# duckdb/duckdb-vss

Hardware: AMD Instinct MI355X
Metric: queries/sec at recall@10, 10M×768 FLOAT top-10; index build rows/sec (higher is better)
Workload: dtype f32

## Files before the change

### duckdb-vss_amd/__init__.py

```python
import ctypes as C
import os
import subprocess

import numpy as np

HERE = os.path.dirname(os.path.abspath(__file__))
ROOT = os.path.dirname(HERE)
LIB_PATH = os.environ.get("VSS_LIBRARY") or os.path.join(HERE, "libvssgpu.so")
CSRC = os.path.join(HERE, "csrc")

METRICS = {"l2sq": 0, "cosine": 1, "ip": 2}
FUNCTIONS = {"array_distance": 0, "array_cosine_distance": 1, "array_negative_inner_product": 2}
FREE_KEY = np.iinfo(np.int64).max

HIPCC_FLAGS = ["--offload-arch=gfx950", "-O3", "-std=c++17", "-ffp-contract=off", "-fPIC", "-Wno-int-to-pointer-cast"]


TRANSLATION_UNITS = ["vss_engine.hip", "vss_exchange.hip", "kernels_l2sq.hip", "kernels_cosine.hip", "kernels_ip.hip",
                     "kernels_boxes_l2sq.hip", "kernels_boxes_cosine.hip", "kernels_boxes_ip.hip",
                     "kernels_setboxes_l2sq.hip", "kernels_setboxes_cosine.hip", "kernels_setboxes_ip.hip"]


def build_library(force=False, extra_flags=(), out=None):
    out = out or os.path.join(HERE, "libvssgpu.so")
# ... 14 lines not shown
            raise RuntimeError("hipcc failed")
    subprocess.check_call(["hipcc", "--offload-arch=gfx950", "-shared", "-fPIC"] + objs + ["-o", out])
    return out


_u64, _i64, _vp, _int, _u32 = C.c_uint64, C.c_int64, C.c_void_p, C.c_int, C.c_uint32
WRITE_CB = C.CFUNCTYPE(_int, _vp, _vp, _u64)
READ_CB = C.CFUNCTYPE(_int, _vp, _vp, _u64)

SIGNATURES = {
    "vss_version": (C.c_char_p, []),
    "vss_create": (_int, [_u64, _int, _u64, _u64, _u64, _u64, _int, C.POINTER(_vp)]),
    "vss_destroy": (None, [_vp]),
    "vss_last_error": (C.c_char_p, [_vp]),
    "vss_set_stream": (_int, [_vp, _vp]),
    "vss_synchronize": (_int, [_vp]),
    "vss_reserve": (_int, [_vp, _u64, _u64]),
    "vss_stage_batch": (_int, [_vp, _vp, _vp, _vp, _u64]),
    "vss_stage_batch_device": (_int, [_vp, _vp, _vp, _u64]),
    "vss_build_finalize": (_int, [_vp]),
    "vss_add_batch": (_int, [_vp, _vp, _vp, _vp, _u64]),
    "vss_set_build_params": (_int, [_vp, _u64, _u64]),
    "vss_set_build_reorder": (_int, [_vp, _int]),
    "vss_set_option": (_int, [_vp, C.c_char_p, _i64]),
    "vss_search": (_int, [_vp, _vp, _u64, _u64, _vp, _vp]),
    "vss_search_batch": (_int, [_vp, _vp, _u64, _u64, _u64, _vp, _vp, _vp]),
    "vss_search_batch_device": (_int, [_vp, _vp, _u64, _u64, _u64, _vp, _vp, _vp]),
    "vss_search_batch_filtered": (_int, [_vp, _vp, _u64, _u64, _u64, _vp, _u64, _vp, _vp, _vp]),
    "vss_search_batch_filtered_device": (_int, [_vp, _vp, _u64, _u64, _u64, _vp, _u64, _vp, _vp, _vp]),
    "vss_search_batch_filtered_groups": (_int, [_vp, _vp, _u64, _u64, _u64, _vp, _u64, _u64, _vp, _vp, _vp, _vp]),
    "vss_search_batch_filtered_groups_device": (_int, [_vp, _vp, _u64, _u64, _u64, _vp, _u64, _u64, _vp, _vp, _vp, _vp]),
    "vss_search_batch_device_begin": (_int, [_vp, _int, _vp, _u64, _u64, _u64, _vp, _vp, _vp]),
    "vss_search_multi_device_begin": (_int, [_vp, _int, _u64, _vp, _u64, _u64, _u64, _vp, _vp, _vp]),
    "vss_search_batch_filtered_device_begin": (_int, [_vp, _int, _vp, _u64, _u64, _u64, _vp, _u64, _vp, _vp, _vp]),
    "vss_search_batch_filtered_groups_device_begin": (_int, [_vp, _int, _vp, _u64, _u64, _u64, _vp, _u64, _u64, _vp, _vp, _vp,
                                                             _vp]),
    "vss_search_multi_filtered_device_begin": (_int, [_vp, _int, _u64, _vp, _u64, _u64, _u64, _vp, _vp, _u64, _vp, _vp, _vp,
                                                      _vp]),
    "vss_search_by_label_device_begin": (_int, [_vp, _int, _vp, _u64, _u64, _u64, _vp, _vp, _vp, _vp]),
    "vss_search_multi_by_label_device_begin": (_int, [_vp, _int, _u64, _vp, _u64, _u64, _u64, _vp, _vp, _vp, _vp]),
    "vss_search_batch_end": (_int, [_vp, _int]),
    "vss_search_exact_batch": (_int, [_vp, _vp, _u64, _u64, _vp, _vp, _vp]),
    "vss_search_exact_batch_device": (_int, [_vp, _vp, _u64, _u64, _vp, _vp, _vp]),
    "vss_search_exact_batch_filtered_groups": (_int, [_vp, _vp, _u64, _u64, _vp, _u64, _u64, _vp, _vp, _vp, _vp]),
    "vss_search_exact_batch_filtered_groups_device": (_int, [_vp, _vp, _u64, _u64, _vp, _u64, _u64, _vp, _vp, _vp, _vp]),
    "vss_last_exact_filtered": (_int, [_vp, _vp]),
    "vss_search_batch_filtered_groups_auto": (_int, [_vp, _vp, _u64, _u64, _u64, _vp, _u64, _u64, _vp, _u64, _vp, _vp, _vp,
                                                     _vp]),
    "vss_search_batch_filtered_groups_auto_device": (_int, [_vp, _vp, _u64, _u64, _u64, _vp, _u64, _u64, _vp, _u64, _vp, _vp,
                                                            _vp, _vp]),
    "vss_last_filter_route": (_int, [_vp, _vp]),
    "vss_set_labels": (_int, [_vp, _u64, _vp, _u64]),
    "vss_set_labels_device": (_int, [_vp, _u64, _vp, _u64]),
    "vss_clear_labels": (_int, [_vp]),
    "vss_labelled_rows": (_u64, [_vp]),
    "vss_search_batch_by_label": (_int, [_vp, _vp, _u64, _u64, _u64, _vp, _int, _u64, _vp, _vp, _vp, _vp]),
    "vss_search_batch_by_label_device": (_int, [_vp, _vp, _u64, _u64, _u64, _vp, _int, _u64, _vp, _vp, _vp, _vp]),
    "vss_search_batch_by_label_range": (_int, [_vp, _vp, _u64, _u64, _u64, _vp, _vp, _int, _u64, _vp, _vp, _vp, _vp]),
    "vss_search_batch_by_label_range_device": (_int, [_vp, _vp, _u64, _u64, _u64, _vp, _vp, _int, _u64, _vp, _vp, _vp, _vp]),
    "vss_search_batch_by_label_set": (_int, [_vp, _vp, _u64, _u64, _u64, _vp, _u64, _int, _u64, _vp, _vp, _vp, _vp]),
    "vss_search_batch_by_label_set_device": (_int, [_vp, _vp, _u64, _u64, _u64, _vp, _u64, _int, _u64, _vp, _vp, _vp, _vp]),
    "vss_set_label_column": (_int, [_vp, _u32, _u64, _vp, _u64]),
    "vss_set_label_column_device": (_int, [_vp, _u32, _u64, _vp, _u64]),
    "vss_clear_label_column": (_int, [_vp, _u32]),
    "vss_label_column_rows": (_u64, [_vp, _u32]),
    "vss_search_batch_by_label_box": (_int, [_vp, _vp, _u64, _u64, _u64, _vp, _u64, _vp, _vp, _int, _u64, _vp, _vp, _vp, _vp]),
    "vss_search_batch_by_label_box_device": (_int, [_vp, _vp, _u64, _u64, _u64, _vp, _u64, _vp, _vp, _int, _u64, _vp, _vp, _vp,
                                                    _vp]),
    "vss_set_label_column64": (_int, [_vp, _u32, _u64, _vp, _u64]),
    "vss_set_label_column64_device": (_int, [_vp, _u32, _u64, _vp, _u64]),
    "vss_label_column_width": (_u32, [_vp, _u32]),
    "vss_search_batch_by_label_box64": (_int, [_vp, _vp, _u64, _u64, _u64, _vp, _u64, _vp, _vp, _int, _u64, _vp, _vp, _vp, _vp]),
    "vss_search_batch_by_label_box64_device": (_int, [_vp, _vp, _u64, _u64, _u64, _vp, _u64, _vp, _vp, _int, _u64, _vp, _vp, _vp,
                                                      _vp]),
    "vss_search_batch_by_label_set_box": (_int, [_vp, _vp, _u64, _u64, _u64, _u32, _vp, _u32, _vp, _u64, _vp, _vp, _int, _u64, _vp, _vp,
                                                 _vp, _vp]),
    "vss_search_batch_by_label_set_box_device": (_int, [_vp, _vp, _u64, _u64, _u64, _u32, _vp, _u32, _vp, _u64, _vp, _vp, _int, _u64,
                                                        _vp, _vp, _vp, _vp]),
    "vss_last_exact_fallbacks": (_u64, [_vp]),
    "vss_last_search_stats": (_int, [_vp, _vp]),
    "vss_last_search_shape": (_int, [_vp, _vp]),
    "vss_last_search_prescore": (_int, [_vp, _vp]),
    "vss_last_search_prescore_descent": (_int, [_vp, _vp]),
    "vss_last_search_query_stats": (_int, [_vp, _vp, _u64]),
    "vss_timing": (_int, [_vp, _vp, _int]),
    "vss_build_work": (_int, [_vp, _vp]),
    "vss_remove_batch": (_int, [_vp, _vp, _u64, _vp]),
    "vss_compact": (_int, [_vp]),
    "vss_compact_ex": (_int, [_vp, _int, _vp]),
    "vss_size": (_u64, [_vp]),
    "vss_nodes": (_u64, [_vp]),
    "vss_build_progress": (_int, [_vp, _vp, _vp]),
    "vss_capacity": (_u64, [_vp]),
    "vss_max_level": (_u64, [_vp]),
    "vss_memory_usage": (_u64, [_vp]),
    "vss_dimensions": (_u64, [_vp]),
    "vss_metric": (_int, [_vp]),
    "vss_level_stats": (_int, [_vp, _u64, _vp]),
    "vss_serialized_length": (_u64, [_vp]),
    "vss_save": (_int, [_vp, WRITE_CB, _vp]),
    "vss_load": (_int, [_vp, READ_CB, _vp]),
    "vss_distance_batch": (_int, [_int, _vp, _vp, _int, _u64, _u64, _vp, _int]),
    "vss_distance_batch_device": (_int, [_int, _vp, _vp, _int, _u64, _u64, _vp, _vp]),
    "vss_merge_topk_device": (_int, [_vp, _vp, _u64, _u64, _u64, _vp, _vp, _vp, _vp]),
    "vss_packed_block_bytes": (_u64, [_u64, _u64]),
    "vss_merge_topk_packed_device": (_int, [_vp, _u64, _u64, _u64, _vp, _vp, _vp, _vp]),
    "vss_exchange_available": (_int, []),
    "vss_exchange_last_error": (C.c_char_p, []),
    "vss_exchange_unique_id": (_int, [_vp]),
    "vss_exchange_init_rank": (_int, [C.POINTER(_vp), _int, _vp, _int, _int]),
    "vss_exchange_init_all": (_int, [C.POINTER(_vp), _int, C.POINTER(_int)]),
    "vss_exchange_adopt": (_int, [C.POINTER(_vp), _vp, _int, _int]),
    "vss_exchange_ranks": (_int, [_vp]),
    "vss_exchange_allgather": (_int, [_vp, _vp, _vp, _u64, _vp]),
    "vss_exchange_group_begin": (_int, []),
    "vss_exchange_group_end": (_int, []),
    "vss_exchange_destroy": (_int, [_vp]),
}

_lib = None


def load_library():
    global _lib
    if _lib is None:
        if not os.path.exists(LIB_PATH):
            build_library()
        try:
            import torch
        except Exception:
            pass
        lib = C.CDLL(LIB_PATH)
        for name, (res, args) in SIGNATURES.items():
            fn = getattr(lib, name)
            fn.restype = res
            fn.argtypes = args
        if hasattr(lib, "vss_debug_phase_ticks"):
            lib.vss_debug_phase_ticks.restype = _int
            lib.vss_debug_phase_ticks.argtypes = [_vp, _vp, _u64]
        _lib = lib
    return _lib


def _p(a):
    if a is None:
        return None
    if isinstance(a, np.ndarray):
        return a.ctypes.data
    return a


class VssError(RuntimeError):
    pass


class LabelPredicateStruct(C.Structure):
    _fields_ = [("kind", _int), ("set_column", _u32), ("set_width", _u32), ("n_columns", _u32), ("columns", _u32 * 4),
                ("d_want", _vp), ("d_sets", _vp), ("d_lo", _vp), ("d_hi", _vp)]


class LabelPredicate:
    KINDS = {"eq": 0, "range": 1, "set": 2, "box": 3, "box64": 4, "set_box": 5}

    def __init__(self, kind, want=None, lo=None, hi=None, sets=None, set_width=0, columns=(), set_column=0):
        self.kind = kind
        self.keep = (want, lo, hi, sets)
# ... 451 lines not shown
                                                           _p(route)))
        return keys, d, cnt, route

    def search_batch_by_label_set_device(self, d_Q, nq, k, ef, d_sets, width, d_keys, d_dist, d_counts, d_route=None, mode="auto",
                                         route_c=0):
        self._check(self.lib.vss_search_batch_by_label_set_device(self.h, d_Q, nq, k, ef, d_sets, width,
                                                                  self.BY_LABEL_MODES.get(mode, mode), route_c, d_keys, d_dist,
                                                                  d_counts, d_route))

    def search_batch_device(self, d_Q, nq, k, ef, d_keys, d_dist, d_counts, exact=False):
        if exact:
            self._check(self.lib.vss_search_exact_batch_device(self.h, d_Q, nq, k, d_keys, d_dist, d_counts))
        else:
            self._check(self.lib.vss_search_batch_device(self.h, d_Q, nq, k, ef, d_keys, d_dist, d_counts))

    def search_begin(self, context, d_Q, nq, k, ef, d_keys, d_dist, d_counts):
        self._check(self.lib.vss_search_batch_device_begin(self.h, context, d_Q, nq, k, ef, d_keys, d_dist, d_counts))

    def search_multi_begin(self, context, d_Qs, per_batch, k, ef, d_keys, d_dists, d_counts):
        n = len(d_Qs)
        tables = [(C.c_void_p * n)(*[int(p) if p else None for p in t]) for t in (d_Qs, d_keys, d_dists, d_counts)]
        self._check(self.lib.vss_search_multi_device_begin(self.h, context, n, tables[0], per_batch, k, ef, tables[1], tables[2],
                                                           tables[3]))

    def search_filtered_begin(self, context, d_Q, nq, k, ef, d_bitmap, n_bits, d_keys, d_dist, d_counts):
        self._check(self.lib.vss_search_batch_filtered_device_begin(self.h, context, d_Q, nq, k, ef, d_bitmap, n_bits, d_keys,
                                                                    d_dist, d_counts))

    def search_filtered_groups_begin(self, context, d_Q, nq, k, ef, d_bitmaps, n_groups, n_bits, d_group_of, d_keys, d_dist,
                                     d_counts):
        self._check(self.lib.vss_search_batch_filtered_groups_device_begin(self.h, context, d_Q, nq, k, ef, d_bitmaps, n_groups,
                                                                           n_bits, d_group_of, d_keys, d_dist, d_counts))

    def search_multi_filtered_begin(self, context, d_Qs, per_batch, k, ef, d_bitmaps, n_groups, n_bits, d_group_ofs, d_keys,
                                    d_dists, d_counts):
        n = len(d_Qs)
        tables = [(C.c_void_p * n)(*[int(p) if p else None for p in t]) if t is not None else None
                  for t in (d_Qs, d_bitmaps, d_group_ofs, d_keys, d_dists, d_counts)]
        groups = (C.c_uint64 * n)(*[int(g) for g in n_groups]) if n_groups is not None else None
        self._check(self.lib.vss_search_multi_filtered_device_begin(self.h, context, n, tables[0], per_batch, k, ef, tables[1],
                                                                    groups, n_bits, tables[2], tables[3], tables[4], tables[5]))

    def search_by_label_begin(self, context, d_Q, nq, k, ef, predicate, d_keys, d_dist, d_counts):
        self._check(self.lib.vss_search_by_label_device_begin(self.h, context, d_Q, nq, k, ef, C.byref(predicate.c), d_keys, d_dist,
                                                              d_counts))

    def search_multi_by_label_begin(self, context, d_Qs, per_batch, k, ef, predicates, d_keys, d_dists, d_counts):
        n = len(d_Qs)
        for name, t in (("predicates", predicates), ("d_keys", d_keys), ("d_dists", d_dists), ("d_counts", d_counts)):
            if t is not None and len(t) != n:
                raise ValueError("%s has %d entries for %d batches" % (name, len(t), n))
        tables = [(C.c_void_p * n)(*[int(p) if p else None for p in t]) if t is not None else None
                  for t in (d_Qs, d_keys, d_dists, d_counts)]
        preds =(LabelPredicateStruct * len(predicates))(*[p.c for p in predicates]) if predicates is not None else None
        self._check(self.lib.vss_search_multi_by_label_device_begin(self.h, context, n, tables[0], per_batch, k, ef, preds, tables[1],
                                                                    tables[2], tables[3]))

    def set_search_gating(self, on):
        self.set_option("search.gating", 1 if on else 0)

    def search_end(self, context):
        self._check(self.lib.vss_search_batch_end(self.h, context))

    def last_search_stats(self):
        out = np.zeros(4, dtype=np.uint64)
        self._check(self.lib.vss_last_search_stats(self.h, _p(out)))
        return out

    def last_search_shape(self):
        out = np.zeros(8, dtype=np.uint32)
        self._check(self.lib.vss_last_search_shape(self.h, _p(out)))
        return out

    def last_search_prescore(self):
        out = np.zeros(4, dtype=np.uint64)
        self._check(self.lib.vss_last_search_prescore(self.h, _p(out)))
        return out

    def last_search_prescore_descent(self):
        out = np.zeros(2, dtype=np.uint64)
        self._check(self.lib.vss_last_search_prescore_descent(self.h, _p(out)))
        return out

    def last_exact_fallbacks(self):
        return int(self.lib.vss_last_exact_fallbacks(self.h))

    def timing(self, reset=False):
        out = np.zeros(6, dtype=np.float64)
        self._check(self.lib.vss_timing(self.h, _p(out), int(reset)))
        return dict(search_kernel_ms=out[0], build_phase_a_ms=out[1], build_phase_b_ms=out[2], build_wall_ms=out[3],
                    build_batches=int(out[4]), build_retries=int(out[5]))

    def build_work(self):
        out = np.zeros(3, dtype=np.uint64)
        self._check(self.lib.vss_build_work(self.h, _p(out)))
        return dict(insert_distances=int(out[0]), insert_expansions=int(out[1]), link_distances=int(out[2]))

    def last_query_stats(self, nq):
        out = np.zeros((nq, 2), dtype=np.uint32)
        self._check(self.lib.vss_last_search_query_stats(self.h, _p(out), nq))
        return out

    def remove(self, rowids):
        rowids = np.ascontiguousarray(rowids, dtype=np.int64)
        n = _u64(0)
        self._check(self.lib.vss_remove_batch(self.h, _p(rowids), len(rowids), C.byref(n)))
        return n.value

    def compact(self, reorder=True):
        done = C.c_int(0)
        self._check(self.lib.vss_compact_ex(self.h, 1 if reorder else 0, C.byref(done)))
        return bool(done.value)

    def size(self):
        return self.lib.vss_size(self.h)

    def nodes(self):
        return self.lib.vss_nodes(self.h)

    def capacity(self):
        return self.lib.vss_capacity(self.h)

    def max_level(self):
        return self.lib.vss_max_level(self.h)

    def build_progress(self):
        a, b = _u64(0), _u64(0)
        self.lib.vss_build_progress(self.h, C.byref(a), C.byref(b))
        return a.value, b.value

    def memory_usage(self):
        return self.lib.vss_memory_usage(self.h)

    def level_stats(self, level):
        out = np.zeros(4, dtype=np.uint64)
        self._check(self.lib.vss_level_stats(self.h, level, _p(out)))
        return out

    def save(self):
        chunks = []

        def write(ctx, data, size):
            chunks.append(C.string_at(data, size))
            return 1
        cb = WRITE_CB(write)
        self._check(self.lib.vss_save(self.h, cb, None))
        return b"".join(chunks)

    def serialized_length(self):
        return self.lib.vss_serialized_length(self.h)

    def save_into(self, buf):
        state = {"off": 0}
        base = buf.ctypes.data

        def write(ctx, data, size):
            if state["off"] + size > buf.nbytes:
                return 0
            C.memmove(base + state["off"], data, size)
            state["off"] += size
            return 1
        cb = WRITE_CB(write)
        self._check(self.lib.vss_save(self.h, cb, None))
        return state["off"]

    def load(self, blob):
# ... 25 lines not shown
```

### duckdb-vss_amd/csrc/hnsw_kernels.h

```cpp
#pragma once
#include "wave_primitives.h"
#include "engine_layout.h"
#include "prescore_bound.h"
#include "filter_groups.h"
#include "label_filter.h"
#include <type_traits>

namespace vss {

constexpr int64_t FREE_KEY = 0x7FFFFFFFFFFFFFFFll;

constexpr uint64_t FILTER_PER_QUERY = 1ull << 63;
constexpr uint64_t FILTER_BY_LABEL = 1ull << 62;
constexpr uint64_t FILTER_BY_RANGE = 1ull << 61;
constexpr uint64_t FILTER_BY_SET = 1ull << 60;
constexpr uint64_t FILTER_FLAGS = FILTER_PER_QUERY | FILTER_BY_LABEL | FILTER_BY_RANGE | FILTER_BY_SET;
constexpr uint64_t FILTER_BY_BOX = FILTER_BY_RANGE | FILTER_BY_SET;
__host__ __device__ constexpr bool filter_by_box(uint64_t filter_bits) {
	return (filter_bits & FILTER_BY_BOX) == FILTER_BY_BOX;
}
constexpr uint64_t FILTER_BY_BOX64 = FILTER_BY_LABEL | FILTER_BY_RANGE | FILTER_BY_SET;
__host__ __device__ constexpr bool filter_by_box64(uint64_t filter_bits) {
	return (filter_bits & FILTER_BY_BOX64) == FILTER_BY_BOX64;
}
// ... 100 lines not shown
			return false;
		if (key < 0 || (uint64_t)key >= (filter_bits & ~FILTER_FLAGS))
			return false;
		const auto *table = (const __attribute__((address_space(4))) unsigned long long *)filter;
		const unsigned long long head = table[0];
		const uint32_t m = host::label_box64_head_columns(head);
		const auto *mine = table + host::label_box_query_cell(m, __builtin_amdgcn_readfirstlane(query));
		uint64_t cell[host::LABEL_COLUMNS_MAX];
#pragma unroll
		for (uint32_t j = 0; j < host::LABEL_COLUMNS_MAX; ++j) {
			cell[j] = 0;
			if (j < m) {
				if (host::label_box64_head_wide(head, j))
					cell[j] = reinterpret_cast<const uint64_t *>(table[1 + j])[key];
				else
					cell[j] = host::label_widen(reinterpret_cast<const uint32_t *>(table[1 + j])[key]);
			}
		}
		bool in = true;
#pragma unroll
		for (uint32_t j = 0; j < host::LABEL_COLUMNS_MAX; ++j)
			if (j < m)
				in &= host::label_range64_cell_admits(cell[j], mine[2 * j], mine[2 * j + 1]);
		return in;
	}

	__device__ __forceinline__ bool admitted_set_box(uint32_t slot, uint32_t query) const {
		typedef unsigned long long words2 __attribute__((ext_vector_type(2)));
		const int64_t key = keys[slot];
		if (key == 0x7FFFFFFFFFFFFFFFll)
			return false;
		if (key < 0 || (uint64_t)key >= (filter_bits & ~FILTER_FLAGS))
			return false;
		const auto *table = (const __attribute__((address_space(4))) unsigned long long *)filter;
		const unsigned long long head = table[0];
		const uint32_t m = host::label_set_box_head_ranges(head), padded = host::label_set_box_head_padded(head);
		const auto *mine = table + host::label_set_box_query_cell(m, padded, __builtin_amdgcn_readfirstlane(query));
		uint64_t cell[host::LABEL_COLUMNS_MAX];
#pragma unroll
		for (uint32_t j = 0; j < host::LABEL_COLUMNS_MAX; ++j) {
			cell[j] = 0;
			if (j <= m) {
				if (host::label_set_box_head_wide(head, j))
					cell[j] = reinterpret_cast<const uint64_t *>(table[1 + j])[key];
				else
					cell[j] = host::label_widen(reinterpret_cast<const uint32_t *>(table[1 + j])[key]);
			}
		}
		const auto *chunk = (const __attribute__((address_space(4))) words2 *)mine;
		bool hit = false;
		for (uint32_t j = 0; j != padded / 2; ++j) {
			const words2 w = chunk[j];
			hit |= host::label64_hits2(cell[0], w.x, w.y);
		}
		bool in = hit & (cell[0] != host::NO_LABEL64);
#pragma unroll
		for (uint32_t j = 0; j < host::LABEL_SET_BOX_RANGES_MAX; ++j)
			if (j < m)
				in &= host::label_range64_cell_admits(cell[1 + j], mine[padded + 2 * j], mine[padded + 2 * j + 1]);
		return in;
	}

	__device__ __forceinline__ uint32_t *list_ptr(uint32_t slot, int level) const {
		return level == 0 ? links0 + (size_t)slot * M0 : links_up + ((size_t)upper_off[slot] + (level - 1)) * M;
	}
	__device__ __forceinline__ uint32_t list_cap(int level) const {
		return level == 0 ? M0 : M;
	}
};

struct WaveLds {
	VisitedSet visited;
	float4 *q;
	float4 *q2;
	uint32_t *ids;
	float *dist;
	float *cand_d;
	uint32_t *cand_s;
	uint32_t *kept_s;
	float *kept_d;
	uint32_t touch_lines = 0;
	uint32_t *spill_box = nullptr;
	uint32_t query = 0;
};

struct WorkCounters {
	uint32_t distances;
	uint32_t cycles;
#ifdef VSS_PHASE_TIMERS
	uint32_t t_pick, t_gather, t_dist, t_accept, t_descend, t_total;
	uint32_t t_sync1, t_look, t_slice, t_sync2, t_team_passes, t_solo_passes;
#endif
};

#ifdef VSS_PHASE_TIMERS
#define VSS_TICK(var) const unsigned long long var = __builtin_readcyclecounter()
#define VSS_ACC(field, a, b) wc.field += (uint32_t)((b) - (a))
#define VSS_COUNT(field, n) wc.field += (n)
#define VSS_WC_ARG , WorkCounters &wc
#define VSS_WC_PASS , wc
#define VSS_PHASE_STRIDE 12
#else
#define VSS_WC_ARG
#define VSS_WC_PASS
#define VSS_TICK(var)
#define VSS_ACC(field, a, b)
#define VSS_COUNT(field, n)
#endif

__device__ __forceinline__ bool mark_first_visit(VisitedSet &visited, uint32_t id, bool have, bool twins, uint32_t &bad) {
	if (!twins)
		return have && !visited.test_and_set(id, bad);
	const int seen = have ? visited.probe(id, bad) : VisitedSet::SEEN_BEFORE;
	bool fresh = seen == VisitedSet::INSERTED;
	unsigned long long lost = __ballot(seen == VisitedSet::LOST_TO_TWIN);
	while (lost) {
		const uint32_t key = read_lane(id, __builtin_ctzll(lost));
		const bool mine = seen != VisitedSet::SEEN_BEFORE && id == key;
		const unsigned long long group = __ballot(mine);
		const bool inserted_now = __ballot(mine && seen == VisitedSet::INSERTED) != 0;
		if (mine)
			fresh = inserted_now && lane_id() == __builtin_ctzll(group);
		lost &= ~group;
	}
	return fresh;
}

template <bool FILTER>
__device__ __forceinline__ int gather_neighbors(const GraphView &gv, WaveLds &lds, uint32_t slot, int level,
                                                bool have_first = false, uint32_t first = EMPTY_SLOT) {
	const int lane = lane_id();
	const uint32_t cap = gv.list_cap(level);
	const uint32_t *lp = gv.list_ptr(slot, level);
	int n = 0;
	uint32_t bad = 0;
	for (uint32_t off = 0; off < cap; off += 64) {
		uint32_t id;
		if (off == 0 && have_first)
			id = first;
		else
			id = (off + lane < cap) ? lp[off + lane] : EMPTY_SLOT;
		bool take = id != EMPTY_SLOT;
		if (FILTER) {
			take = mark_first_visit(lds.visited, id, take, gv.twins != 0, bad);
			if (lds.visited.compact && lds.spill_box && __ballot(bad != 0)) {
				lds.visited.migrate(reinterpret_cast<uint32_t *>((uintptr_t)lds.spill_box[0] | ((uintptr_t)lds.spill_box[1] << 32)),
				                    lds.spill_box[2]);
				if (lane == 0)
					lds.spill_box[3] = 1u;
				const bool again = bad != 0;
				uint32_t none = 0;
				const bool fresh = mark_first_visit(lds.visited, id, again, gv.twins != 0, none);
				take = again ? fresh : take;
				bad = 0;
			}
		}
		unsigned long long m = __ballot(take);
		if (take)
			lds.ids[n + __popcll(m & lanes_below(lane))] = id;
		n += __popcll(m);
	}
	if (FILTER) {
		lds.visited.count += n;
		if (lds.visited.count > lds.visited.limit) {
			if (!(lds.visited.compact && lds.spill_box))
				return -1;
			lds.visited.migrate(reinterpret_cast<uint32_t *>((uintptr_t)lds.spill_box[0] | ((uintptr_t)lds.spill_box[1] << 32)),
			                    lds.spill_box[2]);
			if (lane == 0)
				lds.spill_box[3] = 1u;
			if (lds.visited.count > lds.visited.limit)
				return -1;
		}
		if (lds.visited.compact && __ballot(bad != 0))
			return -1;
	}
	lds_sync();
	return n;
}

struct ListPrefetch {
	uint32_t slot = EMPTY_SLOT;
	uint32_t cells = EMPTY_SLOT;
	uint32_t cap = 0;
	uint32_t fresh = 0;
	__device__ __forceinline__ void request(const GraphView &gv, uint32_t want, int level) {
		if (want == slot)
			return;
		cap = gv.list_cap(level);
		const uint32_t *lp = gv.list_ptr(want, level);
		cells = lp[(uint32_t)lane_id() < cap ? lane_id() : 0];
		slot = want;
		fresh = 1;
	}
	__device__ __forceinline__ uint32_t masked() const {
		return (uint32_t)lane_id() < cap ? cells : EMPTY_SLOT;
	}
};

template <int K>
struct ListCache {
	static constexpr int slots = K;
	uint32_t slot[K];
	uint32_t cells[K];
	uint32_t cap = 0;
	uint32_t next = 0;
	uint32_t fresh = 0;
	__device__ __forceinline__ ListCache() {
#pragma unroll
		for (int i = 0; i < K; ++i)
			slot[i] = EMPTY_SLOT, cells[i] = EMPTY_SLOT;
	}
	__device__ __forceinline__ bool find(uint32_t want, uint32_t &out) const {
		bool hit = false;
		out = EMPTY_SLOT;
#pragma unroll
		for (int i = 0; i < K; ++i)
			if (slot[i] == want) {
				out = cells[i];
				hit = true;
			}
		if ((uint32_t)lane_id() >= cap)
			out = EMPTY_SLOT;
		return hit;
// ... 97 lines not shown
					}
				cache.clear_fresh();
			}
		}
		if (lane_id() == 0)
			box->touch_n = k;
		__syncthreads();
	}
	template <typename F>
	__device__ __forceinline__ void operator()(const WaveLds &lds, const RowSpace &sp, float qa2, int n, F before_loads
	                                           VSS_WC_ARG) const {
		NoListCache none;
		run(lds, sp, qa2, n, before_loads, none, false);
	}
};
__host__ __device__ constexpr int team_touch_max_lines(int nch) {
	return nch > 0 ? 8 * nch : 8;
}
template <int MT, int NCH, int R, int T>
__device__ __forceinline__ void team_help(const WaveLds &lds, const RowSpace &sp, const TeamBox *box, int wave, uint32_t lines) {
	constexpr int LPH = (team_touch_max_lines(NCH) + T - 2) / (T - 1);
	uint32_t sink[2][LPH];
#pragma unroll
	for (int k = 0; k < 2; ++k)
#pragma unroll
		for (int j = 0; j < LPH; ++j)
			sink[k][j] = 0;
	for (;;) {
		__syncthreads();
		const unsigned long long nq = *reinterpret_cast<const unsigned long long *>(box);
		const int n = uniform((int)(uint32_t)nq);
		if (n < 0)
			break;
		const float qa2 = __int_as_float(uniform((int)(uint32_t)(nq >> 32)));
		int lo, hi;
		team_share(sp, n, T, wave, lo, hi);
		if (hi > lo)
			wave_distances<MT, NCH, R>(sp, lds.q, qa2, lds.ids + lo, hi - lo, lds.dist + lo);
		__syncthreads();
		const uint32_t tn = (uint32_t)uniform((int)box->touch_n);
		if (tn) {
#pragma unroll
			for (int k = 0; k < 2; ++k)
#pragma unroll
				for (int j = 0; j < LPH; ++j)
					asm volatile("" ::"v"(sink[k][j]));
#pragma unroll
			for (int k = 0; k < 2; ++k) {
				if ((uint32_t)k >= tn)
					continue;
				const uint32_t id = box->cells[k][lane_id()];
				if (id == EMPTY_SLOT)
					continue;
				const char *row = reinterpret_cast<const char *>(sp.vectors + (size_t)id * sp.V);
#pragma unroll
				for (int j = 0; j < LPH; ++j) {
					const uint32_t l = (uint32_t)(wave - 1) + (uint32_t)j * (T - 1);
					if (l < lines)
						sink[k][j] = *reinterpret_cast<const uint32_t *>(row + l * 128u);
				}
			}
		}
	}
#pragma unroll
	for (int k = 0; k < 2; ++k)
#pragma unroll
		for (int j = 0; j < LPH; ++j)
			asm volatile("" ::"v"(sink[k][j]));
}

#ifdef VSS_PARANOID
#define VSS_TRACE(sp, idx, expr) ((sp).debug[idx] = (expr))
#define VSS_TRACE_INC(sp, idx) atomicAdd(lane_id() == 0 ? &(sp).debug[idx] : &(sp).debug[64 + lane_id()], 1u)
#else
#define VSS_TRACE(sp, idx, expr)
#define VSS_TRACE_INC(sp, idx)
#endif
#ifndef VSS_WALKER_WAIT_SLEEP
#define VSS_WALKER_WAIT_SLEEP 1
#endif
#ifndef VSS_SCORER_IDLE_SLEEP
#define VSS_SCORER_IDLE_SLEEP 2
#endif
struct Mailbox {
	unsigned long long ticket;
	uint32_t done;
	uint32_t qa2_bits;
	uint32_t slots;
	uint32_t bound_bits;
	uint32_t pad[2];
};

struct PrescoreView {
	const uint32_t *codes;
	const RowCodeMeta *meta;
	unsigned long long *counters;
};
constexpr uint32_t PRESCORE_SLOTS = 16;
__host__ __device__ constexpr int prescore_claim_rows(int R) {
	return 4 * R;
}
__device__ __forceinline__ float code_to_float(uint32_t w, int k) {
	return (float)(int)(int8_t)(w >> (8 * k));
}
template <int MT, int NCH, int CR>
__device__ __forceinline__ unsigned long long prescore_codes(const RowSpace &sp, const PrescoreView &pv, uint32_t dim,
                                                             const float4 *q_lds, float qa2, const uint32_t *ids, int n,
                                                             float bound, float *out, uint32_t &rejected) {
	static_assert(NCH >= 2, "full-wave rows only");
	const uint32_t lane = lane_id();
	constexpr int PER = 64 / CR;
	uint32_t w[NCH][CR];
	float sc[CR];
#pragma unroll
	for (int r = 0; r < CR; ++r) {
		const uint32_t id = ids[r < n ? r : n - 1];
		const uint32_t *crow = pv.codes + (size_t)id * sp.V;
#pragma unroll
		for (int ch = 0; ch < NCH; ++ch)
			w[ch][r] = crow[lane + ch * 64];
		sc[r] = MT == 0 ? pv.meta[id].scale : 0.f;
	}
	const int jm = (int)(lane / PER) < n ? (int)(lane / PER) : n - 1;
	const float4 mraw = *reinterpret_cast<const float4 *>(pv.meta + ids[jm]);
	__builtin_amdgcn_sched_barrier(0);
	float t[CR];
#pragma unroll
	for (int r = 0; r < CR; ++r)
		t[r] = 0.f;
#pragma unroll
	for (int ch = 0; ch < NCH; ++ch) {
		const float4 q = q_lds[lane + ch * 64];
		const float qs[4] = {q.x, q.y, q.z, q.w};
#pragma unroll
		for (int r = 0; r < CR; ++r)
#pragma unroll
			for (int k = 0; k < 4; ++k) {
				const float c = code_to_float(w[ch][r], k);
				if (MT == 0) {
					const float v = __fmaf_rn(-sc[r], c, qs[k]);
					t[r] = __fmaf_rn(v, v, t[r]);
				} else {
					t[r] = __fmaf_rn(qs[k], c, t[r]);
				}
			}
	}
	transposed_reduce64<CR>(t);
	RowCodeMeta m;
	m.scale = mraw.x, m.err = mraw.y, m.norm = mraw.z, m.spare = 0;
	const float lb = prescore_bound(MT, t[0], t[0], m, MT == 0 ? 1.f : vss_sqrt(qa2), dim);
	const bool mine = (lane % PER) == 0 && (int)(lane / PER) < n;
	const bool rej = mine && lb >= bound;
	if (rej)
		out[lane / PER] = __builtin_inff();
	rejected += (uint32_t)__popcll(__ballot(rej));
	return __ballot(mine && !rej);
}
template <int MT, int NCH, int RR>
__device__ __forceinline__ void wave_distances_picked(const RowSpace &sp, const float4 *q_lds, float qa2, const uint32_t *ids,
                                                      unsigned long long &left, int lane_shift, float *out) {
	const uint32_t lane = lane_id();
	int pos[RR], last = 0;
	const float4 *row[RR];
#pragma unroll
	for (int r = 0; r < RR; ++r) {
		if (left)
			last = (int)(__builtin_ctzll(left) >> lane_shift);
		pos[r] = last;
		left &= left - 1ull;
		row[r] = sp.vectors + (size_t)ids[pos[r]] * sp.V;
	}
	float4 x[NCH][RR];
#pragma unroll
	for (int ch = 0; ch < NCH; ++ch)
#pragma unroll
		for (int r = 0; r < RR; ++r)
			x[ch][r] = row[r][lane + ch * 64];
	float ab[RR], b2[RR];
#pragma unroll
	for (int r = 0; r < RR; ++r)
		ab[r] = 0.f, b2[r] = 0.f;
#pragma unroll
	for (int ch = 0; ch < NCH; ++ch) {
		const float4 q = q_lds[lane + ch * 64];
#pragma unroll
		for (int r = 0; r < RR; ++r)
			accumulate4<MT>(q, x[ch][r], ab[r], b2[r]);
	}
	transposed_reduce64<RR>(ab);
	if (MT == 1)
		transposed_reduce64<RR>(b2);
	constexpr int PER = 64 / RR;
	int j = pos[0];
#pragma unroll
	for (int r = 1; r < RR; ++r)
		j = (int)(lane / PER) == r ? pos[r] : j;
	if ((lane % PER) == 0)
		out[j] = finish_distance<MT>(ab[0], qa2, b2[0]);
}


typedef __attribute__((address_space(3))) unsigned long long lds_u64;
typedef __attribute__((address_space(3))) uint32_t lds_u32;
typedef __attribute__((address_space(3))) float lds_f32;
typedef uint32_t lds_u32x4 __attribute__((ext_vector_type(4)));
typedef __attribute__((address_space(3))) lds_u32x4 lds_u32x4_as3;
#define VSS_LDS_PTR(type, ptr) ((type *)(uint32_t)(uintptr_t)(ptr))
#define VSS_LDS_LOAD(type, ptr) __hip_atomic_load(VSS_LDS_PTR(type, ptr), __ATOMIC_RELAXED, __HIP_MEMORY_SCOPE_WORKGROUP)
#define VSS_LDS_STORE(type, ptr, v) __hip_atomic_store(VSS_LDS_PTR(type, ptr), (v), __ATOMIC_RELAXED, __HIP_MEMORY_SCOPE_WORKGROUP)
#define VSS_LDS_ADD(type, ptr, v) __hip_atomic_fetch_add(VSS_LDS_PTR(type, ptr), (v), __ATOMIC_RELAXED, __HIP_MEMORY_SCOPE_WORKGROUP)
#ifdef VSS_RELAXED_MAILBOX
#define VSS_MB_RELEASE __ATOMIC_RELAXED
#define VSS_MB_ACQUIRE __ATOMIC_RELAXED
#else
#define VSS_MB_RELEASE __ATOMIC_RELEASE
#define VSS_MB_ACQUIRE __ATOMIC_ACQUIRE
#endif
#define VSS_LDS_LOAD_ACQ(type, ptr) __hip_atomic_load(VSS_LDS_PTR(type, ptr), VSS_MB_ACQUIRE, __HIP_MEMORY_SCOPE_WORKGROUP)
#define VSS_LDS_STORE_REL(type, ptr, v) __hip_atomic_store(VSS_LDS_PTR(type, ptr), (v), VSS_MB_RELEASE, __HIP_MEMORY_SCOPE_WORKGROUP)
#define VSS_LDS_ADD_ACQ(type, ptr, v) __hip_atomic_fetch_add(VSS_LDS_PTR(type, ptr), (v), VSS_MB_ACQUIRE, __HIP_MEMORY_SCOPE_WORKGROUP)
#define VSS_LDS_ADD_REL(type, ptr, v) __hip_atomic_fetch_add(VSS_LDS_PTR(type, ptr), (v), VSS_MB_RELEASE, __HIP_MEMORY_SCOPE_WORKGROUP)

template <int MT, int NCH, int R, bool PRE = false>
__device__ __forceinline__ bool pool_score(Mailbox *mb, unsigned long long *scrap, const RowSpace &sp, const float4 *q,
                                           const uint32_t *ids, float *dist, const PrescoreView *pv = nullptr, uint32_t dim = 0,
                                           uint32_t *pre_counts = nullptr) {
	const int lane = lane_id();
	unsigned long long *ticket_or_scrap = lane == 0 ? &mb->ticket : scrap + lane;
	uint32_t *done_or_scrap = lane == 0 ? &mb->done : reinterpret_cast<uint32_t *>(scrap + lane);
	bool worked = false;
	for (;;) {
		uint32_t slots = (uint32_t)uniform((int)VSS_LDS_LOAD(lds_u32, &mb->slots));
		const bool wide_claim = PRE && slots == PRESCORE_SLOTS;
		slots = slots == 1 || slots == 2 ? slots : (uint32_t)R;
		const uint32_t pass = wide_claim ? (uint32_t)prescore_claim_rows(R) : slots * (64u >> sp.logG);
		const unsigned long long t = VSS_LDS_ADD_ACQ(lds_u64, ticket_or_scrap, (unsigned long long)pass);
		const uint32_t c = (uint32_t)uniform((int)(uint32_t)t), n = (uint32_t)uniform((int)(uint32_t)(t >> 32));
		VSS_TRACE_INC(sp, 25);
		VSS_TRACE(sp, 27, c);
		VSS_TRACE(sp, 28, n);
		if (c >= n)
			break;
		VSS_TRACE_INC(sp, 26);
		const uint32_t cnt = n - c < pass ? n - c : pass;
#ifdef VSS_PARANOID
		{
			bool bad = n > 4096;
			for (uint32_t j = lane_id(); !bad && j < cnt; j += 64)
				bad = ids[c + j] >= sp.debug_rows;
			if (sp.debug && __ballot(bad)) {
				if (lane_id() == 0 && atomicAdd(&sp.debug[0], 1u) == 0) {
					sp.debug[1] = c, sp.debug[2] = n, sp.debug[3] = ids[c], sp.debug[4] = blockIdx.x;
					sp.debug[5] = (uint32_t)(threadIdx.x >> 6), sp.debug[6] = (uint32_t)(mb->ticket >> 32);
					sp.debug[7] = (uint32_t)mb->ticket, sp.debug[8] = cnt, sp.debug[9] = ids[c + cnt - 1];
				}
				VSS_LDS_ADD(lds_u32, done_or_scrap, cnt);
				worked = true;
				continue;
			}
		}
#endif
		const float qa2 = __uint_as_float(VSS_LDS_LOAD(lds_u32, &mb->qa2_bits));
		if constexpr (PRE) {
			if (pv->codes) {
				const float bound = __uint_as_float((uint32_t)uniform((int)VSS_LDS_LOAD(lds_u32, &mb->bound_bits)));
			if (bound < __builtin_inff()) {
					constexpr int CR = prescore_claim_rows(R);
					constexpr int SHIFT = CR == 16 ? 2 : CR == 8 ? 3 : 4;
					static_assert(CR == 16 || CR == 8 || CR == 4, "rows of codes per claim");
					unsigned long long left = prescore_codes<MT, NCH, CR>(sp, *pv, dim, q, qa2, ids + c, (int)cnt, bound, dist + c, pre_counts[1]);
					pre_counts[0] += cnt;
					while (left) {
						const int have = __popcll(left);
						if (have >= 3 && R >= 4)
							wave_distances_picked<MT, NCH, (R >= 4 ? 4 : 1)>(sp, q, qa2, ids + c, left, SHIFT, dist + c);
						else if (have >= 2)
							wave_distances_picked<MT, NCH, 2>(sp, q, qa2, ids + c, left, SHIFT, dist + c);
						else
							wave_distances_picked<MT, NCH, 1>(sp, q, qa2, ids + c, left, SHIFT, dist + c);
					}
					wave_sync();
					VSS_LDS_ADD_REL(lds_u32, done_or_scrap, cnt);
					VSS_TRACE_INC(sp, 29);
					worked = true;
					continue;
				}
			}
		}
		if (slots == 1)
			wave_distances<MT, NCH, 1>(sp, q, qa2, ids + c, (int)cnt, dist + c);
		else if (slots == 2)
			wave_distances<MT, NCH, 2>(sp, q, qa2, ids + c, (int)cnt, dist + c);
		else
			wave_distances<MT, NCH, R>(sp, q, qa2, ids + c, (int)cnt, dist + c);
		VSS_LDS_ADD_REL(lds_u32, done_or_scrap, cnt);
		VSS_TRACE_INC(sp, 29);
		worked = true;
	}
	return worked;
}

constexpr uint32_t POOL_SPIN_LIMIT = 1u << 26;

struct CrewBox {
	int n;
	float qa2;
	uint32_t walker;
	uint32_t on;
};
static_assert(sizeof(CrewBox) == 16 && sizeof(Mailbox) == 32, "engine LDS header layout");

template <int MT, int NCH, int R, bool PRE = false>
struct PoolScorer {
	static constexpr bool touches_rows = false, touches_lists = true, helpers_touch = false;
	Mailbox *mb;
	uint32_t *exit_flag;
	uint32_t *engine_error;
	uint32_t *walkers_left;
	uint32_t scorers;
	CrewBox *crew;
	uint32_t my_slot;
	uint32_t crew_ok;
	uint32_t no_requests;
	uint32_t touch_ok;
	uint32_t prescore_ok;
	unsigned long long *descent_counters;
	mutable uint32_t crew_on = 0;
	mutable uint32_t level = 0;
	mutable float hop_bound = __builtin_inff();
	mutable uint32_t hop_filtered = 0;
	static constexpr bool bounds_descent = PRE;
	__device__ __forceinline__ void at_level(int l) const {
		level = (uint32_t)l;
	}
	__device__ __forceinline__ void at_bound(float bound) const {
		hop_bound = (PRE && descent_counters) ? bound : __builtin_inff();
	}
	__device__ __forceinline__ void add_descent_counts(uint32_t rows, uint32_t rejected) const {
		if (PRE && descent_counters && rows && lane_id() == 0) {
			atomicAdd(descent_counters, (unsigned long long)rows);
			atomicAdd(descent_counters + 1, (unsigned long long)rejected);
		}
	}

	__device__ __forceinline__ bool wants_requests() const {
		return !(crew_on && no_requests);
	}

	__device__ __forceinline__ bool latency_mode() const {
		return crew_on != 0 && touch_ok != 0;
	}
	__device__ __forceinline__ uint32_t active_walkers() const {
		const uint32_t active = (uint32_t)uniform((int)VSS_LDS_LOAD(lds_u32, walkers_left));
		return active ? active : 1u;
	}
	__device__ __forceinline__ bool post(int buf, const RowSpace &sp, int n, float bound = __builtin_inff()) const {
		Mailbox *box = mb + buf;
		bool sent = false;
		const uint32_t lg = 6u - sp.logG;
		const uint32_t x1 = ((uint32_t)n + (1u << lg) - 1u) >> lg, x2 = (x1 + 1u) >> 1;
		const uint32_t a = active_walkers();
		if (PRE && prescore_ok) {
			const bool filtered = bound < __builtin_inff() && a * x2 > scorers;
			VSS_LDS_STORE(lds_u32, &box->slots, a * x1 <= scorers ? 1u : a * x2 <= scorers ? 2u : filtered ? PRESCORE_SLOTS : (uint32_t)R);
			VSS_LDS_STORE(lds_u32, &box->bound_bits, __float_as_uint(filtered ? bound : __builtin_inff()));
			sent = filtered;
		} else {
			VSS_LDS_STORE(lds_u32, &box->slots, a * x1 <= scorers ? 1u : a * x2 <= scorers ? 2u : (uint32_t)R);
		}
		VSS_LDS_STORE(lds_u32, &box->done, 0u);
		VSS_LDS_STORE_REL(lds_u64, &box->ticket, (unsigned long long)(uint32_t)n << 32);
		VSS_TRACE_INC(sp, 16);
		VSS_TRACE(sp, 17, (uint32_t)n);
		return sent;
	}
	__device__ __forceinline__ void wait(int buf, const RowSpace &sp, int n) const {
		Mailbox *box = mb + buf;
		uint32_t spins = 0;
		while (uniform((int)VSS_LDS_LOAD_ACQ(lds_u32, &box->done)) < n) {
			__builtin_amdgcn_s_sleep(VSS_WALKER_WAIT_SLEEP);
			if ((spins & 1023u) == 0) {
				VSS_TRACE(sp, 20, spins);
				VSS_TRACE(sp, 21, VSS_LDS_LOAD(lds_u32, &box->done));
			}
			if (++spins > POOL_SPIN_LIMIT || ((spins & 1023u) == 0 && uniform((int)VSS_LDS_LOAD(lds_u32, exit_flag)))) {
				if (lane_id() == 0) {
					VSS_LDS_STORE(lds_u32, exit_flag, 2u);
					__hip_atomic_store(engine_error, 1u, __ATOMIC_RELAXED, __HIP_MEMORY_SCOPE_SYSTEM);
				}
				__builtin_amdgcn_endpgm();
			}
		}
		wave_sync();
		VSS_TRACE_INC(sp, 18);
	}
	__device__ __forceinline__ bool begin(int buf, const RowSpace &sp, float qa2, int n, float bound = __builtin_inff()) const {
		if (crew_ok && !crew_on && uniform((int)VSS_LDS_LOAD(lds_u32, walkers_left)) == 1) {
			crew_on = 1u;
#ifdef VSS_PHASE_TIMERS
			if (lane_id() < 3)
				reinterpret_cast<unsigned long long *>(reinterpret_cast<unsigned char *>(crew) - ENGINE_CREW_OFFSET + ENGINE_SCRAP_OFFSET)[lane_id()] = 0;
#endif
			VSS_LDS_STORE_REL(lds_u32, &crew->on, 1u);
		}
		if (crew_on) {
			if (lane_id() == 0) {
				crew->n = n;
				crew->qa2 = qa2;
				crew->walker = 2u * my_slot + (uint32_t)buf + (level << 8);
			}
			lds_barrier();
			return false;
		}
		return post(buf, sp, n, bound);
	}
	__device__ __forceinline__ void end(int buf, const RowSpace &sp, int n) const {
		if (crew_on)
			lds_barrier();
		else
			wait(buf, sp, n);
	}
	template <typename F>
	__device__ __forceinline__ void operator()(const WaveLds &lds, const RowSpace &sp, float qa2, int n, F before_loads
	                                           VSS_WC_ARG) const {
		if (n <= 0) {
			hop_filtered = 0;
			before_loads();
			return;
		}
		VSS_TICK(tp0);
		hop_filtered = begin(0, sp, qa2, n, hop_bound) ? 1u : 0u;
		VSS_TICK(tpb);
		VSS_ACC(t_solo_passes, tp0, tpb);
		before_loads();
		VSS_TICK(tp1);
		end(0, sp, n);
		VSS_TICK(tp3);
		VSS_ACC(t_look, tp0, tp1);
		VSS_ACC(t_sync2, tp1, tp3);
	}
	__device__ __forceinline__ void dismiss_crew() const {
		if (lane_id() == 0)
			crew->n = -1;
		lds_barrier();
	}
};

template <int MT, bool AHEAD = false, class Scorer>
__device__ __forceinline__ uint32_t descend(const GraphView &gv, WaveLds &lds, float qa2, uint32_t closest,
                                            int begin_level, int end_level, const Scorer &score, WorkCounters &wc) {
	const int lane = lane_id();
	float closest_dist = wave_distance_one<MT>(gv.sp, lds.q, qa2, closest);
	wc.distances += 1;
	ListPrefetch below;
	int below_level = -1;
	const bool can_ahead = AHEAD && gv.M0 <= 64;
	uint32_t pre_rows = 0, pre_rejected = 0;
	for (int level = begin_level; level > end_level; --level) {
		bool changed;
		do {
			changed = false;
			const bool have_first = can_ahead && below.slot == closest && below_level == level;
			const int n = gather_neighbors<false>(gv, lds, closest, level, have_first, have_first ? below.masked() : EMPTY_SLOT);
			if constexpr (AHEAD)
				score.at_level(level);
			score.at_bound(closest_dist);
			score(lds, gv.sp, qa2, n, [&] {
				if constexpr (AHEAD) {
					if (can_ahead && !(below.slot == closest && below_level == level - 1)) {
						below.slot = EMPTY_SLOT;
						below.request(gv, closest, level - 1);
						below_level = level - 1;
					}
				}
			} VSS_WC_PASS);
			wc.distances += n;
			wc.cycles += 1;
			bool counted = false;
			if constexpr (Scorer::bounds_descent) {
				counted = score.hop_filtered != 0;
				if (counted)
					pre_rows += (uint32_t)n;
			}
			for (int off = 0; off < n; off += 64) {
				const float d = (off + lane < n) ? lds.dist[off + lane] : __builtin_inff();
				if constexpr (Scorer::bounds_descent) {
					if (counted)
						pre_rejected += (uint32_t)__popcll(__ballot(off + lane < n && d == __builtin_inff()));
				}
				float m = d;
				m = fminf(m, lane_xor<32>(m));
				m = fminf(m, lane_xor<16>(m));
				m = fminf(m, lane_xor<8>(m));
				m = fminf(m, lane_xor<4>(m));
				m = fminf(m, lane_xor<2>(m));
				m = fminf(m, lane_xor<1>(m));
				if (m < closest_dist) {
					const unsigned long long who = __ballot(d == m);
					closest_dist = m;
					closest = lds.ids[off + __builtin_ctzll(who)];
					changed = true;
				}
			}
			wave_sync();
		} while (changed);
	}
	if constexpr (AHEAD)
		score.at_level(end_level);
	if constexpr (Scorer::bounds_descent) {
		score.at_bound(__builtin_inff());
		score.add_descent_counts(pre_rows, pre_rejected);
	}
	return closest;
}
// ... 305 lines not shown
					sb.dist(b)[at] = d;
				}
				n += __popcll(m);
			}
			lds.visited.count += n;
			wave_sync();
			if (lds.visited.count > lds.visited.limit || (lds.visited.compact && __ballot(bad != 0)))
				return LEVEL_VISITED_OVERFLOW;
		} else {
			b = have_spec ? 1 - spec_buf : 0;
			lds.ids = sb.ids(b);
			n = gather_neighbors<true>(gv, lds, cs, 0, ahead.slot == cs, ahead.masked());
			if (n < 0)
				return LEVEL_VISITED_OVERFLOW;
			if (n > 0)
				pool.post(b, gv.sp, n);
			if (ns != EMPTY_SLOT)
				ahead.request(gv, ns, 0);
		}
		VSS_TICK(tk2);
		VSS_ACC(t_gather, tk1, tk2);
		if (ns != EMPTY_SLOT && !(have_spec && spec_slot == ns) && pool.active_walkers() <= max_active) {
			const int ob = 1 - b;
			if (have_spec)
				pool.wait(spec_buf, gv.sp, spec_n);
			have_spec = false;
			const uint32_t id = ahead.slot == ns ? ahead.masked() : EMPTY_SLOT;
			const bool take = id != EMPTY_SLOT && !lds.visited.contains(id);
			const unsigned long long m = __ballot(take);
			if (take)
				sb.ids(ob)[__popcll(m & lanes_below(lane))] = id;
			const int n2 = __popcll(m);
			wave_sync();
			if (n2 > 0) {
				pool.post(ob, gv.sp, n2);
				have_spec = true;
				spec_slot = ns;
				spec_buf = ob;
				spec_n = n2;
			}
		}
		VSS_TICK(tk2b);
		VSS_ACC(t_look, tk2, tk2b);
		if (n == 0)
			continue;
		pool.wait(b, gv.sp, n);
		wc.distances += n;
		VSS_TICK(tk3);
		VSS_ACC(t_dist, tk2b, tk3);
		for (int off = 0; off < n; off += 64) {
			const bool have = off + lane < n;
			const float d = have ? sb.dist(b)[off + lane] : 0.f;
			const uint32_t id = have ? sb.ids(b)[off + lane] : 0;
			const unsigned long long pass = __ballot(have && (L.size < limit || d < radius));
			L.accept(d, id, pass, radius);
		}
		wave_sync();
		VSS_TICK(tk4);
		VSS_ACC(t_accept, tk3, tk4);
	}
	if (have_spec)
		pool.wait(spec_buf, gv.sp, spec_n);
	return LEVEL_OK;
}

template <int MT, int PK, class List, class Pool>
__device__ __forceinline__ int level_search_pipelined(const GraphView &gv, WaveLds &lds, const SpecBuffers &sb, float qa2,
                                                      uint32_t start, int limit, List &L, const Pool &pool, WorkCounters &wc) {
	const int lane = lane_id();
	lds.visited.clear();
	L.reset(limit);
	if (lane == 0)
		lds.visited.test_and_set(start);
	lds.visited.count = 1;
	const float d0 = wave_distance_one<MT>(gv.sp, lds.q, qa2, start);
	wc.distances += 1;
	wave_sync();
	float radius = d0;
	L.insert(d0, start);

	ListCache<PK> ahead;
	float e_d = __builtin_inff();
	uint32_t e_s = EMPTY_SLOT;
	auto request_ahead = [&] {
		float d1 = 0.f;
		uint32_t s1 = 0, s2 = 0;
		int have;
		if constexpr (PK > 1) {
			have = L.first_two_unexpanded_entry(d1, s1, s2);
		} else {
			have = L.first_unexpanded_entry(d1, s1) >= 0 ? 1 : 0;
		}
		e_d = have > 0 ? d1 : __builtin_inff();
		e_s = have > 0 ? s1 : EMPTY_SLOT;
		if (!pool.wants_requests())
			return;
		if (have > 0)
			ahead.request(gv, s1, 0);
		if constexpr (PK > 1) {
			if (have > 1)
				ahead.request(gv, s2, 0);
		}
	};
	auto open_expansion = [&](uint32_t cs, int buf) -> int {
		VSS_TICK(tg0);
		uint32_t first_cells;
		const bool have_first = ahead.find(cs, first_cells);
		VSS_COUNT(t_slice, have_first ? 1u : 0u);
		lds.ids = sb.ids(buf);
		const int n = gather_neighbors<true>(gv, lds, cs, 0, have_first, first_cells);
		VSS_TICK(tg1);
		VSS_ACC(t_gather, tg0, tg1);
		if (n > 0)
			pool.begin(buf, gv.sp, qa2, n, L.size >= limit ? radius : __builtin_inff());
		VSS_TICK(tg2);
		VSS_ACC(t_solo_passes, tg1, tg2);
		return n;
	};
	auto accept = [&](int buf, int n) {
		const bool have = lane < n;
		const float d = have ? sb.dist(buf)[lane] : 0.f;
		const uint32_t id = have ? sb.ids(buf)[lane] : 0;
		const unsigned long long pass = __ballot(have && (L.size < limit || d < radius));
		L.accept(d, id, pass, radius);
	};

	int b = 0, n_cur = 0;
	for (;;) {
		if (n_cur == 0) {
			VSS_TICK(tk0);
			float cd;
			uint32_t cs;
			const int pos = L.first_unexpanded_entry(cd, cs);
			if (pos < 0)
				break;
			L.mark_expanded(pos);
			wc.cycles += 1;
			VSS_TICK(tk1);
			VSS_ACC(t_pick, tk0, tk1);
			n_cur = open_expansion(cs, b);
			if (n_cur < 0)
				return LEVEL_VISITED_OVERFLOW;
			request_ahead();
			continue;
		}
		VSS_TICK(tw0);
		pool.end(b, gv.sp, n_cur);
		VSS_TICK(tw1);
		VSS_ACC(t_sync2, tw0, tw1);
		wc.distances += n_cur;
		uint32_t next = EMPTY_SLOT;
		bool tie;
		{
			const bool have = lane < n_cur;
			const float d = have ? sb.dist(b)[lane] : 0.f;
			const uint32_t id = have ? sb.ids(b)[lane] : 0;
			const bool admitted = have && (L.size < limit || d < radius);
			float m = admitted ? d : __builtin_inff();
			m = fminf(m, lane_xor<32>(m));
			m = fminf(m, lane_xor<16>(m));
			m = fminf(m, lane_xor<8>(m));
			m = fminf(m, lane_xor<4>(m));
			m = fminf(m, lane_xor<2>(m));
			m = fminf(m, lane_xor<1>(m));
			const unsigned long long who = __ballot(admitted && !(d > m));
			const float ms = __int_as_float(uniform(__float_as_int(m)));
			tie = who && (__popcll(who) > 1 || !(__builtin_fabsf(ms) < __builtin_inff()) || ms == e_d);
			if (!tie)
				next = (who && ms < e_d) ? read_lane(id, __builtin_ctzll(who)) : e_s;
		}
		VSS_TICK(tw2);
		VSS_ACC(t_pick, tw1, tw2);
		if (tie) {
			accept(b, n_cur);
			n_cur = 0;
			VSS_TICK(tw3);
			VSS_ACC(t_accept, tw2, tw3);
			continue;
		}
		const int nb = 1 - b;
		int n_next = 0;
		if (next != EMPTY_SLOT) {
			wc.cycles += 1;
			n_next = open_expansion(next, nb);
			if (n_next < 0)
				return LEVEL_VISITED_OVERFLOW;
		}
		VSS_TICK(ta0);
		accept(b, n_cur);
		uint32_t first = EMPTY_SLOT;
		int pos;
		{
			float cd;
			uint32_t w = EMPTY_SLOT;
			pos = L.first_unexpanded_entry(cd, w);
			if (pos >= 0)
				first = w;
		}
		if (first != next) {
			if (n_next > 0)
				pool.end(nb, gv.sp, n_next);
			return LEVEL_INTERNAL;
		}
		if (next == EMPTY_SLOT)
			break;
		L.mark_expanded(pos);
		request_ahead();
		VSS_TICK(ta1);
		VSS_ACC(t_accept, ta0, ta1);
		b = nb;
		n_cur = n_next;
	}
	return LEVEL_OK;
}

template <int MT, int NCH, int R>
__device__ __forceinline__ int refine_candidates(const GraphView &gv, WaveLds &lds, int count, int needed,
                                                 WorkCounters &wc) {
	const int lane = lane_id();
	if (count < needed) {
		for (int i = lane; i < count; i += 64) {
			lds.kept_s[i] = lds.cand_s[i];
			lds.kept_d[i] = lds.cand_d[i];
		}
		wave_sync();
		return count;
	}
	if (lane == 0) {
		lds.kept_s[0] = lds.cand_s[0];
		lds.kept_d[0] = lds.cand_d[0];
	}
	wave_sync();
	int submitted = 1, consumed = 1;
	while (submitted < needed && consumed < count) {
		const uint32_t cs = lds.cand_s[consumed];
		const float cd = lds.cand_d[consumed];
		stage_row(lds.q2, gv.sp.vectors + (size_t)cs * gv.sp.V, gv.sp.V);
		const float c2 = MT == 1 ? wave_query_norm(gv.sp, lds.q2) : 0.f;
		const int pass = R * (64 >> gv.sp.logG);
		bool bad = false;
		for (int off = 0; off < submitted && !bad; off += pass) {
			const int n = submitted - off < pass ? submitted - off : pass;
			wave_distances<MT, NCH, R>(gv.sp, lds.q2, c2, lds.kept_s + off, n, lds.dist);
			wc.distances += n;
			for (int o = 0; o < n; o += 64) {
				const bool b = (o + lane < n) && (lds.dist[o + lane] < cd);
				bad = bad || (__ballot(b) != 0ull);
			}
			wave_sync();
		}
		if (!bad) {
			if (lane == 0) {
				lds.kept_s[submitted] = cs;
				lds.kept_d[submitted] = cd;
			}
			submitted++;
			wave_sync();
		}
		consumed++;
	}
	return submitted;
}

constexpr int MAX_COALESCED = 32;
struct SearchArgs {
	GraphView gv;
	const float *queries[MAX_COALESCED];
	uint32_t batch_size;
	uint32_t q_stride;
	uint32_t n_queries;
	uint32_t k, ef;
	uint32_t entry;
	int max_level;
	uint32_t tomb;
	uint32_t hash_log2;
	uint32_t list_cap_max;
	uint32_t walkers;
	uint32_t stage_cap;
	uint32_t spec_active;
	uint32_t touch_lines;
	uint32_t crew;
	uint32_t pipelined;
	const uint32_t *work;
	uint32_t *queue;
	uint32_t queue_sel;
	uint32_t *engine_error;
	uint32_t *drain_flag;
	uint32_t *done_count;
	int64_t *out_keys[MAX_COALESCED];
	float *out_d[MAX_COALESCED];
	uint32_t *out_count[MAX_COALESCED];
	uint32_t *out_stats;
	uint32_t *status;
	uint32_t *retry_hash;
	uint32_t retry_log2;
	uint32_t *global_hash;
	float *list_buf;
	uint32_t list_cap;
	uint32_t list_lds;
	float *cand_buf;
	uint32_t cand_cap;
	uint32_t visited_compact;
	unsigned long long *phase_ticks;
	PrescoreView prescore;
	uint32_t prescore_descent;
};

__device__ __forceinline__ void bind_visited(VisitedSet &v, uint32_t *table, uint32_t hash_log2) {
	v.table = table;
	v.mask = (1u << hash_log2) - 1;
	v.shift = 32 - hash_log2;
	v.limit = ((1u << hash_log2) / 8) * 7;
	v.count = 0;
	v.compact = 0;
}
__device__ __forceinline__ void bind_visited_compact(VisitedSet &v, uint32_t form) {
	const uint32_t cells_log2 = compact_visited::cells_log2_of(form);
	v.mask = (1u << cells_log2) - 1;
	v.limit = ((1u << cells_log2) / 4) * 3;
	v.compact = form;
}

__device__ __forceinline__ void carve_lds(WaveLds &lds, unsigned char *base, uint32_t hash_log2, uint32_t V,
                                          uint32_t list_cap_max, uint32_t cand_cap, uint32_t *global_hash = nullptr) {
	unsigned char *p = base;
	bind_visited(lds.visited, global_hash ? global_hash + ((size_t)blockIdx.x << hash_log2) : reinterpret_cast<uint32_t *>(p),
	             hash_log2);
	if (!global_hash)
		p += align16((1u << hash_log2) * 4);
	lds.q = reinterpret_cast<float4 *>(p);
	p += align16(V * 16);
	lds.q2 = reinterpret_cast<float4 *>(p);
	p += align16(V * 16);
	lds.ids = reinterpret_cast<uint32_t *>(p);
	p += align16(list_cap_max * 4);
	lds.dist = reinterpret_cast<float *>(p);
	p += align16(list_cap_max * 4);
	lds.cand_d = reinterpret_cast<float *>(p);
	p += align16(cand_cap * 4);
	lds.cand_s = reinterpret_cast<uint32_t *>(p);
	p += align16(cand_cap * 4);
	lds.kept_s = reinterpret_cast<uint32_t *>(p);
	p += align16((list_cap_max + 1) * 4);
	lds.kept_d = reinterpret_cast<float *>(p);
}

struct EngineSlot {
	float4 *q;
	uint32_t *ids, *ids2;
	float *dist, *dist2;
	uint32_t *hash;
	float *stage_d;
	uint32_t *stage_s;
	float *list_d;
	uint32_t *list_s;
	float *list_tops;
};
__device__ __forceinline__ EngineSlot engine_slot(unsigned char *smem, uint32_t s, uint32_t hash_log2, uint32_t V,
                                                  uint32_t list_cap_max, bool hash_in_lds, uint32_t stage_cap,
                                                  uint32_t list_cells = 0) {
	unsigned char *p =
	    smem + ENGINE_HEADER_BYTES + s * engine_slot_bytes(hash_log2, V, list_cap_max, hash_in_lds, stage_cap, list_cells);
	EngineSlot e;
	e.hash = hash_in_lds ? reinterpret_cast<uint32_t *>(p) : nullptr;
	if (hash_in_lds)
		p += align16((1u << hash_log2) * 4);
	e.q = reinterpret_cast<float4 *>(p);
	p += align16(V * 16);
	e.ids = reinterpret_cast<uint32_t *>(p);
	p += align16(list_cap_max * 4);
	e.dist = reinterpret_cast<float *>(p);
	p += align16(list_cap_max * 4);
	e.ids2 = reinterpret_cast<uint32_t *>(p);
	p += align16(list_cap_max * 4);
	e.dist2 = reinterpret_cast<float *>(p);
	p += align16(list_cap_max * 4);
	e.stage_d = stage_cap ? reinterpret_cast<float *>(p) : nullptr;
	p += align16(stage_cap * 4);
	e.stage_s = stage_cap ? reinterpret_cast<uint32_t *>(p) : nullptr;
	p += align16(stage_cap * 4);
	e.list_d = list_cells ? reinterpret_cast<float *>(p) : nullptr;
	p += align16(list_cells * 4);
	e.list_s = list_cells ? reinterpret_cast<uint32_t *>(p) : nullptr;
	p += align16(list_cells * 4);
	e.list_tops = list_cells ? reinterpret_cast<float *>(p) : nullptr;
	return e;
}

// ... 99 lines not shown
				others += simd_of[w] != wsimd;
			const bool use_spare = spare && others >= 4;
			H = 0, h = -1;
			for (int w = S; w < waves; ++w) {
				const bool takes = !use_spare || simd_of[w] != wsimd;
				if (w == wave)
					h = takes ? H : -1;
				H += takes;
			}
			H = uniform(H), h = uniform(h);
			inv_h = (65536u + (uint32_t)H - 1u) / (uint32_t)H;
		}
		const uint32_t *ids = (where & 1u) ? ids1 : ids0;
		float *dist = (where & 1u) ? dist1 : dist0;
		const uint32_t un = (uint32_t)n;
		const int ceil_nh = (un + (uint32_t)H - 1u) * (uint32_t)H < 65536u ? (int)(((un + (uint32_t)H - 1u) * inv_h) >> 16)
		                                                                    : (int)((un + (uint32_t)H - 1u) / (uint32_t)H);
		const int per = (ceil_nh + RG - 1) & ~(RG - 1);
		const int lo = h < 0 ? n : (h * per < n ? h * per : n);
		const int hi = lo + per < n ? lo + per : n;
#ifdef VSS_PHASE_TIMERS
		unsigned long long t_issue = th0;
#endif
		if (hi > lo) {
			asm volatile("" ::"v"(sink));
			CrewTouch hook;
			hook.gv = &a.gv, hook.ids = ids + lo, hook.rows = hi - lo, hook.level = level, hook.sink = &sink;
			hook.lines = touch_on ? ((level == 0 ? a.gv.M0 : a.gv.M) > 32 ? 2u : 1u) : 0u;
#ifdef VSS_PHASE_TIMERS
			hook.t_issue = &t_issue;
#endif
			const int slots = per >> (6 - (int)a.gv.sp.logG);
			if (slots <= 1)
				wave_distances<MT, NCH, 1>(a.gv.sp, q, qa2, ids + lo, hi - lo, dist + lo, hook);
			else if (slots == 2)
				wave_distances<MT, NCH, 2>(a.gv.sp, q, qa2, ids + lo, hi - lo, dist + lo, hook);
			else
				wave_distances<MT, NCH, R>(a.gv.sp, q, qa2, ids + lo, hi - lo, dist + lo, hook);
		}
		VSS_TICK(th2);
		lds_barrier();
#ifdef VSS_PHASE_TIMERS
		if (h == 0 && lane_id() == 0) {
			acc[0] += t_issue - th0;
			acc[1] += th2 - t_issue;
			acc[2] += __builtin_readcyclecounter() - th2;
		}
#endif
	}
	asm volatile("" ::"v"(sink));
}

constexpr int LDS_LIST_E = 64;
template <int MT, int NCH, int R, int E, int THREADS, int GROUPS>
__device__ __forceinline__ void search_engine(SearchArgs &a) {
	static_assert(E == 0 || E == LDS_LIST_E || (E >= 1 && E <= MAX_LIST_REGS), "candidate list: registers, HBM or LDS");
	extern __shared__ __attribute__((aligned(16))) unsigned char smem[];
	const int lane = lane_id();
	const uint32_t wave = (uint32_t)uniform((int)(threadIdx.x >> 6));
	const uint32_t S = a.walkers;
	const bool hash_in_lds = a.global_hash == nullptr;
	const uint32_t list_cells = E == LDS_LIST_E ? a.list_lds : 0u;
	uint32_t *exit_flag = reinterpret_cast<uint32_t *>(smem);
	uint32_t *walkers_left = exit_flag + 1;
	CrewBox *crew = reinterpret_cast<CrewBox *>(smem + ENGINE_CREW_OFFSET);
	Mailbox *boxes = reinterpret_cast<Mailbox *>(smem + ENGINE_BOX_OFFSET);
	unsigned long long *scrap = reinterpret_cast<unsigned long long *>(smem + ENGINE_SCRAP_OFFSET);
	if (threadIdx.x == 0) {
		*exit_flag = 0;
		*walkers_left = S;
		crew->n = 0, crew->qa2 = 0.f, crew->walker = 0, crew->on = 0;
		a.queue[a.queue_sel ^ 2u] = 0;
	}
	VSS_TRACE(a.gv.sp, 30, blockDim.x);
	VSS_TRACE(a.gv.sp, 31, S);
	if (lane == 0)
		smem[ENGINE_SIMD_OFFSET + wave] = (unsigned char)__builtin_amdgcn_s_getreg((1 << 11) | (4 << 6) | 4);
	if (threadIdx.x < ENGINE_BOXES) {
		boxes[threadIdx.x].ticket = 0;
		boxes[threadIdx.x].done = 0;
		boxes[threadIdx.x].qa2_bits = 0;
		boxes[threadIdx.x].slots = R;
		boxes[threadIdx.x].bound_bits = 0x7F800000u;
	}
	__syncthreads();
	constexpr bool PRE = NCH >= 2 && E >= 1 && E != LDS_LIST_E && E <= pipelined_max_regs(THREADS);

	if (wave >= S) {
		uint32_t pre_counts[2] = {0, 0};
		auto leave = [&] {
			if constexpr (PRE) {
				if (lane == 0 && pre_counts[0]) {
					atomicAdd(a.prescore.counters, (unsigned long long)pre_counts[0]);
					atomicAdd(a.prescore.counters + 1, (unsigned long long)pre_counts[1]);
				}
			}
		};
		for (;;) {
			bool worked = false;
			VSS_TRACE_INC(a.gv.sp, 24);
			for (uint32_t s = 0; s < 2 * S; ++s) {
				const unsigned long long t = VSS_LDS_LOAD(lds_u64, &boxes[s].ticket);
				if (uniform((int)((uint32_t)t < (uint32_t)(t >> 32)))) {
					const EngineSlot es =
					    engine_slot(smem, s >> 1, a.hash_log2, a.gv.sp.V, a.list_cap_max, hash_in_lds, a.stage_cap, list_cells);
					worked |= pool_score<MT, NCH, R, PRE>(&boxes[s], scrap, a.gv.sp, es.q, (s & 1) ? es.ids2 : es.ids,
					                                      (s & 1) ? es.dist2 : es.dist, &a.prescore, a.gv.dim, pre_counts);
				}
			}
			if (uniform((int)VSS_LDS_LOAD(lds_u32, exit_flag))) {
				leave();
				return;
			}
			if (uniform((int)VSS_LDS_LOAD_ACQ(lds_u32, &crew->on))) {
				leave();
				crew_help<MT, NCH, R>(smem, a, crew, (int)wave, (int)S, (int)(blockDim.x >> 6), hash_in_lds, list_cells);
				return;
			}
			if (!worked)
				__builtin_amdgcn_s_sleep(VSS_SCORER_IDLE_SLEEP);
		}
	}

	__builtin_amdgcn_s_setprio(2);
	const EngineSlot es = engine_slot(smem, wave, a.hash_log2, a.gv.sp.V, a.list_cap_max, hash_in_lds, a.stage_cap, list_cells);
	const size_t gslot = (size_t)blockIdx.x * S + wave;
	WaveLds lds;
	bind_visited(lds.visited, hash_in_lds ? es.hash : a.global_hash + (gslot << a.hash_log2), a.hash_log2);
	if constexpr (E == MAX_LIST_REGS) {
		if (a.visited_compact)
			bind_visited_compact(lds.visited, a.visited_compact);
	}
	lds.q = es.q, lds.ids = es.ids, lds.dist = es.dist;
	lds.q2 = nullptr, lds.kept_s = nullptr, lds.kept_d = nullptr;
	lds.cand_d = nullptr, lds.cand_s = nullptr;
	lds.touch_lines = a.touch_lines & TOUCH_LISTS;
	PoolScorer<MT, NCH, R, PRE> score {&boxes[2 * wave], exit_flag, a.engine_error, walkers_left, (blockDim.x >> 6) - S, crew, wave,
	                                   ((a.crew & CREW_ON) && !a.spec_active) ? 1u : 0u, (a.crew & CREW_NO_REQUESTS) ? 1u : 0u,
	                                   (a.crew & CREW_TOUCH) ? 1u : 0u, (PRE && a.prescore.codes) ? 1u : 0u,
	                                   (PRE && a.prescore.codes && a.prescore_descent) ? a.prescore.counters + 2 : nullptr};
	const SpecBuffers sb {es.ids, es.ids2, es.dist, es.dist2};
	CandQueue cq;
	cq.bind(a.cand_buf + gslot * 2 * a.cand_cap, reinterpret_cast<uint32_t *>(a.cand_buf + gslot * 2 * a.cand_cap) + a.cand_cap,
	        (int)a.cand_cap);
	typename std::conditional<E == LDS_LIST_E, LdsList,
	                          typename std::conditional<E == 0, MemList, WaveList<(E == 0 || E == LDS_LIST_E ? 1 : E)>>::type>::type L;
	if constexpr (E == 0)
		L.bind(a.list_buf + gslot * 2 * a.list_cap, reinterpret_cast<uint32_t *>(a.list_buf + gslot * 2 * a.list_cap) + a.list_cap);
	if constexpr (E == LDS_LIST_E)
		L.bind(es.list_d, es.list_s, es.list_tops);
	const int limit = a.ef > a.k ? a.ef : a.k;

	constexpr bool CAN_MOVE = E == MAX_LIST_REGS;
	if constexpr (CAN_MOVE) {
		if (a.retry_hash && hash_in_lds && es.stage_d) {
			lds.spill_box = reinterpret_cast<uint32_t *>(es.stage_d);
			if (lane == 0) {
				const uintptr_t t = (uintptr_t)(a.retry_hash + (gslot << a.retry_log2));
				lds.spill_box[0] = (uint32_t)t, lds.spill_box[1] = (uint32_t)(t >> 32), lds.spill_box[2] = a.retry_log2, lds.spill_box[3] = 0;
			}
			lds_sync();
		}
	}
	for (;;) {
		const uint32_t idx = (uint32_t)uniform((int)atomicAdd(lane == 0 ? a.queue + a.queue_sel : a.queue + 4 + lane, 1u));
		if (idx >= a.n_queries)
			break;
		if (idx + 1 == a.n_queries && a.drain_flag)
			__hip_atomic_store(a.drain_flag, 1u, __ATOMIC_RELAXED, __HIP_MEMORY_SCOPE_SYSTEM);
		const uint32_t qi = a.work ? a.work[idx] : idx;
		if constexpr (GROUPS)
			lds.query = qi;
		VSS_TRACE(a.gv.sp, 19, 1u);
		const uint32_t batch = qi / a.batch_size, row = qi - batch * a.batch_size;
		stage_query(lds.q, a.queries[batch] + (size_t)row * a.q_stride, a.gv.dim, a.gv.sp.V);
		VSS_TRACE(a.gv.sp, 19, 2u);
		const float qa2 = (MT == 1 || (PRE && MT == 2 && a.prescore.codes)) ? wave_query_norm(a.gv.sp, lds.q) : 0.f;
		VSS_LDS_STORE(lds_u32, &boxes[2 * wave].qa2_bits, __float_as_uint(qa2));
		VSS_LDS_STORE(lds_u32, &boxes[2 * wave + 1].qa2_bits, __float_as_uint(qa2));
		lds.ids = es.ids, lds.dist = es.dist;
		WorkCounters wc = {};
		VSS_TICK(tq0);
		uint32_t closest = descend<MT, (E >= 1 && E <= 4)>(a.gv, lds, qa2, a.entry, a.max_level, 0, score, wc);
		VSS_TICK(tq1);
		VSS_ACC(t_descend, tq0, tq1);
		VSS_TRACE(a.gv.sp, 19, 3u);
		int rc;
		constexpr int PK = (NCH == 6 || NCH == 4 || E == 0 || E == LDS_LIST_E || E >= 8) ? 1 : 2;
		if (a.tomb == 1) {
			if constexpr (E == 2 || E == 4 || E == 8) {
				RegQueue<(E == 8 ? E : 2 * E)> rq;
				rc = level_search_impl<MT, false, true, 1, MAX_LIST_REGS, GROUPS>(a.gv, lds, qa2, closest, EMPTY_SLOT, 0, limit, L, rq, score, wc);
			} else {
				rc = LEVEL_QUEUE_OVERFLOW;
			}
		} else if (a.tomb)
			rc = level_search_impl<MT, false, true, 1, MAX_LIST_REGS, GROUPS>(a.gv, lds, qa2, closest, EMPTY_SLOT, 0, limit, L, cq, score, wc);
		else if (GROUPS)
			rc = LEVEL_INTERNAL;
		else if (a.spec_active)
			rc = level_search_spec<MT>(a.gv, lds, sb, qa2, closest, limit, L, score, a.spec_active, wc);
		else if (E > 0 && E != LDS_LIST_E && E <= pipelined_max_regs(THREADS) && a.pipelined) {
			if constexpr (E > 0 && E != LDS_LIST_E && E <= pipelined_max_regs(THREADS))
				rc = level_search_pipelined<MT, PK>(a.gv, lds, sb, qa2, closest, limit, L, score, wc);
			else
				rc = LEVEL_INTERNAL;
		} else
			rc = level_search_impl<MT, false, false, PK>(a.gv, lds, qa2, closest, EMPTY_SLOT, 0, limit, L, cq, score, wc);
		bool moved = false;
		if constexpr (CAN_MOVE) {
			if (lds.spill_box) {
				moved = uniform((int)lds.spill_box[3]) != 0;
				if (moved) {
					uint32_t hl = a.hash_log2;
					asm volatile("" : "+s"(hl));
					bind_visited(lds.visited, es.hash, hl);
					if (a.visited_compact)
						bind_visited_compact(lds.visited, a.visited_compact);
					if (lane == 0)
						lds.spill_box[3] = 0;
					lds_sync();
				}
			}
		}
		VSS_TRACE(a.gv.sp, 19, 4u);
		const int count = rc == LEVEL_OK ? (L.size < (int)a.k ? L.size : (int)a.k) : 0;
		emit_results(a.gv, a.out_keys[batch] + (size_t)row * a.k, a.out_d[batch] ? a.out_d[batch] + (size_t)row * a.k : nullptr,
		             (int)a.k, L, count);
		if (lane == 0) {
			a.out_count[batch][row] = count;
			a.status[qi] = (rc == LEVEL_OK && moved) ? (uint32_t)LEVEL_OK_RETRIED : (uint32_t)rc;
			if (a.out_stats) {
				a.out_stats[2 * qi] = wc.distances;
				a.out_stats[2 * qi + 1] = wc.cycles;
			}
#ifdef VSS_PHASE_TIMERS
			if (a.phase_ticks) {
				unsigned long long *o = a.phase_ticks + VSS_PHASE_STRIDE * (size_t)qi;
				o[0] = wc.t_pick, o[1] = wc.t_gather, o[2] = wc.t_dist, o[3] = wc.t_accept, o[4] = wc.t_descend;
				o[5] = __builtin_readcyclecounter() - tq0;
				o[6] = wc.t_sync1, o[7] = wc.t_look, o[8] = wc.t_slice, o[9] = wc.t_sync2, o[10] = wc.t_team_passes;
				o[11] = wc.t_solo_passes;
				if (score.crew_on) {
					unsigned long long *acc = reinterpret_cast<unsigned long long *>(smem + ENGINE_SCRAP_OFFSET);
					o[6] = acc[0], o[8] = acc[1], o[10] = acc[2];
					acc[0] = acc[1] = acc[2] = 0;
				}
			}
#endif
		}
		if (a.done_count) {
			__threadfence_system();
			if (lane == 0)
				__hip_atomic_fetch_add(a.done_count, 1u, __ATOMIC_RELEASE, __HIP_MEMORY_SCOPE_SYSTEM);
		}
	}
	VSS_TRACE(a.gv.sp, 19, 5u);
	if (score.crew_on) {
		score.dismiss_crew();
		return;
	}
	if (lane == 0 && VSS_LDS_ADD(lds_u32, walkers_left, 0xFFFFFFFFu) == 1u)
		VSS_LDS_STORE(lds_u32, exit_flag, 1u);
	VSS_TRACE(a.gv.sp, 19, 6u);
}

template <int MT, int NCH, int R, int E, int THREADS = 1024>
__global__ __launch_bounds__(THREADS) void k_search(SearchArgs a) {
	search_engine<MT, NCH, R, E, THREADS, 0>(a);
}
template <int MT, int NCH, int R, int E, int THREADS = 1024>
__global__ __launch_bounds__(THREADS) void k_search_groups(SearchArgs a) {
	search_engine<MT, NCH, R, E, THREADS, 1>(a);
}
template <int MT, int NCH, int R, int E, int THREADS = 1024>
__global__ __launch_bounds__(THREADS) void k_search_labels(SearchArgs a) {
	search_engine<MT, NCH, R, E, THREADS, 2>(a);
}
template <int MT, int NCH, int R, int E, int THREADS = 1024>
__global__ __launch_bounds__(THREADS) void k_search_ranges(SearchArgs a) {
	search_engine<MT, NCH, R, E, THREADS, 3>(a);
}
template <int MT, int NCH, int R, int E, int THREADS = 1024>
__global__ __launch_bounds__(THREADS) void k_search_sets(SearchArgs a) {
	search_engine<MT, NCH, R, E, THREADS, 4>(a);
}
template <int MT, int NCH, int R, int E, int THREADS = 1024>
__global__ __launch_bounds__(THREADS) void k_search_boxes(SearchArgs a) {
// ... 707 lines not shown
```

### duckdb-vss_amd/csrc/host_logic.h

```cpp
#pragma once
#include <algorithm>
#include <cmath>
#include <cstddef>
#include <cstdint>
#include <vector>

#include "engine_layout.h"
#include "lds_list_index.h"
#include "visited_compact.h"

namespace vss {
namespace host {

constexpr int64_t FREE_KEY_HOST = 0x7FFFFFFFFFFFFFFFll;
constexpr uint32_t NO_SLOT = 0xFFFFFFFFu;

inline size_t ceil_pow2(size_t v) {
	size_t p = 1;
	while (p < v)
		p <<= 1;
	return p;
}
inline uint32_t log2u(size_t v) {
	uint32_t l = 0;
// ... 216 lines not shown
constexpr uint32_t LDS_BYTES_PER_CU = 160u * 1024;
struct SearchShapePolicy {
	uint32_t solo_mode = 1;
	uint32_t solo_max_queries = 32;
	uint32_t solo_max_bytes = 32 * 1024;
	bool team = true;
	uint32_t n_cus = 256;
	bool touch_rows = true, touch_lists = true;
	uint32_t touch_max_queries = 256;
	bool force_looping = false;
	bool crew = true;
	uint32_t engine_walkers = 0;
};
struct SearchShape {
	bool solo = false, team = false;
	uint32_t touch_lines = 0;
	bool crew = false;
	bool roomy = false;
};
inline uint32_t chunks_per_lane(uint64_t V, uint64_t G, bool force_looping) {
	return (V % G == 0 && !force_looping) ? (uint32_t)(V / G) : 0u;
}
inline bool team_variant_exists(uint32_t nch) {
	return nch <= 1;
}
inline uint32_t team_touch_lines_max(uint32_t nch) {
	return nch > 0 ? 8 * nch : 8;
}
inline bool wants_solo(const SearchShapePolicy &p, uint32_t n, uint64_t M0, uint64_t V, uint64_t G) {
	if (p.solo_mode != 1)
		return p.solo_mode == 2;
	if (M0 * V * 16 > p.solo_max_bytes)
		return false;
	return n <= p.solo_max_queries ||
	       (p.team && team_variant_exists(chunks_per_lane(V, G, p.force_looping)) && n <= p.n_cus);
}
inline bool one_walker_launch(const SearchShapePolicy &p, uint32_t n) {
	return p.engine_walkers ? p.engine_walkers == 1 : n <= p.n_cus;
}
inline SearchShape search_shape_before_lds(const SearchShapePolicy &p, uint32_t n, uint64_t M0, uint64_t V, uint64_t G) {
	SearchShape s;
	s.solo = wants_solo(p, n, M0, V, G);
	if (!s.solo) {
		s.crew = p.crew;
		const bool one_walker = s.roomy = one_walker_launch(p, n);
		if (s.crew && one_walker && n <= p.n_cus && n <= p.touch_max_queries && p.touch_lists)
			s.touch_lines = TOUCH_LISTS;
		return s;
	}
	s.roomy = true;
	return s;
}
inline void settle_solo_shape(const SearchShapePolicy &p, SearchShape &s, uint32_t n, uint64_t V, uint64_t G, uint32_t solo_lds_bytes) {
	if (!s.solo)
		return;
	const uint32_t nch = chunks_per_lane(V, G, p.force_looping);
	s.team = p.team && team_variant_exists(nch) && n <= p.n_cus && solo_lds_bytes + TEAM_BOX_BYTES <= LDS_BYTES_PER_CU;
	if (n <= p.touch_max_queries) {
		const uint32_t row_lines = (uint32_t)((V * 16 + 127) / 128);
		const uint32_t max_lines = s.team ? team_touch_lines_max(nch) : 4u;
		if (p.touch_rows && row_lines <= max_lines)
			s.touch_lines = row_lines;
		if (p.touch_lists)
			s.touch_lines |= TOUCH_LISTS;
	}
}
inline SearchShape choose_search_shape(const SearchShapePolicy &p, uint32_t n, uint64_t M0, uint64_t V, uint64_t G,
                                       uint32_t solo_lds_bytes) {
	SearchShape s = search_shape_before_lds(p, n, M0, V, G);
	settle_solo_shape(p, s, n, V, G, solo_lds_bytes);
	return s;
}

struct SearchEngineConfig {
	SearchShapePolicy policy;
	uint64_t M0 = 32, V = 1, G = 1, list_cap_max = 64;
	uint64_t nodes = 0;
	uint32_t hash_max_log2 = 10;
	uint32_t search_waves = 16, search_walkers_cap = 4, search_wgs_per_cu = 1;
	uint32_t search_spec_active = 0;
	bool search_pipelined = true, search_wide_lists = true;
	uint32_t search_list_lds = 1, search_prescore = 1;
	bool search_prescore_descent = true;
	bool retry_in_place = true;
	uint64_t visited_per_limit = 0;
	uint32_t hash_lds_max_log2 = 13, hash_lds_max_override = 0;
	bool visited_compact_on = true;
	uint32_t search_crew_tune = 0;
};
struct SearchLaunchInput {
	uint32_t n = 0;
	uint64_t limit = 0;
	uint32_t bump = 0, min_hash_log2 = 0;
	uint64_t list_cap = 0;
	uint32_t cand_cap = 0;
	uint32_t tomb = 0;
	bool direct_io = false;
};
struct SearchLaunchPlan {
	bool solo = false, team = false;
	uint32_t threads = 0, walkers = 0, grid = 0, lds_bytes = 0, regs = 0, nch = 0;
	uint32_t hash_log2 = 0;
	bool hash_in_lds = false;
	uint32_t visited_compact = 0, stage_cap = 0;
	uint32_t retry_log2 = 0;
	bool roomy = false;
	uint32_t list_place = LIST_IN_REGISTERS, list_lds = 0;
	uint32_t pipelined = 0, crew = 0, touch_lines = 0, spec_active = 0;
	bool wants_prescore = false;
	uint32_t prescore_descent = 0;
	uint64_t global_hash = 0, retry_hash = 0, list_buf = 0, cand_buf = 0;
	uint32_t shape[8] = {0, 0, 0, 0, 0, 0, 0, 0};
};
inline SearchLaunchPlan plan_search_launch(const SearchEngineConfig &e, const SearchLaunchInput &in) {
	SearchLaunchPlan a;
	const SearchShapePolicy &policy = e.policy;
	const uint32_t n = in.n, n_cus = policy.n_cus, V = (uint32_t)e.V, list_cap_max = (uint32_t)e.list_cap_max;
	SearchShape shape = search_shape_before_lds(policy, n, e.M0, e.V, e.G);
	const bool solo = a.solo = shape.solo;
	const bool roomy = a.roomy = shape.roomy;
	a.hash_log2 = visited_set_log2(in.limit, in.bump, e.M0, e.list_cap_max,
	                               e.visited_per_limit ? e.visited_per_limit : search_cells_per_limit(in.limit), e.hash_max_log2);
	if (roomy && a.hash_log2 <= e.hash_lds_max_log2)
		a.hash_log2 = std::min<uint32_t>({a.hash_log2 + 2, 14u, std::max(a.hash_log2, e.hash_max_log2)});
	a.hash_log2 = std::max(a.hash_log2, std::min(in.min_hash_log2, e.hash_max_log2));
	const uint32_t lds_table_log2 = roomy ? 14u : (e.hash_lds_max_override ? e.hash_lds_max_override : e.hash_lds_max_log2);
	bool hash_in_lds = a.hash_log2 <= lds_table_log2;
	a.visited_compact = e.visited_compact_on ? compact_visited_cells_log2(hash_in_lds, solo, !in.list_cap, in.limit, e.nodes,
	                                                                      !in.bump && !in.min_hash_log2, lds_table_log2)
	                                         : 0u;
	if (a.visited_compact) {
		a.hash_log2 = lds_table_log2;
		hash_in_lds = true;
	}
	a.hash_in_lds = hash_in_lds;
	uint32_t waves = std::max<uint32_t>(2, std::min<uint32_t>(e.search_waves, 16));
	const bool wide_limit = in.limit > 64u * PIPELINED_MAX_REGS;
	const bool can_pipeline = e.search_pipelined && !solo && !in.tomb && !in.list_cap && list_cap_max <= 64;
	const bool wide_list = can_pipeline && e.search_wide_lists && wide_limit;
	if (wide_list)
		waves = std::min<uint32_t>(waves, WIDE_LIST_THREADS / 64);
	a.pipelined = (can_pipeline && (wide_list || !wide_limit)) ? 1u : 0u;
	const bool wide_register_list = !solo && !in.list_cap && wide_limit;
	a.stage_cap = wide_register_list ? 4u : 0u;
	const uint32_t slot_bytes = engine_slot_bytes(a.hash_log2, V, list_cap_max, hash_in_lds, a.stage_cap);
	const uint32_t walkers_cap = std::min<uint32_t>(policy.engine_walkers ? ENGINE_MAX_WALKERS : e.search_walkers_cap, waves - 1);
	uint32_t S = policy.engine_walkers ? policy.engine_walkers : (n + n_cus - 1) / n_cus;
	S = std::max<uint32_t>(1, std::min(S, engine_walkers_that_fit(slot_bytes, walkers_cap)));
	uint32_t walkers_lds = 0;
	a.list_place = candidate_list_placement(e.search_list_lds, in.list_cap, solo, slot_bytes, S, walkers_cap, &walkers_lds);
	const bool list_in_lds = a.list_place == LIST_IN_LDS;
	a.list_lds = list_in_lds ? (uint32_t)in.list_cap : 0u;
	if (list_in_lds)
		S = std::min(S, walkers_lds);
	const auto engine_lds = [&](uint32_t walkers) {
		return engine_lds_bytes(walkers, a.hash_log2, V, list_cap_max, hash_in_lds, a.stage_cap, a.list_lds);
	};
	uint32_t wgs_per_cu = std::max<uint32_t>(1, std::min<uint32_t>(16u / waves, LDS_BYTES_PER_CU / std::max<uint32_t>(1, engine_lds(S))));
	wgs_per_cu = std::min(wgs_per_cu, e.search_wgs_per_cu);
	uint32_t grid = std::min<uint32_t>(n_cus * wgs_per_cu, (n + S - 1) / S);
	const uint32_t solo_lds = wave_lds_bytes(a.hash_log2, V, list_cap_max, a.stage_cap, hash_in_lds);
	if (solo) {
		S = 1;
		grid = std::min<uint32_t>(n, n_cus * std::max<uint32_t>(1, std::min<uint32_t>(8, LDS_BYTES_PER_CU / solo_lds)));
	}
	if (e.retry_in_place && wide_register_list && hash_in_lds) {
		const uint32_t have_log2 = a.visited_compact ? compact_visited::cells_log2_of(a.visited_compact) : a.hash_log2;
		const uint32_t want_log2 = std::min<uint32_t>(17u, e.hash_max_log2);
		if (want_log2 > have_log2)
			a.retry_log2 = want_log2;
	}
	const uint64_t per_walker = (hash_in_lds ? 0 : (4ull << a.hash_log2)) + (list_in_lds ? 0 : 8ull * in.list_cap) +
	                            (in.tomb == 2 ? 8ull * in.cand_cap : 0) + (a.retry_log2 ? (4ull << a.retry_log2) : 0);
	const uint64_t budget = 16ull << 30;
	while (per_walker * grid * S > budget && (grid > 1 || S > 1)) {
		if (S > 1)
			S--;
		else
			grid = (grid + 1) / 2;
	}
	a.walkers = S;
	a.grid = grid;
	const uint64_t resident = (uint64_t)grid * S;
	a.global_hash = hash_in_lds ? 0 : resident << a.hash_log2;
	a.retry_hash = a.retry_log2 ? resident << a.retry_log2 : 0;
	a.list_buf = (in.list_cap && !list_in_lds) ? resident * 2 * in.list_cap : 0;
	a.cand_buf = in.tomb == 2 ? resident * 2 * in.cand_cap : 0;
	a.spec_active = (!in.tomb && !solo && list_cap_max <= 64) ? e.search_spec_active : 0;
	settle_solo_shape(policy, shape, n, e.V, e.G, solo_lds);
	a.team = shape.team;
	a.touch_lines = shape.touch_lines;
	a.crew = shape.crew ? (CREW_ON | ((policy.touch_lists && list_cap_max <= 64) ? CREW_TOUCH : 0u) | e.search_crew_tune) : 0u;
	a.wants_prescore = a.pipelined && !in.direct_io && (e.search_prescore == 2 || !wide_limit);
	a.prescore_descent = (a.wants_prescore && e.search_prescore_descent) ? 1u : 0u;
	a.nch = chunks_per_lane(e.V, e.G, policy.force_looping);
	a.regs = (uint32_t)((in.limit + 63) / 64);
	a.lds_bytes = solo ? solo_lds + (a.team ? TEAM_BOX_BYTES : 0u) : engine_lds(S);
	a.threads = solo ? (a.team ? 64 * VSS_TEAM_WAVES : 64) : 64 * waves;
	const uint32_t words[8] = {a.threads, S, grid, a.lds_bytes, a.list_place, hash_in_lds ? (a.visited_compact ? 1u : 0u) : 2u,
	                           solo ? 1u : 0u, 0u};
	std::copy(words, words + 8, a.shape);
	return a;
}

}
}
```

### duckdb-vss_amd/csrc/prescore_bound.h

```cpp
#pragma once
#include <math.h>
#include <stdint.h>

#if defined(__HIPCC__) || defined(__CUDACC__)
#define VSS_PRESCORE_HD __host__ __device__
#else
#define VSS_PRESCORE_HD
#endif

namespace vss {

struct RowCodeMeta {
	float scale;
	float err;
	float norm;
	uint32_t spare;
};

constexpr float PRESCORE_NO_BOUND = -INFINITY;

VSS_PRESCORE_HD inline double prescore_slack(uint32_t dim) {
	return ((double)dim + 64.0) * (1.0 / 2097152.0);
}

VSS_PRESCORE_HD inline float prescore_round_down(double x) {
	float f = (float)x;
	if ((double)f > x)
		f = nextafterf(f, -INFINITY);
	return f;
}

VSS_PRESCORE_HD inline float prescore_bound(int metric, float t, float s2, const RowCodeMeta &m, float q_norm, uint32_t dim) {
	const double scale = m.scale, E = m.err, rn = m.norm, qn = q_norm;
	if (!(E < (double)INFINITY) || !(scale > 0.0) || !(rn >= 0x1p-40 && rn <= 0x1p40) || !(E <= rn))
		return PRESCORE_NO_BOUND;
	if (metric != 0 && !(qn >= 0x1p-40 && qn <= 0x1p40))
		return PRESCORE_NO_BOUND;
	const double slack = prescore_slack(dim);
	double lb;
	if (metric == 0) {
		if (!(s2 >= 0.f) || !(s2 < INFINITY))
			return PRESCORE_NO_BOUND;
		double root = sqrt((double)s2) * (1.0 - 0.5 * slack) - E - 0x1p-21 * (rn + E);
		if (root < 0.0)
			root = 0.0;
		lb = root * root * (1.0 - slack) - 0x1p-120;
	} else {
		if (!(fabsf(t) < INFINITY))
			return PRESCORE_NO_BOUND;
		const double ub = scale * (double)t + qn * E;
		const double qr = qn * rn;
		if (metric == 1)
			lb = 1.0 - ub / qr - slack;
		else
			lb = 1.0 - ub - slack * qr - 0x1p-22 * (1.0 + qr);
	}
	if (!(lb == lb))
		return PRESCORE_NO_BOUND;
	return prescore_round_down(lb);
}

}
```

### duckdb-vss_amd/csrc/vss_engine.hip

```cpp
#include <hip/hip_runtime.h>

#include <algorithm>
#include <atomic>
#include <chrono>
#include <cmath>
#include <cstdarg>
#include <cstdio>
#include <cstdlib>
#include <cstring>
#include <condition_variable>
#include <mutex>
#include <shared_mutex>
#include <string>
#include <thread>
#include <vector>

#define VSS_ENGINE_TU
#include "../../include/vssgpu.h"
#include "launchers.h"
#include "host_logic.h"
#include "filter_groups.h"
#include "label_filter.h"
#include "exact_filtered_kernels.h"
#include "filter_route_kernels.h"
// ... 475 lines not shown
	bool lists_may_repeat = false;
	KeyMap keymap;
	FreeRing free_slots;
	std::atomic<uint64_t> progress_linked {0}, progress_total {0};
	std::atomic<uint64_t> group_table_bytes {0};

	std::vector<uint32_t> st_slot, st_src;
	std::vector<int64_t> pending_keys;
	uint64_t n_pending = 0;
	DevBuf<float> d_pending;
	DevBuf<uint32_t> d_row_slot, d_row_src, d_parked;

	DevBuf<float> d_vectors;
	DevBuf<uint32_t> d_links0, d_links_up, d_upper_off, d_list_owner;
	DevBuf<uint8_t> d_levels;
	DevBuf<int64_t> d_keys;

	DevBuf<uint32_t> d_labels;
	uint64_t labelled_rows = 0;
	DevBuf<uint32_t> d_more_labels[LABEL_COLUMNS_MAX - 1];
	uint64_t more_labelled_rows[LABEL_COLUMNS_MAX - 1] = {};
	uint64_t label_column_bytes[LABEL_COLUMNS_MAX] = {};
	uint32_t label_width[LABEL_COLUMNS_MAX] = {};
	std::atomic<uint64_t> label_bytes {0};
	DevBuf<uint32_t> &label_cells(uint32_t column) {
		return column ? d_more_labels[column - 1] : d_labels;
	}
	uint64_t &label_rows(uint32_t column) {
		return column ? more_labelled_rows[column - 1] : labelled_rows;
	}

	DevBuf<uint32_t> d_req_list, d_req_src, d_req_rank, d_sorted_src, d_touched, d_list_count, d_list_offset,
	    d_counters;
	DevBuf<float> d_req_d, d_sorted_d;
	uint32_t *h_counters = nullptr;
	DevBuf<uint32_t> d_node_status, d_work_build;
	DevBuf<float> d_build_list;
	uint32_t *h_debug = nullptr;
	DevBuf<unsigned long long> d_work_stats;
	std::vector<uint32_t> h_node_status;

	struct SearchCtx {
		hipStream_t stream = nullptr;
		bool own_stream = false;
		DevBuf<uint32_t> d_stats, d_status, d_work, d_global_hash, d_retry_hash, d_queue;
		DevBuf<float> d_list_buf, d_cand_buf;
		uint32_t cand_cap = 0;
		DevBuf<float> d_q, d_out_d;
		DevBuf<int64_t> d_out_keys;
		DevBuf<uint32_t> d_out_count;
		DevBuf<uint64_t> d_filter;
		DevBuf<uint64_t> d_group_filter;
		DevBuf<uint32_t> d_group_of;
		DevBuf<const unsigned long long *> d_group_bitmap;
		uint64_t group_bytes = 0;
		DevBuf<float> d_route_q, d_route_d;
		DevBuf<int64_t> d_route_keys;
		DevBuf<uint32_t> d_route_group, d_route_count, d_route_map;
		unsigned char *pinned_io = nullptr;
		size_t pinned_cap = 0;
		bool leased = false;
		DevBuf<unsigned long long> d_phase;
		uint32_t *h_status = nullptr, *h_stats = nullptr;
		uint32_t *h_queue = nullptr;
		bool flag_wait = false;
		bool unsynced = false;
		uint32_t flag_target = 0;
		std::chrono::steady_clock::time_point flag_t0;
		uint32_t queue_sel = 0;
		size_t h_cap = 0;
		hipEvent_t ev0 = nullptr, ev1 = nullptr;
		bool pending = false;
		bool direct_io = false;
		SearchArgs args;
		uint64_t nq = 0, limit = 0, list_cap = 0;
		uint32_t bump = 0;
		uint32_t min_hash_log2 = 0;
		uint32_t shape[8] = {0, 0, 0, 0, 0, 0, 0, 0};
		bool first_pass = true;
		double kernel_ms = 0;
		uint64_t stats[4] = {0, 0, 0, 0};
		DevBuf<unsigned long long> d_prescore;
		unsigned long long *h_prescore = nullptr;
		unsigned long long prescore_base[4] = {0, 0, 0, 0};
		bool prescore_first = false, prescore_used = false;
	};
	static constexpr int EXPLICIT_CTX = 4, MAX_CTX = 12;
	SearchCtx ctx[MAX_CTX];
	std::mutex lease_mu;
	std::condition_variable lease_cv;
	void count_group_tables(SearchCtx &c) {
		const uint64_t now = c.d_group_filter.n * 8 + c.d_group_of.n * 4 + c.d_group_bitmap.n * 8;
		group_table_bytes.fetch_add(now - c.group_bytes, std::memory_order_relaxed);
		c.group_bytes = now;
	}
	int lease_context() {
		std::unique_lock<std::mutex> lk(lease_mu);
		for (;;) {
			for (int i = EXPLICIT_CTX; i != MAX_CTX; ++i)
				if (!ctx[i].leased) {
					ctx[i].leased = true;
					return i;
				}
			lease_cv.wait(lk);
		}
	}
	void return_context(int i) {
		{
			std::lock_guard<std::mutex> lk(lease_mu);
			ctx[i].leased = false;
		}
		lease_cv.notify_one();
	}
	std::mutex ctx0_mu;
	std::mutex exact_mu;
	std::mutex route_mu;

	uint32_t search_prescore = 1;
	bool search_prescore_descent = true;
	DevBuf<uint32_t> d_codes;
	DevBuf<RowCodeMeta> d_code_meta;
	StaleSlots codes_stale;
	std::mutex codes_mu;
	uint64_t codes_refused_capacity = 0;
	uint64_t last_prescore[4] = {0, 0, 0, 0};
	uint64_t last_prescore_descent[2] = {0, 0};
	bool codes_wanted() const {
		const uint32_t nch = (G == 64 && V % 64 == 0 && !force_looping) ? V / 64 : 0;
		return search_prescore && (nch == 2 || nch == 3 || nch == 4 || nch == 6);
	}
	void free_codes() {
		d_codes.free(), d_code_meta.free();
		codes_stale.clear();
		codes_refused_capacity = 0;
	}
	bool ensure_codes(hipStream_t s, bool may_allocate) {
		if (!codes_wanted() || !capacity)
			return false;
		std::lock_guard<std::mutex> lk(codes_mu);
		if (d_codes.n < capacity * V || d_code_meta.n < capacity) {
			if (!may_allocate || codes_refused_capacity == capacity)
				return false;
			HIP_TRY(hipStreamSynchronize(s));
			if (!d_codes.try_ensure(capacity * V) || !d_code_meta.try_ensure(capacity)) {
				d_codes.free(), d_code_meta.free();
				codes_refused_capacity = capacity;
				return false;
			}
			codes_stale.mark_all();
		}
		const StaleSlots before = codes_stale;
		uint64_t first = 0, end = 0;
		if (codes_stale.take(count, first, end)) {
			const uint32_t grid = (uint32_t)std::min<uint64_t>((end - first + 3) / 4, (uint64_t)n_cus * 16);
			hipLaunchKernelGGL(k_encode_rows, dim3(grid), dim3(256), 0, s, reinterpret_cast<const float4 *>(d_vectors.p), V, first, end,
			                   d_codes.p, d_code_meta.p);
			hipError_t status = hipGetLastError();
			if (status == hipSuccess)
				status = hipStreamSynchronize(s);
			if (status != hipSuccess) {
				codes_stale = before;
				throw HipError {status, "k_encode_rows"};
			}
		}
		return true;
	}

	void refresh_codes() noexcept {
		try {
			(void)ensure_codes(stream, true);
		} catch (...) {
			(void)hipGetLastError();
		}
	}

	uint64_t last_stats[4] = {0, 0, 0, 0};
	uint32_t last_shape[8] = {0, 0, 0, 0, 0, 0, 0, 0};
	std::vector<uint32_t> last_query_stats;
	double timing[6] = {0, 0, 0, 0, 0, 0};
	hipEvent_t ev[4] = {nullptr, nullptr, nullptr, nullptr};
	void ensure_events() {
		for (auto &e : ev)
			if (!e)
				HIP_TRY(hipEventCreate(&e));
	}

	DevBuf<float> d_row_norm2, d_q_norm2, d_scores, d_best_s, d_qpad, d_cand_s;
	DevBuf<uint32_t> d_best_i, d_cand_cnt, d_cand_i, d_norm_ext, d_certified, d_redo_map;
	uint32_t exact_certify = 1, exact_redo_qt = MS_QT;
	uint64_t last_exact_fallbacks = 0;
	bool exact_filter = true;
	uint64_t norms_valid_for = ~0ull;
	DevBuf<uint32_t> d_xf_lists, d_xf_counts, d_xf_tables;
	uint64_t exact_filter_budget = EXACT_FILTER_LIST_ENTRIES;
	uint64_t last_exact_filtered[4] = {0, 0, 0, 0};
	uint64_t last_filter_route[8] = {0, 0, 0, 0, 0, 0, 0, 0};
	std::atomic<uint64_t> exact_filter_bytes {0};
	uint64_t mutations = 0;

	int fail(const char *fmt, ...) {
		char buf[512];
		va_list ap;
		va_start(ap, fmt);
		vsnprintf(buf, sizeof buf, fmt, ap);
		va_end(ap);
		tls_error = buf;
		return VSS_ERROR;
	}

// ... 294 lines not shown
		const uint64_t nr = reused.size(), first = count + staged;
		const size_t stride = (size_t)V * 4;
		const hipMemcpyKind kind = device_ptrs ? hipMemcpyDeviceToDevice : hipMemcpyHostToDevice;
		auto copy_rows = [&](uint64_t a, uint64_t b, float *dst) {
			if (a == b)
				return;
			if (!sparse) {
				HIP_TRY(hipMemcpy2DAsync(dst, stride * 4, vecs + a * dim, dim * 4, dim * 4, b - a, kind, stream));
				return;
			}
			for (uint64_t i = a; i < b;) {
				uint64_t j = i;
				while (j + 1 < b && rows[j + 1] == rows[j] + 1)
					j++;
				HIP_TRY(hipMemcpy2DAsync(dst + (i - a) * stride, stride * 4, vecs + rows[i] * dim, dim * 4, dim * 4,
				                         j - i + 1, kind, stream));
				i = j + 1;
			}
		};
		if (nr) {
			if (st_slot.empty())
				for (uint64_t i = 0; i != staged; ++i)
					st_slot.push_back((uint32_t)(count + i)), st_src.push_back(EMPTY_SLOT);
			d_pending.ensure((n_pending + nr) * stride, n_pending * stride, stream, 0);
			copy_rows(0, nr, d_pending.p + n_pending * stride);
			for (uint64_t i = 0; i != nr; ++i) {
				st_slot.push_back(reused[i]), st_src.push_back((uint32_t)(n_pending + i));
				pending_keys.push_back(kbuf[i]);
				keys_h[reused[i]] = kbuf[i];
				if (keymap.ready)
					keymap.put(kbuf[i], reused[i]);
			}
			n_pending += nr;
			mutations++;
		}
		int rc = VSS_OK;
		if (nv > nr) {
			copy_rows(nr, nv, d_vectors.p + first * stride);
			codes_stale.mark(first, first + (nv - nr));
			std::memcpy(keys_h.data() + first, kbuf.data() + nr, (nv - nr) * 8);
			if (!st_slot.empty())
				for (uint64_t i = 0; i != nv - nr; ++i)
					st_slot.push_back((uint32_t)(first + i)), st_src.push_back(EMPTY_SLOT);
			rc = stage_metadata(first, nv - nr);
		}
		if (!device_ptrs)
			HIP_TRY(hipStreamSynchronize(stream));
		return rc;
	}

	LaunchCfg launch_cfg(uint32_t grid, uint32_t lds, uint64_t list_limit) const {
		LaunchCfg c;
		c.nch = (V % G == 0 && !force_looping) ? V / G : 0;
		c.regs = (uint32_t)((list_limit + 63) / 64);
		c.grid = grid;
		c.lds = lds;
		c.threads = 64;
		c.stream = stream;
		return c;
	}
	template <typename A>
	void launch_by_metric(hipError_t (*f0)(const A &, const LaunchCfg &), hipError_t (*f1)(const A &, const LaunchCfg &),
	                      hipError_t (*f2)(const A &, const LaunchCfg &), const A &a, const LaunchCfg &c) const {
		HIP_TRY((metric == 0 ? f0 : metric == 1 ? f1 : f2)(a, c));
	}

	uint32_t search_waves = 16, search_walkers = 0;
	uint32_t search_walkers_cap = 4;
	uint32_t search_wgs_per_cu = 1;
	uint32_t search_spec_active = 0;
	uint32_t search_solo = 1, solo_max_queries = 32, solo_max_bytes = 32 * 1024;
	host::SearchEngineConfig search_engine_config() const {
		host::SearchEngineConfig e;
		host::SearchShapePolicy &p = e.policy;
		p.solo_mode = search_solo, p.solo_max_queries = solo_max_queries, p.solo_max_bytes = solo_max_bytes;
		p.team = search_team, p.n_cus = n_cus;
		p.touch_rows = search_touch_rows, p.touch_lists = search_touch_lists, p.touch_max_queries = search_touch_max_queries;
		p.force_looping = force_looping;
		p.crew = search_crew, p.engine_walkers = search_walkers;
		e.M0 = M0, e.V = V, e.G = G, e.list_cap_max = list_cap_max(), e.nodes = count, e.hash_max_log2 = hash_max_log2();
		e.search_waves = search_waves, e.search_walkers_cap = search_walkers_cap, e.search_wgs_per_cu = search_wgs_per_cu;
		e.search_spec_active = search_spec_active, e.search_pipelined = search_pipelined, e.search_wide_lists = search_wide_lists;
		e.search_list_lds = search_list_lds, e.search_prescore = search_prescore, e.search_prescore_descent = search_prescore_descent;
		e.retry_in_place = retry_in_place, e.visited_per_limit = visited_per_limit;
		e.hash_lds_max_log2 = HASH_LDS_MAX_LOG2, e.hash_lds_max_override = hash_lds_max_override;
		e.visited_compact_on = visited_compact_on, e.search_crew_tune = search_crew_tune;
		return e;
	}
	bool search_reg_queue = true;
	uint32_t reg_queue_max_limit = 64 * MAX_LIST_REGS;
	uint32_t n_cus = 256;
	bool force_looping = false;
	uint32_t exact_probe = 0;
	uint32_t exact_kernel = 5;
	uint32_t HASH_LDS_MAX_LOG2 = 13;
	uint32_t BUILD_HASH_LDS_MAX_LOG2 = 11;
	uint32_t hash_max_log2() const {
		return std::max<uint32_t>(10, log2u((count + staged + 2) * 8 / 7 + 64));
	}
	bool retry_in_place = true;
	uint64_t visited_per_limit = 0;
	uint32_t hash_lds_max_override = 0;
	bool visited_compact_on = true;
	uint32_t hash_log2_for(uint64_t limit, uint32_t bump, uint64_t per_limit = 64) const {
		if (visited_per_limit)
			per_limit = visited_per_limit;
		return host::visited_set_log2(limit, bump, M0, list_cap_max(), per_limit, hash_max_log2());
	}
	DevBuf<uint32_t> d_global_hash;
	uint32_t *global_hash_for(uint32_t hash_log2, uint64_t grid) {
		if (hash_log2 <= BUILD_HASH_LDS_MAX_LOG2)
			return nullptr;
		d_global_hash.ensure(grid << hash_log2, 0, stream);
		return d_global_hash.p;
	}

	void ensure_build_scratch(uint64_t batch, uint64_t max_lv) {
		const uint64_t req_cap = batch * M * (max_lv + 1) + 64;
		d_req_list.ensure(req_cap, 0, stream), d_req_src.ensure(req_cap, 0, stream);
		d_req_rank.ensure(req_cap, 0, stream), d_req_d.ensure(req_cap, 0, stream);
		d_sorted_src.ensure(req_cap, 0, stream), d_sorted_d.ensure(req_cap, 0, stream);
		d_touched.ensure(req_cap, 0, stream);
		const uint64_t lists = capacity + d_list_owner.n;
		d_list_count.ensure(lists, 0, stream, 0);
		d_list_offset.ensure(lists, 0, stream, 0);
		d_counters.ensure(8, 0, stream, 0);
		d_work_stats.ensure(4, 0, stream, 0);
		if (!h_counters)
			HIP_TRY(hipHostMalloc((void **)&h_counters, 8 * sizeof(uint32_t), hipHostMallocDefault));
	}

	int build_finalize() {
		if (!staged && !n_pending)
			return VSS_OK;
		if (refuse_while_probing("vss_build_finalize") != VSS_OK)
			return VSS_ERROR;
		const bool reuse = !st_slot.empty();
		lists_may_repeat |= reuse;
		const uint64_t first = count, n = reuse ? st_slot.size() : staged;
		std::vector<uint8_t> lv_rows;
		if (reuse) {
			lv_rows.resize(n);
			for (uint64_t i = 0; i != n; ++i)
				lv_rows[i] = levels_h[st_slot[i]];
			d_row_slot.ensure(n, 0, stream), d_row_src.ensure(n, 0, stream);
			HIP_TRY(hipMemcpyAsync(d_row_slot.p, st_slot.data(), n * 4, hipMemcpyHostToDevice, stream));
			HIP_TRY(hipMemcpyAsync(d_row_src.p, st_src.data(), n * 4, hipMemcpyHostToDevice, stream));
		}
		const uint8_t *lv = reuse ? lv_rows.data() : levels_h.data() + first;
		auto slot_of = [&](uint64_t row) { return reuse ? (uint64_t)st_slot[row] : first + row; };
		uint64_t solo_row = ~0ull;
		for (uint64_t i = 0; reuse && i != n; ++i)
			if (st_src[i] != EMPTY_SLOT && st_slot[i] == entry)
				solo_row = i;
		std::vector<uint64_t> sizes = batch_schedule(first, max_level, lv, n, max_batch, growth_div, solo_row);
		uint64_t biggest = 0, top_lv = 0;
		for (uint64_t b : sizes)
			biggest = std::max(biggest, b);
		for (uint64_t i = 0; i != n; ++i)
			top_lv = std::max<uint64_t>(top_lv, lv[i]);
		ensure_build_scratch(biggest, top_lv);
		uint64_t appended = 0;
		progress_linked.store(0, std::memory_order_relaxed);
		progress_total.store(n, std::memory_order_relaxed);
		uint64_t done = 0;
		int rc = VSS_OK;
// ... 144 lines not shown
				HIP_TRY(hipMemcpyAsync(d_vectors.p + slot * stride, d_pending.p + src * stride, stride * 4,
				                       hipMemcpyDeviceToDevice, stream));
				codes_stale.mark(slot, (uint64_t)slot + 1);
				HIP_TRY(hipMemcpyAsync(d_keys.p + slot, &pending_keys[src], 8, hipMemcpyHostToDevice, stream));
			}
			for (uint64_t j = 0; j != b; ++j) {
				if ((int)lv[done + j] > max_level) {
					max_level = lv[done + j];
					entry = (uint32_t)slot_of(done + j);
				}
			}
			for (uint64_t j = 0; j != b; ++j)
				appended += !reuse || st_src[done + j] == EMPTY_SLOT;
			tombstones -= batch_reused;
			done += b;
			count = first + appended;
			progress_linked.store(done, std::memory_order_relaxed);
		}
		HIP_TRY(hipStreamSynchronize(stream));
		if (pending_b) {
			float ms = 0;
			HIP_TRY(hipEventElapsedTime(&ms, ev[2], ev[3]));
			timing[2] += ms;
		}
		timing[3] += std::chrono::duration<double, std::milli>(std::chrono::steady_clock::now() - wall0).count();
		for (uint64_t i = done; reuse && i < n; ++i) {
			if (st_src[i] == EMPTY_SLOT)
				continue;
			const uint32_t slot = st_slot[i];
			if (keymap.ready)
				keymap.erase(keys_h[slot]);
			keys_h[slot] = VSS_FREE_KEY;
			if (free_slots.reserve(free_slots.size() + 1))
				free_slots.push(slot);
		}
		staged = first + staged - count;
		st_slot.clear(), st_src.clear(), pending_keys.clear();
		n_pending = 0;
		mutations++;
		if (rc == VSS_OK && reorder_after_build && !tombstones && !staged && first == 0)
			rc = compact(true);
		return rc;
	}

	SearchCtx &context(int slot) {
		SearchCtx &c = ctx[slot];
		if (!c.stream) {
			if (slot == 0) {
				c.stream = stream;
			} else {
				HIP_TRY(hipStreamCreateWithFlags(&c.stream, hipStreamNonBlocking));
				c.own_stream = true;
			}
			HIP_TRY(hipEventCreate(&c.ev0));
			HIP_TRY(hipEventCreate(&c.ev1));
			HIP_TRY(hipHostMalloc((void **)&c.h_queue, 16, hipHostMallocCoherent));
		}
		if (slot == 0)
			c.stream = stream;
		return c;
	}

	void launch_search_kernel(SearchCtx &c, uint32_t n) {
		SearchArgs &a = c.args;
		a.n_queries = n;
		host::SearchLaunchInput in;
		in.n = n, in.limit = c.limit, in.bump = c.bump, in.min_hash_log2 = c.min_hash_log2;
		in.list_cap = c.list_cap, in.cand_cap = c.cand_cap, in.tomb = a.tomb, in.direct_io = c.direct_io;
		const host::SearchLaunchPlan plan = host::plan_search_launch(search_engine_config(), in);
		a.hash_log2 = plan.hash_log2, a.visited_compact = plan.visited_compact, a.stage_cap = plan.stage_cap;
		a.list_lds = plan.list_lds, a.walkers = plan.walkers;
		a.spec_active = plan.spec_active, a.touch_lines = plan.touch_lines, a.crew = plan.crew, a.pipelined = plan.pipelined;
		a.prescore = PrescoreView {nullptr, nullptr, nullptr};
		bool codes_ready = false;
		if (plan.wants_prescore) {
			try {
				codes_ready = ensure_codes(c.stream, false);
			} catch (const HipError &) {
				(void)hipGetLastError();
			}
		}
		if (codes_ready) {
			if (!c.d_prescore.p) {
				c.d_prescore.ensure(4, 0, c.stream, 0);
				HIP_TRY(hipHostMalloc((void **)&c.h_prescore, 4 * sizeof(unsigned long long), hipHostMallocDefault));
				for (int i = 0; i < 4; ++i)
					c.h_prescore[i] = 0, c.prescore_base[i] = 0;
			}
			a.prescore = PrescoreView {d_codes.p, d_code_meta.p, c.d_prescore.p};
			c.prescore_used = true;
		}
		a.prescore_descent = a.prescore.codes ? plan.prescore_descent : 0u;
		if (c.first_pass)
			c.prescore_first = a.prescore.codes != nullptr;
		a.global_hash = nullptr;
		if (plan.global_hash) {
			c.d_global_hash.ensure(plan.global_hash, 0, c.stream);
			a.global_hash = c.d_global_hash.p;
		}
		a.retry_hash = nullptr, a.retry_log2 = 0;
		if (plan.retry_hash && c.d_retry_hash.try_ensure(plan.retry_hash))
			a.retry_hash = c.d_retry_hash.p, a.retry_log2 = plan.retry_log2;
		a.list_cap = (uint32_t)c.list_cap;
		a.list_buf = nullptr;
		if (plan.list_buf) {
			c.d_list_buf.ensure(plan.list_buf, 0, c.stream);
			a.list_buf = c.d_list_buf.p;
		}
		a.cand_cap = c.cand_cap;
		a.cand_buf = nullptr;
		if (plan.cand_buf) {
			c.d_cand_buf.ensure(plan.cand_buf, 0, c.stream);
			a.cand_buf = c.d_cand_buf.p;
		}
		if (!c.d_queue.p) {
			c.d_queue.ensure(4 + 64, 0, c.stream);
			HIP_TRY(hipMemsetAsync(c.d_queue.p, 0, (4 + 64) * sizeof(uint32_t), c.stream));
			c.queue_sel = 0;
		}
		a.queue = c.d_queue.p;
		a.queue_sel = c.queue_sel;
		c.queue_sel ^= 2u;
		c.flag_wait = c.direct_io && probe_flag_wait;
		if (c.unsynced && !c.flag_wait) {
			HIP_TRY(hipStreamSynchronize(c.stream));
			c.unsynced = false;
		}
		a.engine_error = c.h_queue + 1;
		if (c.flag_wait) {
			if (!c.unsynced)
				c.h_queue[1] = 0, c.h_queue[3] = 0;
			a.drain_flag = nullptr;
			a.done_count = c.h_queue + 3;
		} else {
			c.h_queue[1] = 0, c.h_queue[2] = 0;
			a.drain_flag = c.h_queue + 2;
			a.done_count = nullptr;
		}
		LaunchCfg cfg;
		cfg.nch = plan.nch, cfg.regs = plan.regs, cfg.grid = plan.grid, cfg.lds = plan.lds_bytes, cfg.threads = plan.threads;
		cfg.stream = c.stream;
		if (c.first_pass) {
			std::memcpy(c.shape, plan.shape, sizeof c.shape);
			c.first_pass = false;
		}
		if (c.flag_wait)
			c.flag_t0 = std::chrono::steady_clock::now();
		else
			HIP_TRY(hipEventRecord(c.ev0, c.stream));
		if (plan.solo)
			launch_by_metric<SearchArgs>(launch_search_solo<0>, launch_search_solo<1>, launch_search_solo<2>, a, cfg);
		else
			launch_by_metric<SearchArgs>(launch_search<0>, launch_search<1>, launch_search<2>, a, cfg);
		if (c.flag_wait)
			c.flag_target = (c.unsynced ? c.flag_target : 0u) + n;
		else
			HIP_TRY(hipEventRecord(c.ev1, c.stream));
		if (!c.direct_io) {
			HIP_TRY(hipMemcpyAsync(c.h_status, c.d_status.p, c.nq * 4, hipMemcpyDeviceToHost, c.stream));
			HIP_TRY(hipMemcpyAsync(c.h_stats, c.d_stats.p, c.nq * 8, hipMemcpyDeviceToHost, c.stream));
		}
		if (a.prescore.codes)
			HIP_TRY(hipMemcpyAsync(c.h_prescore, c.d_prescore.p, 4 * sizeof(unsigned long long), hipMemcpyDeviceToHost, c.stream));
	}

	bool search_gating = true;
	void wait_for_drain_of_previous_launch(int slot);
	bool probe_flag_wait = true;
	bool search_touch_rows = true, search_touch_lists = true;
	uint32_t search_touch_max_queries = 256;
	bool search_team = true;
	bool search_crew = true;
	uint32_t search_crew_tune = 0;
	bool search_pipelined = true;
	bool search_wide_lists = true;
	uint32_t search_list_lds = 1;

	SearchRequest request(int slot, const float *const *d_queries, uint64_t n_batches, uint64_t per_batch, uint64_t k, uint64_t ef,
	                      int64_t *const *d_keys_out, float *const *d_dist_out, uint32_t *const *d_count_out) const {
		return {slot, n_batches, per_batch, d_queries, d_keys_out, d_dist_out, d_count_out, (uint32_t)dim, k, ef};
	}

	int resolve_label_batches(SearchCtx &c, const SearchPredicate &p, uint64_t n_batches, uint64_t per_batch, uint64_t cap_q, GraphView &gv) {
		LabelBatchShape s = {LabelKind::EQ, p.width, 0, (uint32_t)per_batch};
		uint64_t addresses[LABEL_COLUMNS_MAX] = {}, rows = labelled_rows, flags = 0;
		uint32_t wide_mask = 0;
		if (p.kind == SearchPredicate::BY_LABEL || p.kind == SearchPredicate::BY_RANGE || p.kind == SearchPredicate::BY_SET) {
			if (!d_labels.p || label_width[0] == 64 || (p.kind == SearchPredicate::BY_SET && (p.width < 1 || p.width > LABEL_SET_MAX)))
				return fail("search by label: over an index whose 32-bit labels have been set, set width 1 to %u", (unsigned)LABEL_SET_MAX);
			s.kind = p.kind == SearchPredicate::BY_LABEL ? LabelKind::EQ : p.kind == SearchPredicate::BY_RANGE ? LabelKind::RANGE : LabelKind::SET;
			flags = p.kind == SearchPredicate::BY_LABEL ? FILTER_BY_LABEL : p.kind == SearchPredicate::BY_RANGE ? FILTER_BY_RANGE : FILTER_BY_SET;
			addresses[0] = (uint64_t)reinterpret_cast<uintptr_t>(d_labels.p);
		} else {
			LabelBoxColumns box;
			const bool set_box = p.kind == SearchPredicate::BY_SET_BOX;
			if ((p.kind != SearchPredicate::BY_BOX && p.kind != SearchPredicate::BY_BOX64 && !set_box) ||
			    !named_label_columns(p.columns, p.n_columns, box) || (set_box && (p.width < 1 || p.width > LABEL_SET_MAX)))
				return fail("search by label box: over 1 to %u distinct label columns that have been set, set width 1 to %u",
				            (unsigned)LABEL_COLUMNS_MAX, (unsigned)LABEL_SET_MAX);
			wide_mask = box.wide_mask();
			if (p.kind == SearchPredicate::BY_BOX && wide_mask)
				return fail("search by label box: a named column holds 64-bit cells");
			s.kind = set_box ? LabelKind::SET_BOX : p.kind == SearchPredicate::BY_BOX ? LabelKind::BOX : LabelKind::BOX64;
			s.m = set_box ? box.m - 1 : box.m;
			flags = set_box ? FILTER_BY_SET_BOX : p.kind == SearchPredicate::BY_BOX ? FILTER_BY_BOX : FILTER_BY_BOX64;
			for (uint32_t j = 0; j != box.m; ++j)
				addresses[j] = (uint64_t)reinterpret_cast<uintptr_t>(box.cells[j]);
			rows = box.shortest_rows();
		}
		const uint64_t nq = n_batches * per_batch;
		if (!c.d_group_bitmap.try_grow(label_batches_table_cells(s, cap_q)))
			return fail("search by label: no device memory for the predicates of %llu queries", (unsigned long long)cap_q);
		count_group_tables(c);
		unsigned long long *table = reinterpret_cast<unsigned long long *>(c.d_group_bitmap.p);
		const LabelTableHead head = label_batches_table_head(s, addresses, wide_mask);
		const dim3 grid((uint32_t)(nq * label_batches_query_units(s) / 256 + 1));
		if (s.kind == LabelKind::BOX64 || s.kind == LabelKind::SET_BOX) {
			ResolveLabelBatchesArgs<uint64_t> res = {{}, s, head, (uint32_t)nq, table};
			for (uint64_t b = 0; b != n_batches; ++b)
				res.batch[b] = {static_cast<const uint64_t *>(p.label_words[b].words), static_cast<const uint64_t *>(p.label_words[b].lo),
				                static_cast<const uint64_t *>(p.label_words[b].hi)};
			hipLaunchKernelGGL(k_resolve_label_batches64, grid, dim3(256), 0, c.stream, res);
		} else {
			ResolveLabelBatchesArgs<uint32_t> res = {{}, s, head, (uint32_t)nq, table};
			for (uint64_t b = 0; b != n_batches; ++b)
				res.batch[b] = {static_cast<const uint32_t *>(p.label_words[b].words), static_cast<const uint32_t *>(p.label_words[b].lo),
				                static_cast<const uint32_t *>(p.label_words[b].hi)};
			hipLaunchKernelGGL(k_resolve_label_batches, grid, dim3(256), 0, c.stream, res);
		}
		HIP_TRY(hipGetLastError());
		gv.filter = table;
		const uint64_t cut = p.kind == SearchPredicate::BY_LABEL ? FILTER_BY_LABEL : p.kind == SearchPredicate::BY_RANGE ? FILTER_BY_RANGE : FILTER_BY_SET;
		gv.filter_bits = std::min<uint64_t>(rows, cut - 1) | FILTER_PER_QUERY | flags;
		return VSS_OK;
	}

	int search_begin(const SearchRequest &r) {
		const int slot = r.slot;
		const uint64_t n_batches = r.n_batches, per_batch = r.per_batch, k = r.k;
		uint64_t ef = r.ef;
		if (slot < 0 || slot >= MAX_CTX)
			return fail("search context %d out of range (0..%d)", slot, MAX_CTX - 1);
		if (n_batches < 1 || n_batches > MAX_COALESCED)
			return fail("1 to %d batches per launch", MAX_COALESCED);
		SearchCtx &c = context(slot);
		if (c.pending)
// ... 226 lines not shown
				HIP_TRY(hipStreamSynchronize(c.stream));
				c.unsynced = false;
			}
			if (!c.nq)
				break;
			if (!c.flag_wait) {
				float ms = 0;
				HIP_TRY(hipEventElapsedTime(&ms, c.ev0, c.ev1));
				c.kernel_ms += ms;
			}
			if (c.h_queue[1])
				return fail("search engine: a walking wave gave up waiting for its scoring waves (internal error)");
#ifdef VSS_PARANOID
			{
				const uint32_t *note = h_debug;
				if (note[0])
					return fail("paranoid: %u bad chunks; first: c %u n %u id %u block %u wave %u ticket {n %u next %u} cnt %u last id %u",
					            note[0], note[1], note[2], note[3], note[4], note[5], note[6], note[7], note[8], note[9]);
			}
#endif
			work.clear();
			bool visited_full = false, queue_full = false;
			for (uint64_t i = 0; i != c.nq; ++i) {
				if (!c.h_status[i])
					continue;
				if (c.h_status[i] == LEVEL_OK_RETRIED) {
					c.h_status[i] = LEVEL_OK;
					if (rounds == 0)
						c.stats[3] += 1;
					continue;
				}
				if (c.h_status[i] > LEVEL_QUEUE_OVERFLOW)
					return fail("search engine: query %llu was not processed (status %u; internal error)", (unsigned long long)i,
					            c.h_status[i]);
				work.push_back((uint32_t)i);
				visited_full |= c.h_status[i] == LEVEL_VISITED_OVERFLOW;
				queue_full |= c.h_status[i] == LEVEL_QUEUE_OVERFLOW;
			}
			if (work.empty())
				break;
			if ((visited_full && c.args.hash_log2 >= hash_max_log2()) ||
			    (queue_full && c.args.tomb == 2 && c.cand_cap >= count + 1))
				return fail("search scratch overflow although sized for the whole index");
			if (++rounds > 64)
				return fail("search engine: scratch retries do not converge (internal error)");
			if (visited_full) {
				c.bump += 2;
				c.min_hash_log2 = std::max(c.args.hash_log2, c.args.retry_log2) + 1;
			}
			if (queue_full) {
				if (c.args.tomb == 1)
					c.args.tomb = 2;
				else
					c.cand_cap = (uint32_t)std::min<uint64_t>(count + 1, (uint64_t)c.cand_cap * 8);
			}
			c.stats[3] += work.size();
			c.d_work.ensure(c.nq, 0, c.stream);
			HIP_TRY(hipMemcpyAsync(c.d_work.p, work.data(), work.size() * 4, hipMemcpyHostToDevice, c.stream));
			HIP_TRY(hipStreamSynchronize(c.stream));
			c.args.work = c.d_work.p;
			launch_search_kernel(c, (uint32_t)work.size());
		}
		for (uint64_t i = 0; i != c.nq; ++i) {
			c.stats[0] += c.h_stats[2 * i];
			c.stats[1] += c.h_stats[2 * i + 1];
		}
		{
			std::lock_guard<std::mutex> lk(stats_mu);
			std::memcpy(last_stats, c.stats, sizeof last_stats);
			std::memcpy(last_shape, c.shape, sizeof last_shape);
			last_prescore[0] = c.prescore_first ? 1 : 0;
			last_prescore[1] = last_prescore[2] = 0;
			if (c.prescore_used) {
				last_prescore[1] = c.h_prescore[0] - c.prescore_base[0];
				last_prescore[2] = c.h_prescore[1] - c.prescore_base[1];
				c.prescore_base[0] = c.h_prescore[0], c.prescore_base[1] = c.h_prescore[1];
			}
			last_prescore_descent[0] = last_prescore_descent[1] = 0;
			if (c.prescore_used) {
				last_prescore_descent[0] = c.h_prescore[2] - c.prescore_base[2];
				last_prescore_descent[1] = c.h_prescore[3] - c.prescore_base[3];
				c.prescore_base[2] = c.h_prescore[2], c.prescore_base[3] = c.h_prescore[3];
			}
			last_prescore[3] = d_codes.n * sizeof(uint32_t) + d_code_meta.n * sizeof(RowCodeMeta);
			timing[0] = c.kernel_ms;
			if (keep_query_stats)
				last_query_stats.assign(c.h_stats, c.h_stats + 2 * c.nq);
		}
		return VSS_OK;
	}

	int search_launch(const SearchRequest &r) {
		std::unique_lock<std::mutex> lk0(ctx0_mu, std::defer_lock);
		if (r.slot == 0)
			lk0.lock();
		int rc = search_begin(r);
		if (rc != VSS_OK)
			return rc;
		return search_end(r.slot, r.keep_query_stats);
	}

	struct Lease {
		vss_index *ix;
		int slot;
		explicit Lease(vss_index *i) : ix(i), slot(i->lease_context()) {
		}
		~Lease() {
			ix->ctx[slot].pending = false;
			ix->return_context(slot);
		}
	};

	int stage_group_table(SearchCtx &c, const FilterGroupBatch &table, uint64_t n_bits, uint64_t nq) {
		const uint64_t words = table.n_groups * filter_group_words(n_bits);
		if (!c.d_group_filter.try_grow(std::max<uint64_t>(words, 1)) || (table.group_of && !c.d_group_of.try_grow(nq)))
			return fail("filtered search: no device memory for %llu bitmaps of %llu bits and the groups of %llu queries",
			            (unsigned long long)table.n_groups, (unsigned long long)n_bits, (unsigned long long)nq);
		count_group_tables(c);
		if (words)
			HIP_TRY(hipMemcpyAsync(c.d_group_filter.p, table.allowed, words * 8, hipMemcpyHostToDevice, c.stream));
		if (table.group_of)
			HIP_TRY(hipMemcpyAsync(c.d_group_of.p, table.group_of, nq * 4, hipMemcpyHostToDevice, c.stream));
		return VSS_OK;
	}
	int stage_wanted_labels(SearchCtx &c, const uint32_t *want, uint64_t nq) {
		if (!c.d_group_of.try_grow(nq))
			return fail("search by label: no device memory for the wanted labels of %llu queries", (unsigned long long)nq);
		count_group_tables(c);
		HIP_TRY(hipMemcpyAsync(c.d_group_of.p, want, nq * 4, hipMemcpyHostToDevice, c.stream));
		return VSS_OK;
	}
	int stage_label_ranges(SearchCtx &c, const uint32_t *lo, const uint32_t *hi, uint64_t nq) {
		if (!c.d_group_of.try_grow(2 * nq))
			return fail("search by label range: no device memory for the ranges of %llu queries", (unsigned long long)nq);
		count_group_tables(c);
		HIP_TRY(hipMemcpyAsync(c.d_group_of.p, lo, nq * 4, hipMemcpyHostToDevice, c.stream));
		HIP_TRY(hipMemcpyAsync(c.d_group_of.p + nq, hi, nq * 4, hipMemcpyHostToDevice, c.stream));
		return VSS_OK;
	}
	int stage_label_sets(SearchCtx &c, const uint32_t *sets, uint32_t width, uint64_t nq) {
		if (!c.d_group_of.try_grow(nq * width))
			return fail("search by label set: no device memory for the sets of %llu queries", (unsigned long long)nq);
		count_group_tables(c);
		HIP_TRY(hipMemcpyAsync(c.d_group_of.p, sets, nq * width * 4, hipMemcpyHostToDevice, c.stream));
		return VSS_OK;
	}
	int stage_label_boxes(SearchCtx &c, const uint32_t *boxes, uint32_t m, uint64_t nq, uint32_t end_words = 1) {
		if (!c.d_group_of.try_grow(nq * 2 * m * end_words))
			return fail("search by label box: no device memory for the boxes of %llu queries", (unsigned long long)nq);
		count_group_tables(c);
		HIP_TRY(hipMemcpyAsync(c.d_group_of.p, boxes, nq * 2 * m * end_words * 4, hipMemcpyHostToDevice, c.stream));
		return VSS_OK;
	}
	int stage_label_set_boxes(SearchCtx &c, const uint32_t *rows, uint32_t row_words, uint64_t nq) {
		if (!c.d_group_of.try_grow(nq * row_words))
			return fail("search by label set box: no device memory for the predicates of %llu queries", (unsigned long long)nq);
		count_group_tables(c);
		HIP_TRY(hipMemcpyAsync(c.d_group_of.p, rows, nq * row_words * 4, hipMemcpyHostToDevice, c.stream));
		return VSS_OK;
	}
	void stage_queries(SearchCtx &c, const float *queries, uint64_t nq, uint64_t k) {
		c.d_q.ensure(nq * dim, 0, c.stream), c.d_out_count.ensure(nq, 0, c.stream);
		c.d_out_keys.ensure(nq * k, 0, c.stream), c.d_out_d.ensure(nq * k, 0, c.stream);
		HIP_TRY(hipMemcpyAsync(c.d_q.p, queries, nq * dim * 4, hipMemcpyHostToDevice, c.stream));
	}
	void fetch_results(SearchCtx &c, uint64_t nq, uint64_t k, int64_t *out_keys, float *out_d, uint32_t *out_counts) {
// ... 463 lines not shown
				hipLaunchKernelGGL(k_exact_select_lists, dim3(pass.query_end - pass.query_begin), dim3(SEL_THREADS), 0, stream, s);
			}
		}
		RerankArgs r;
		r.gv = view();
		r.queries = b.d_queries;
		r.q_stride = b.q_stride;
		r.n_queries = (uint32_t)nq;
		r.k = (uint32_t)k;
		r.KP = (uint32_t)KP;
		r.best_i = d_best_i.p;
		r.out_keys = out.keys;
		r.out_d = out.dist;
		r.out_count = out.count;
		r.best_s = nullptr, r.norm_ext = nullptr, r.certified = nullptr;
		r.query_map = d_xf_tables.p + at_order;
		const uint32_t lds = align16(V * 16) + 2 * align16((uint32_t)KP * 4);
		launch_by_metric<RerankArgs>(launch_rerank<0>, launch_rerank<1>, launch_rerank<2>, r, launch_cfg((uint32_t)nq, lds, 64));
		HIP_TRY(hipGetLastError());
		HIP_TRY(hipEventRecord(ev[1], stream));
		HIP_TRY(hipStreamSynchronize(stream));
		float ms = 0;
		HIP_TRY(hipEventElapsedTime(&ms, ev[0], ev[1]));
		{
			std::lock_guard<std::mutex> lk(stats_mu);
			timing[0] = ms;
		}
		return VSS_OK;
	}

	int exact_filtered_host(const HostCall &hc, const uint64_t *allowed, uint64_t n_groups, uint64_t n_bits, const uint32_t *group_of) {
		return staged_call(
		    hc, true, [&](SearchCtx &c) { return stage_group_table(c, FilterGroupBatch {allowed, nullptr, n_groups}, n_bits, hc.nq); },
		    [&](SearchCtx &c, const DeviceBatch &b, const DeviceAnswers &out, std::vector<uint8_t> &) {
			    return exact_filtered_launch(
			        b, GroupedRows::bitmaps(c.d_group_filter.p, n_groups, n_bits, HostWords(group_of), DeviceWords(nullptr)), out);
		    });
	}

	int filtered_auto(const DeviceBatch &b, const GroupedRows &g, uint64_t route_c, const DeviceAnswers &out, std::vector<uint8_t> &route) {
		const uint64_t nq = b.nq, k = b.k;
		const uint64_t limit = filter_route_limit(k, b.ef, efs), C = route_c ? route_c : FILTER_ROUTE_C, L = count - tombstones;
		SearchCtx &c = context(b.slot);
		FilterRoutePlan rp;
		{
			std::lock_guard<std::mutex> exact_lock(exact_mu);
			last_exact_fallbacks = 0;
			std::fill(last_exact_filtered, last_exact_filtered + 4, 0);
			std::fill(last_filter_route, last_filter_route + 8, 0);
			ExactFilterPlan all;
			exact_filter_order(g.group_of, nq, g.n_groups, all);
			std::vector<uint32_t> lengths;
			if (const int rc = exact_filtered_count(all, nq, 2, g, lengths))
				return rc;
			filter_route_partition(all, lengths.data(), g.group_of, nq, L, limit, C, route_c ? 0 : FILTER_ROUTE_MIN_WALK, rp);
			const uint64_t nu = all.groups.size(), nx = rp.exact.groups.size();
			if (!rp.exact.order.empty()) {
				uint32_t *taken_counts = nx == nu ? nullptr : d_xf_counts.p;
				const uint32_t n_blocks = (uint32_t)((count + FL_WAVE_SLOTS - 1) / FL_WAVE_SLOTS);
				if (nx != nu && n_blocks) {
					taken_counts = d_xf_counts.p + nu * n_blocks;
					uint32_t *d_rows = d_xf_tables.p + ExactFilterTables(nu, nq, g.group_cells()).at_totals;
					HIP_TRY(hipMemcpyAsync(d_rows, rp.exact_rows.data(), nx * 4, hipMemcpyHostToDevice, stream));
					const dim3 grid(std::min<uint32_t>((n_blocks + 255) / 256, 64), (uint32_t)std::min<uint64_t>(nx, 65535));
					hipLaunchKernelGGL(k_route_take_rows, grid, dim3(256), 0, stream, d_xf_counts.p, d_rows, (uint32_t)nx, n_blocks,
					                   taken_counts);
					HIP_TRY(hipStreamSynchronize(stream));
				}
				if (const int rc = exact_filtered_score(rp.exact, rp.exact_lengths, taken_counts, b, g, out))
					return rc;
			}
			last_filter_route[0] = rp.graph_queries.size(), last_filter_route[1] = rp.exact.order.size();
			last_filter_route[2] = rp.n_graph_groups, last_filter_route[3] = rp.n_exact_groups;
			last_filter_route[4] = L, last_filter_route[5] = C, last_filter_route[6] = limit;
		}
		route = rp.route;
		const uint64_t ng = rp.graph_queries.size(), n_unknown = rp.unknown_queries.size();
		if (!ng) {
			std::lock_guard<std::mutex> lk(stats_mu);
			std::fill(last_stats, last_stats + 4, 0);
			std::fill(last_shape, last_shape + 8, 0);
			std::fill(last_prescore, last_prescore + 4, 0);
			last_prescore_descent[0] = last_prescore_descent[1] = 0;
		}
		if (!ng && !n_unknown)
			return VSS_OK;
		std::unique_lock<std::mutex> route_lock(route_mu, std::defer_lock);
		if (b.slot == 0)
			route_lock.lock();
		if (!c.d_route_map.try_grow(ng + n_unknown) || !c.d_route_q.try_grow(std::max<uint64_t>(ng * dim, 1)) ||
		    !c.d_route_group.try_grow(std::max<uint64_t>(ng * g.group_cells(), 1)) || !c.d_route_keys.try_grow(std::max<uint64_t>(ng * k, 1)) ||
		    !c.d_route_d.try_grow(std::max<uint64_t>(ng * k, 1)) || !c.d_route_count.try_grow(std::max<uint64_t>(ng, 1)))
			return fail("routed filtered search: no device memory for a compact batch of %llu queries", (unsigned long long)ng);
		if (n_unknown) {
			HIP_TRY(hipMemcpyAsync(c.d_route_map.p + ng, rp.unknown_queries.data(), n_unknown * 4, hipMemcpyHostToDevice, c.stream));
			hipLaunchKernelGGL(k_route_blank, dim3((uint32_t)((n_unknown + 3) / 4)), dim3(256), 0, c.stream, c.d_route_map.p + ng,
			                   (uint32_t)n_unknown, (uint32_t)k, out.keys, out.dist, out.count);
		}
		if (ng) {
			HIP_TRY(hipMemcpyAsync(c.d_route_map.p, rp.graph_queries.data(), ng * 4, hipMemcpyHostToDevice, c.stream));
			RouteGatherArgs ga;
			ga.queries = b.d_queries, ga.group_of = g.d_group_of, ga.map = c.d_route_map.p;
			ga.n = (uint32_t)ng, ga.q_stride = (uint32_t)dim;
			ga.vec4 = dim % 4 == 0 && reinterpret_cast<uintptr_t>(b.d_queries) % 16 == 0 && reinterpret_cast<uintptr_t>(c.d_route_q.p) % 16 == 0;
			ga.out_queries = c.d_route_q.p, ga.out_group_of = c.d_route_group.p;
			hipLaunchKernelGGL(k_route_gather, dim3((uint32_t)((ng + 3) / 4)), dim3(256), 0, c.stream, ga);
			if (const GroupedRows::WalkWords w = g.more_walk_words(ng); w.words) {
				const dim3 grid((uint32_t)((ng * w.per + 255) / 256));
				void (*const column)(const uint32_t *, const uint32_t *, uint32_t, uint32_t *) = k_route_gather_words;
				void (*const matrix)(const uint32_t *, const uint32_t *, uint32_t, uint32_t, uint32_t *) = k_route_gather_words;
				if (w.per == 1)
					hipLaunchKernelGGL(column, grid, dim3(256), 0, c.stream, w.words, c.d_route_map.p, (uint32_t)ng, c.d_route_group.p + w.at);
				else
					hipLaunchKernelGGL(matrix, grid, dim3(256), 0, c.stream, w.words, c.d_route_map.p, (uint32_t)ng, w.per,
					                   c.d_route_group.p + w.at);
			}
			HIP_TRY(hipGetLastError());
			SearchRequest r = request(b.slot, &c.d_route_q.p, 1, ng, k, b.ef, &c.d_route_keys.p, &c.d_route_d.p, &c.d_route_count.p);
			r.predicate = g.walk_predicate(c.d_route_group.p, ng);
			if (const int rc = search_launch(r))
				return rc;
			RouteScatterArgs s;
			s.map = c.d_route_map.p, s.n = (uint32_t)ng, s.k = (uint32_t)k;
			s.keys = c.d_route_keys.p, s.dist = c.d_route_d.p, s.count = c.d_route_count.p;
			s.out_keys = out.keys, s.out_dist = out.dist, s.out_count = out.count;
			hipLaunchKernelGGL(k_route_scatter, dim3((uint32_t)((ng + 3) / 4)), dim3(256), 0, c.stream, s);
		}
		HIP_TRY(hipGetLastError());
		HIP_TRY(hipStreamSynchronize(c.stream));
		return VSS_OK;
	}

	int filtered_auto_host(const HostCall &hc, const uint64_t *allowed, uint64_t n_groups, uint64_t n_bits, const uint32_t *group_of,
	                       uint64_t route_c) {
		return staged_call(
		    hc, true, [&](SearchCtx &c) { return stage_group_table(c, FilterGroupBatch {allowed, group_of, n_groups}, n_bits, hc.nq); },
		    [&](SearchCtx &c, const DeviceBatch &b, const DeviceAnswers &out, std::vector<uint8_t> &route) {
			    const DeviceWords d_group_of(group_of ? c.d_group_of.p : nullptr);
			    return filtered_auto(b, GroupedRows::bitmaps(c.d_group_filter.p, n_groups, n_bits, HostWords(group_of), d_group_of), route_c,
			                         out, route);
		    });
	}

	int by_label_launch(const DeviceBatch &b, HostWords want, DeviceWords d_want, uint64_t route_c, const DeviceAnswers &out,
	                    std::vector<uint8_t> &route) {
		std::vector<uint32_t> values, group_of;
		label_groups(want.p, b.nq, values, group_of);
		const GroupedRows g = GroupedRows::labels(values, d_labels.p, labelled_rows, HostWords(group_of.data()), d_want);
		if (!d_want.p) {
			route.assign(b.nq, FILTER_ROUTE_EXACT);
			return exact_filtered_launch(b, g, out);
		}
		return filtered_auto(b, g, route_c, out, route);
	}

	int by_label_host(const HostCall &hc, bool exact, const uint32_t *want, uint64_t route_c) {
		return staged_call(
		    hc, true, [&](SearchCtx &c) { return exact ? (int)VSS_OK : stage_wanted_labels(c, want, hc.nq); },
		    [&](SearchCtx &c, const DeviceBatch &b, const DeviceAnswers &out, std::vector<uint8_t> &route) {
			    return by_label_launch(b, HostWords(want), DeviceWords(exact ? nullptr : c.d_group_of.p), route_c, out, route);
		    });
	}

	int by_range_launch(const DeviceBatch &b, HostWords lo, HostWords hi, DeviceWords d_lo, DeviceWords d_hi, uint64_t route_c,
	                    const DeviceAnswers &out, std::vector<uint8_t> &route) {
		std::vector<LabelRange> pairs;
// ... 661 lines not shown
	}
	count = live;
	n_upper = nup;
	tombstones = 0;
	free_slots.clear();
	max_level = live ? nml : -1;
	entry = nentry;
	keymap = KeyMap();
	mutations++;
	return VSS_OK;
}

#define VSS_GUARD_WITH(LOCK, index, ...)                                                                               \
	if (!(index))                                                                                                      \
		return VSS_ERROR;                                                                                              \
	LOCK _lk((index)->rw);                                                                                             \
	try {                                                                                                              \
		(void)hipSetDevice((index)->device);                                                                           \
		__VA_ARGS__                                                                                                    \
	} catch (const HipError &e) {                                                                                      \
		return (index)->fail("HIP error %d (%s) in %s", (int)e.code, hipGetErrorString(e.code), e.what);               \
	} catch (const std::exception &e) {                                                                                \
		return (index)->fail("%s", e.what());                                                                          \
	}
#define VSS_GUARD(index, ...) VSS_GUARD_WITH(std::unique_lock<std::shared_mutex>, index, __VA_ARGS__)
#define VSS_SHARED(index, ...) VSS_GUARD_WITH(std::shared_lock<std::shared_mutex>, index, __VA_ARGS__)

namespace {
struct OptionRule {
	const char *name;
	int64_t lo, hi;
	void (*apply)(vss_index *, int64_t);
	const char *what;
};
const OptionRule OPTION_RULES[] = {
    {"search.waves", 2, 16, [](vss_index *h, int64_t v) { h->search_waves = (uint32_t)v; },
     "wavefronts per workgroup of the search engine"},
    {"search.walkers", 0, ENGINE_MAX_WALKERS, [](vss_index *h, int64_t v) { h->search_walkers = (uint32_t)v; },
     "walking waves among them (0 = chosen per launch); at least one scoring wave must remain"},
    {"search.solo", 0, 2, [](vss_index *h, int64_t v) { h->search_solo = (uint32_t)v; },
     "the one-wave-per-query shape: 0 never, 1 automatic, 2 always"},
    {"search.solo_max_queries", 1, 1 << 30, [](vss_index *h, int64_t v) { h->solo_max_queries = (uint32_t)v; },
     "largest launch the automatic rule gives the solo shape"},
    {"search.team", 0, 1, [](vss_index *h, int64_t v) { h->search_team = v != 0; }, "eight-wave teams in the solo shape"},
    {"search.crew", 0, 31,
     [](vss_index *h, int64_t v) {
	     h->search_crew = (v & 1) != 0;
	     if (v & 16)
		     h->search_crew_tune = (uint32_t)v & (CREW_SPARE_SIMD | CREW_NO_REQUESTS);
     },
     "the last walker of a workgroup runs its scoring waves as a crew (1 | 16 | refinement bits 4, 8)"},
    {"search.pipelined", 0, 1, [](vss_index *h, int64_t v) { h->search_pipelined = v != 0; }, "software-pipelined level search"},
    {"search.wide_lists", 0, 1, [](vss_index *h, int64_t v) { h->search_wide_lists = v != 0; },
     "limits of 257-512 in 12-wave workgroups with the pipelined level search"},
    {"search.visited_compact", 0, 1, [](vss_index *h, int64_t v) { h->visited_compact_on = v != 0; },
     "compact exact visited sets (16-bit cells) in LDS at limits of 257-512"},
    {"search.visited_lds_log2_max", 0, 14, [](vss_index *h, int64_t v) { h->hash_lds_max_override = (uint32_t)v; },
     "largest visited-set table (log2 of its 32-bit cells) kept in LDS with several walkers per workgroup; 0 = the engine's own "
     "(13); 1 = every such table in HBM"},
    {"search.visited_cells_per_limit", 0, 1 << 20, [](vss_index *h, int64_t v) { h->visited_per_limit = (uint64_t)v; },
     "visited-set cells per entry of the search limit; 0 = the sizing rule's own, else at least 4"},
    {"search.retry_in_place", 0, 1, [](vss_index *h, int64_t v) { h->retry_in_place = v != 0; },
     "a query that outgrows its LDS-resident visited set is repeated by its walker within the launch"},
    {"search.probe_flag_wait", 0, 1, [](vss_index *h, int64_t v) { h->probe_flag_wait = v != 0; },
     "host-pointer probes of at most 256 queries wait on a pinned flag instead of the stream"},
    {"search.lookahead", 0, ENGINE_MAX_WALKERS, [](vss_index *h, int64_t v) { h->search_spec_active = (uint32_t)v; },
     "one expansion of look-ahead while at most this many walkers of a workgroup still run (0 = off)"},
    {"search.gating", 0, 1, [](vss_index *h, int64_t v) { h->search_gating = v != 0; },
     "a launch is issued when its predecessor on the device starts to drain"},
    {"search.list_lds", 0, 2, [](vss_index *h, int64_t v) { h->search_list_lds = (uint32_t)v; },
     "candidate lists of limits 513-4096 in LDS: 0 never (HBM), 1 when the workgroup keeps its walkers, 2 whenever one walker fits"},
    {"search.prescore", 0, 2,
     [](vss_index *h, int64_t v) {
	     h->search_prescore = (uint32_t)v;
	     if (!h->search_prescore)
		     h->free_codes();
	     else if (h->stream)
		     h->refresh_codes();
     },
     "scoring waves reject rows on exact bounds from 8-bit row codes before reading their f32 components: 0 never, 1 at limits of "
     "at most 256, 2 in every pipelined launch"},
    {"search.prescore_descent", 0, 1, [](vss_index *h, int64_t v) { h->search_prescore_descent = v != 0; },
     "in launches that filter on row codes, the greedy descent's rows are bounded against its closest distance too"},
};
const char *set_option_checked(vss_index *h, const char *name, int64_t value) {
	for (const OptionRule &r : OPTION_RULES) {
		if (std::strcmp(r.name, name))
			continue;
		if (value < r.lo || value > r.hi)
			return "value out of range";
		if (!std::strcmp(name, "search.visited_cells_per_limit") && value != 0 && value < 4)
			return "value out of range";
		const uint32_t waves = !std::strcmp(name, "search.waves") ? (uint32_t)value : h->search_waves;
		const uint32_t walkers = !std::strcmp(name, "search.walkers") ? (uint32_t)value : h->search_walkers;
		if (walkers && walkers >= waves)
			return "at least one scoring wave must remain";
		r.apply(h, value);
		return nullptr;
	}
	return "no such option";
}
}

extern "C" {

const char *vss_version(void) {
	return "vssgpu 0.1 (gfx950, wave64)";
}

int vss_create(uint64_t dim, int metric, uint64_t M, uint64_t M0, uint64_t efc, uint64_t efs, int device,
               vss_index **out) {
	if (!out)
		return VSS_ERROR;
	*out = nullptr;
	int n_dev = 0;
	if (hipGetDeviceCount(&n_dev) != hipSuccess || n_dev <= device || device < 0) {
		fprintf(stderr, "vssgpu: no HIP device %d available (found %d) — the engine has no CPU fallback\n", device,
		        n_dev);
		return VSS_ERROR;
	}
	if (!dim || metric < 0 || metric > 2 || M < 2 || M0 < 2)
		return VSS_ERROR;
	if (M0 < M) {
		fprintf(stderr, "vssgpu: M0 (%llu) must not be smaller than M (%llu)\n", (unsigned long long)M0,
		        (unsigned long long)M);
		return VSS_ERROR;
	}
	auto *h = new vss_index();
	h->device = device;
	h->configure(dim, metric, M, M0);
	h->efc = efc ? efc : 128;
	h->efs = efs ? efs : 64;
	if (hipSetDevice(device) != hipSuccess || hipStreamCreateWithFlags(&h->stream, hipStreamNonBlocking) != hipSuccess) {
		delete h;
		return VSS_ERROR;
	}
	h->own_stream = true;
#ifdef VSS_PARANOID
	if (hipHostMalloc((void **)&h->h_debug, 128 * sizeof(uint32_t), hipHostMallocDefault) != hipSuccess) {
		vss_destroy(h);
		return VSS_ERROR;
	}
	std::memset(h->h_debug, 0, 128 * sizeof(uint32_t));
#endif
	hipDeviceProp_t prop;
	if (hipGetDeviceProperties(&prop, device) == hipSuccess && prop.multiProcessorCount > 0)
		h->n_cus = (uint32_t)prop.multiProcessorCount;
	static const struct { const char *env, *option; } ENV_OPTIONS[] = {
	    {"VSS_SEARCH_WAVES", "search.waves"}, {"VSS_SEARCH_WALKERS", "search.walkers"}, {"VSS_SEARCH_SPEC", "search.lookahead"},
	    {"VSS_SEARCH_SOLO", "search.solo"}, {"VSS_SEARCH_SOLO_MAX", "search.solo_max_queries"}, {"VSS_SEARCH_TEAM", "search.team"},
	    {"VSS_SEARCH_CREW", "search.crew"}, {"VSS_SEARCH_PIPELINED", "search.pipelined"},
	    {"VSS_SEARCH_WIDE_LISTS", "search.wide_lists"}, {"VSS_VISITED_COMPACT", "search.visited_compact"},
	    {"VSS_SEARCH_RETRY_IN_PLACE", "search.retry_in_place"}, {"VSS_HASH_LDS_MAX_LOG2", "search.visited_lds_log2_max"},
	    {"VSS_VISITED_PER_LIMIT", "search.visited_cells_per_limit"}, {"VSS_PROBE_FLAG_WAIT", "search.probe_flag_wait"},
	    {"VSS_SEARCH_LIST_LDS", "search.list_lds"}, {"VSS_SEARCH_PRESCORE", "search.prescore"},
	    {"VSS_SEARCH_PRESCORE_DESCENT", "search.prescore_descent"},
	};
	for (const auto &e : ENV_OPTIONS)
		if (const char *t = getenv(e.env)) {
			if (const char *why = set_option_checked(h, e.option, (int64_t)atoll(t)))
				fprintf(stderr, "vssgpu: %s=%s ignored (%s: %s)\n", e.env, t, e.option, why);
		}
	if (const char *t = getenv("VSS_SEARCH_REG_QUEUE"))
		h->search_reg_queue = atoi(t) != 0;
	if (const char *t = getenv("VSS_SEARCH_REG_QUEUE_MAX"))
		h->reg_queue_max_limit = (uint32_t)std::max(0, std::min(64 * MAX_LIST_REGS, atoi(t)));
	if (const char *t = getenv("VSS_FORCE_LOOPING"))
		h->force_looping = atoi(t) != 0;
	if (const char *t = getenv("VSS_EXACT_PROBE"))
		h->exact_probe = (uint32_t)atoi(t);
	if (const char *t = getenv("VSS_EXACT_KERNEL"))
		h->exact_kernel = (uint32_t)std::max(1, std::min(5, atoi(t)));
	if (const char *t = getenv("VSS_SEARCH_WGS_PER_CU"))
		h->search_wgs_per_cu = (uint32_t)std::max(1, std::min(8, atoi(t)));
	if (const char *t = getenv("VSS_SEARCH_WALKERS_CAP"))
		h->search_walkers_cap = (uint32_t)std::max(1, std::min((int)ENGINE_MAX_WALKERS, atoi(t)));
	if (const char *t = getenv("VSS_EXACT_FILTER"))
		h->exact_filter = atoi(t) != 0;
	if (const char *t = getenv("VSS_EXACT_CERTIFY"))
		h->exact_certify = (uint32_t)std::max(1, std::min(2, atoi(t)));
	if (const char *t = getenv("VSS_EXACT_REDO_QT"))
		h->exact_redo_qt = (uint32_t)std::max(1, std::min(MS_QT, atoi(t)));
	if (const char *t = getenv("VSS_EXACT_FILTER_LIST_ENTRIES")) {
		const long long v = atoll(t);
		if (v < (long long)EXACT_FILTER_LIST_ENTRIES_MIN || v > (long long)EXACT_FILTER_LIST_ENTRIES_MAX)
			fprintf(stderr, "vssgpu: VSS_EXACT_FILTER_LIST_ENTRIES=%s ignored (%llu .. %llu list entries per pass)\n", t,
			        (unsigned long long)EXACT_FILTER_LIST_ENTRIES_MIN, (unsigned long long)EXACT_FILTER_LIST_ENTRIES_MAX);
		else
			h->exact_filter_budget = (uint64_t)v;
	}
	if (const char *t = getenv("VSS_SEARCH_CREW_TUNE"))
		h->search_crew_tune = (uint32_t)atoi(t) & (CREW_SPARE_SIMD | CREW_NO_REQUESTS);
	if (const char *t = getenv("VSS_SEARCH_TOUCH_LISTS"))
		h->search_touch_lists = atoi(t) != 0;
	if (const char *t = getenv("VSS_SEARCH_TOUCH_ROWS"))
		h->search_touch_rows = atoi(t) != 0;
	if (const char *t = getenv("VSS_SEARCH_TOUCH_MAX"))
		h->search_touch_max_queries = (uint32_t)std::max(0, atoi(t));
	*out = h;
	return VSS_OK;
}

void vss_destroy(vss_index *h) {
	if (!h)
		return;
	(void)hipSetDevice(h->device);
	{
		DeviceGate &dg = g_gate[(unsigned)h->device % 64];
		std::lock_guard<std::mutex> lk(dg.mu);
		if (dg.last.owner == h)
			dg.last = GateEntry();
	}
	if (h->stream)
		(void)hipStreamSynchronize(h->stream);
	h->release();
	if (h->own_stream && h->stream)
		(void)hipStreamDestroy(h->stream);
	delete h;
}

const char *vss_last_error(vss_index *h) {
	return h ? tls_error.c_str() : "null index";
}

int vss_set_stream(vss_index *h, void *s) {
	VSS_GUARD(h, {
		HIP_TRY(hipStreamSynchronize(h->stream));
		if (s) {
			if (h->own_stream)
				(void)hipStreamDestroy(h->stream);
			h->stream = (hipStream_t)s;
			h->own_stream = false;
		} else if (!h->own_stream) {
			HIP_TRY(hipStreamCreateWithFlags(&h->stream, hipStreamNonBlocking));
			h->own_stream = true;
		}
		return VSS_OK;
	})
}
// ... 908 lines not shown
	LabelBoxColumns box;
	SearchPredicate::LabelWords words[MAX_FILTER_GROUP_BATCHES] = {};
	for (uint64_t b = 0; b != n_batches; ++b) {
		const vss_label_predicate &p = preds[b];
		char what[96];
		if (multi)
			std::snprintf(what, sizeof what, "%s: batch %llu", entry, (unsigned long long)b);
		else
			std::snprintf(what, sizeof what, "%s", entry);
		const int graph = VSS_BY_LABEL_GRAPH;
		int rc = VSS_OK;
		if (p.kind == VSS_LABEL_EQ)
			rc = check_by_label(h, what, Q[b], per_batch, static_cast<const uint32_t *>(p.d_want), graph, out[b], out_counts[b]);
		else if (p.kind == VSS_LABEL_RANGE)
			rc = check_by_label_range(h, what, Q[b], per_batch, static_cast<const uint32_t *>(p.d_lo), static_cast<const uint32_t *>(p.d_hi),
			                          graph, out[b], out_counts[b]);
		else if (p.kind == VSS_LABEL_SET)
			rc = check_by_label_set(h, what, Q[b], per_batch, static_cast<const uint32_t *>(p.d_sets), p.set_width, graph, out[b], out_counts[b]);
		else if (p.kind == VSS_LABEL_SET_BOX)
			rc = check_by_label_set_box(h, what, Q[b], per_batch, p.set_column, p.d_sets, p.set_width, p.columns, p.n_columns, p.d_lo, p.d_hi,
			                            graph, out[b], out_counts[b], box);
		else
			rc = check_by_label_box(h, what, Q[b], per_batch, p.columns, p.n_columns, p.d_lo, p.d_hi, graph, out[b], out_counts[b], box,
			                        p.kind == VSS_LABEL_BOX64);
		if (rc != VSS_OK)
			return rc;
		words[b] = {p.kind == VSS_LABEL_EQ ? p.d_want : p.d_sets, p.d_lo, p.d_hi};
	}
	if (per_batch && k) {
		if (p0.kind == VSS_LABEL_EQ)
			r.predicate = SearchPredicate::by_label(nullptr, h->labelled_rows).with_batches(words);
		else if (p0.kind == VSS_LABEL_RANGE)
			r.predicate = SearchPredicate::by_range(nullptr, nullptr, h->labelled_rows).with_batches(words);
		else if (p0.kind == VSS_LABEL_SET)
			r.predicate = SearchPredicate::by_set(nullptr, p0.set_width, h->labelled_rows).with_batches(words);
		else if (p0.kind == VSS_LABEL_BOX)
			r.predicate = SearchPredicate::by_box(nullptr, box.columns, box.m, box.shortest_rows()).with_batches(words);
		else if (p0.kind == VSS_LABEL_BOX64)
			r.predicate = SearchPredicate::by_box64(nullptr, box.columns, box.m, box.shortest_rows()).with_batches(words);
		else
			r.predicate = SearchPredicate::by_set_box(nullptr, p0.set_width, box.columns, box.m, box.shortest_rows()).with_batches(words);
	}
	return h->search_begin(r);
}

int vss_search_by_label_device_begin(vss_index *h, int context, const float *Q, uint64_t nq, uint64_t k, uint64_t ef,
                                     const vss_label_predicate *predicate, int64_t *out, float *out_d, uint32_t *out_counts) {
	VSS_SHARED(h, { return label_begin(h, "vss_search_by_label_device_begin", false, context, 1, &Q, nq, k, ef, predicate, &out, &out_d, &out_counts); })
}

int vss_search_multi_by_label_device_begin(vss_index *h, int context, uint64_t n_batches, const float *const *Q, uint64_t per_batch,
                                           uint64_t k, uint64_t ef, const vss_label_predicate *preds, int64_t *const *out,
                                           float *const *out_d, uint32_t *const *out_counts) {
	VSS_SHARED(h, {
		return label_begin(h, "vss_search_multi_by_label_device_begin", true, context, n_batches, Q, per_batch, k, ef, preds, out, out_d,
		                   out_counts);
	})
}

int vss_last_search_stats(vss_index *h, uint64_t *out4) {
	VSS_SHARED(h, {
		std::lock_guard<std::mutex> lk(h->stats_mu);
		std::memcpy(out4, h->last_stats, sizeof h->last_stats);
		return VSS_OK;
	})
}

int vss_last_search_prescore(vss_index *h, uint64_t *out4) {
	VSS_SHARED(h, {
		std::lock_guard<std::mutex> lk(h->stats_mu);
		std::memcpy(out4, h->last_prescore, sizeof h->last_prescore);
		return VSS_OK;
	})
}

int vss_last_search_prescore_descent(vss_index *h, uint64_t *out2) {
	VSS_SHARED(h, {
		std::lock_guard<std::mutex> lk(h->stats_mu);
		std::memcpy(out2, h->last_prescore_descent, sizeof h->last_prescore_descent);
		return VSS_OK;
	})
}

uint64_t vss_last_exact_fallbacks(vss_index *h) {
	if (!h)
		return 0;
	std::lock_guard<std::mutex> lk(h->exact_mu);
	return h->last_exact_fallbacks;
}

int vss_last_search_shape(vss_index *h, uint32_t *out8) {
	VSS_SHARED(h, {
		std::lock_guard<std::mutex> lk(h->stats_mu);
		std::memcpy(out8, h->last_shape, sizeof h->last_shape);
		return VSS_OK;
	})
}

#ifdef VSS_PHASE_TIMERS
int vss_debug_phase_ticks(vss_index *h, unsigned long long *out, uint64_t nq) {
	VSS_SHARED(h, {
		if (!h->ctx[0].d_phase.p || h->ctx[0].d_phase.n < nq * VSS_PHASE_STRIDE)
			return h->fail("no phase ticks recorded for %llu queries", (unsigned long long)nq);
		HIP_TRY(hipMemcpy(out, h->ctx[0].d_phase.p, nq * VSS_PHASE_STRIDE * 8, hipMemcpyDeviceToHost));
		return VSS_OK;
	})
}
#endif

int vss_build_work(vss_index *h, uint64_t *out3) {
	VSS_SHARED(h, {
		std::memset(out3, 0, 3 * sizeof(uint64_t));
		if (h->d_work_stats.p) {
			HIP_TRY(hipStreamSynchronize(h->stream));
			unsigned long long v[4];
			HIP_TRY(hipMemcpy(v, h->d_work_stats.p, sizeof v, hipMemcpyDeviceToHost));
			out3[0] = v[0];
			out3[1] = v[1];
			out3[2] = v[2];
		}
		return VSS_OK;
	})
}

int vss_timing(vss_index *h, double *out6, int reset) {
	VSS_SHARED(h, {
		std::lock_guard<std::mutex> lk(h->stats_mu);
		std::memcpy(out6, h->timing, sizeof h->timing);
		if (reset)
			std::memset(h->timing, 0, sizeof h->timing);
		return VSS_OK;
	})
}

int vss_last_search_query_stats(vss_index *h, uint32_t *out, uint64_t nq) {
	VSS_SHARED(h, {
		std::lock_guard<std::mutex> lk(h->stats_mu);
		if (h->last_query_stats.size() < nq * 2)
			return h->fail("no per-query stats recorded for %llu queries", (unsigned long long)nq);
		std::memcpy(out, h->last_query_stats.data(), nq * 8);
		return VSS_OK;
	})
}

int vss_remove_batch(vss_index *h, const int64_t *rowids, uint64_t n, uint64_t *removed) {
	VSS_GUARD(h, { return h->remove(rowids, n, removed); })
}

int vss_compact(vss_index *h) {
	VSS_GUARD(h, {
		const int rc = h->compact(true);
		if (rc == VSS_OK)
			h->refresh_codes();
		return rc;
	})
}

int vss_compact_ex(vss_index *h, int reorder, int *out_reordered) {
	VSS_GUARD(h, {
		const int rc = h->compact(reorder != 0);
		if (rc == VSS_OK)
			h->refresh_codes();
		if (out_reordered)
			*out_reordered = rc == VSS_OK && h->last_compact_reordered ? 1 : 0;
		return rc;
	})
// ... 195 lines not shown
```

### include/vssgpu.h

```cpp
#ifndef VSSGPU_H
#define VSSGPU_H
#include <stdint.h>
#ifdef __cplusplus
extern "C" {
#endif

typedef struct vss_index vss_index;

enum { VSS_OK = 0, VSS_ERROR = 1 };

enum { VSS_METRIC_L2SQ = 0, VSS_METRIC_COSINE = 1, VSS_METRIC_IP = 2 };

enum { VSS_FN_ARRAY_DISTANCE = 0, VSS_FN_ARRAY_COSINE_DISTANCE = 1, VSS_FN_ARRAY_NEGATIVE_INNER_PRODUCT = 2 };

#define VSS_FREE_KEY INT64_MAX


int vss_create(uint64_t dim, int metric, uint64_t M, uint64_t M0, uint64_t ef_construction, uint64_t ef_search,
               int device, vss_index **out);
void vss_destroy(vss_index *index);
const char *vss_last_error(vss_index *index);
int vss_set_stream(vss_index *index, void *hip_stream);
int vss_synchronize(vss_index *index);

// ... 76 lines not shown
int vss_search_batch_by_label_set_device(vss_index *index, const float *d_queries, uint64_t n_queries, uint64_t k, uint64_t ef,
                                         const uint32_t *d_sets, uint64_t width, int mode, uint64_t route_c,
                                         int64_t *d_out_rowids, float *d_out_distances, uint32_t *d_out_counts,
                                         uint8_t *d_out_route);
#define VSS_LABEL_COLUMNS_MAX 4
int vss_set_label_column(vss_index *index, uint32_t column, uint64_t first_rowid, const uint32_t *labels, uint64_t n);
int vss_set_label_column_device(vss_index *index, uint32_t column, uint64_t first_rowid, const uint32_t *d_labels, uint64_t n);
int vss_clear_label_column(vss_index *index, uint32_t column);
uint64_t vss_label_column_rows(const vss_index *index, uint32_t column);
int vss_search_batch_by_label_box(vss_index *index, const float *queries, uint64_t n_queries, uint64_t k, uint64_t ef,
                                  const uint32_t *columns, uint64_t n_columns, const uint32_t *lo, const uint32_t *hi, int mode,
                                  uint64_t route_c, int64_t *out_rowids, float *out_distances, uint32_t *out_counts,
                                  uint8_t *out_route);
int vss_search_batch_by_label_box_device(vss_index *index, const float *d_queries, uint64_t n_queries, uint64_t k, uint64_t ef,
                                         const uint32_t *columns, uint64_t n_columns, const uint32_t *d_lo, const uint32_t *d_hi,
                                         int mode, uint64_t route_c, int64_t *d_out_rowids, float *d_out_distances,
                                         uint32_t *d_out_counts, uint8_t *d_out_route);
#define VSS_NO_LABEL64 0xFFFFFFFFFFFFFFFFull
int vss_set_label_column64(vss_index *index, uint32_t column, uint64_t first_rowid, const uint64_t *labels, uint64_t n);
int vss_set_label_column64_device(vss_index *index, uint32_t column, uint64_t first_rowid, const uint64_t *d_labels, uint64_t n);
uint32_t vss_label_column_width(const vss_index *index, uint32_t column);
int vss_search_batch_by_label_box64(vss_index *index, const float *queries, uint64_t n_queries, uint64_t k, uint64_t ef,
                                    const uint32_t *columns, uint64_t n_columns, const uint64_t *lo, const uint64_t *hi, int mode,
                                    uint64_t route_c, int64_t *out_rowids, float *out_distances, uint32_t *out_counts,
                                    uint8_t *out_route);
int vss_search_batch_by_label_box64_device(vss_index *index, const float *d_queries, uint64_t n_queries, uint64_t k, uint64_t ef,
                                           const uint32_t *columns, uint64_t n_columns, const uint64_t *d_lo, const uint64_t *d_hi,
                                           int mode, uint64_t route_c, int64_t *d_out_rowids, float *d_out_distances,
                                           uint32_t *d_out_counts, uint8_t *d_out_route);
int vss_search_batch_by_label_set_box(vss_index *index, const float *queries, uint64_t n_queries, uint64_t k, uint64_t ef,
                                      uint32_t set_column, const uint64_t *sets, uint32_t set_width, const uint32_t *columns,
                                      uint64_t n_columns, const uint64_t *lo, const uint64_t *hi, int mode, uint64_t route_c,
                                      int64_t *out_rowids, float *out_distances, uint32_t *out_counts, uint8_t *out_route);
int vss_search_batch_by_label_set_box_device(vss_index *index, const float *d_queries, uint64_t n_queries, uint64_t k, uint64_t ef,
                                             uint32_t set_column, const uint64_t *d_sets, uint32_t set_width, const uint32_t *columns,
                                             uint64_t n_columns, const uint64_t *d_lo, const uint64_t *d_hi, int mode,
                                             uint64_t route_c, int64_t *d_out_rowids, float *d_out_distances,
                                             uint32_t *d_out_counts, uint8_t *d_out_route);
int vss_search_batch_device_begin(vss_index *index, int context, const float *d_queries, uint64_t n_queries, uint64_t k,
                                  uint64_t ef, int64_t *d_out_rowids, float *d_out_distances, uint32_t *d_out_counts);
int vss_search_multi_device_begin(vss_index *index, int context, uint64_t n_batches, const float *const *d_queries,
                                  uint64_t n_per_batch, uint64_t k, uint64_t ef, int64_t *const *d_out_rowids,
                                  float *const *d_out_distances, uint32_t *const *d_out_counts);
int vss_search_batch_filtered_device_begin(vss_index *index, int context, const float *d_queries, uint64_t n_queries,
                                           uint64_t k, uint64_t ef, const uint64_t *d_allowed, uint64_t n_bits,
                                           int64_t *d_out_rowids, float *d_out_distances, uint32_t *d_out_counts);
int vss_search_batch_filtered_groups_device_begin(vss_index *index, int context, const float *d_queries, uint64_t n_queries,
                                                  uint64_t k, uint64_t ef, const uint64_t *d_allowed, uint64_t n_groups,
                                                  uint64_t n_bits, const uint32_t *d_group_of, int64_t *d_out_rowids,
                                                  float *d_out_distances, uint32_t *d_out_counts);
int vss_search_multi_filtered_device_begin(vss_index *index, int context, uint64_t n_batches, const float *const *d_queries,
                                           uint64_t n_per_batch, uint64_t k, uint64_t ef, const uint64_t *const *d_allowed,
                                           const uint64_t *n_groups, uint64_t n_bits, const uint32_t *const *d_group_of,
                                           int64_t *const *d_out_rowids, float *const *d_out_distances,
                                           uint32_t *const *d_out_counts);
enum { VSS_LABEL_EQ = 0, VSS_LABEL_RANGE = 1, VSS_LABEL_SET = 2, VSS_LABEL_BOX = 3, VSS_LABEL_BOX64 = 4, VSS_LABEL_SET_BOX = 5 };
typedef struct vss_label_predicate {
	int kind;
	uint32_t set_column;
	uint32_t set_width;
	uint32_t n_columns;
	uint32_t columns[4];
	const void *d_want;
	const void *d_sets;
	const void *d_lo, *d_hi;
} vss_label_predicate;
int vss_search_by_label_device_begin(vss_index *index, int context, const float *d_queries, uint64_t n_queries, uint64_t k,
                                     uint64_t ef, const vss_label_predicate *predicate, int64_t *d_out_rowids,
                                     float *d_out_distances, uint32_t *d_out_counts);
int vss_search_multi_by_label_device_begin(vss_index *index, int context, uint64_t n_batches, const float *const *d_queries,
                                           uint64_t n_per_batch, uint64_t k, uint64_t ef, const vss_label_predicate *predicates,
                                           int64_t *const *d_out_rowids, float *const *d_out_distances,
                                           uint32_t *const *d_out_counts);
int vss_search_batch_end(vss_index *index, int context);
int vss_search_exact_batch(vss_index *index, const float *queries, uint64_t n_queries, uint64_t k,
                           int64_t *out_rowids, float *out_distances, uint32_t *out_counts);
int vss_search_exact_batch_device(vss_index *index, const float *d_queries, uint64_t n_queries, uint64_t k,
                                  int64_t *d_out_rowids, float *d_out_distances, uint32_t *d_out_counts);
uint64_t vss_last_exact_fallbacks(vss_index *index);
int vss_last_search_stats(vss_index *index, uint64_t *out4);
int vss_last_search_shape(vss_index *index, uint32_t *out8);
int vss_last_search_prescore(vss_index *index, uint64_t *out4);
int vss_last_search_prescore_descent(vss_index *index, uint64_t *out2);
int vss_timing(vss_index *index, double *out6, int reset);
int vss_build_work(vss_index *index, uint64_t *out3);
int vss_last_search_query_stats(vss_index *index, uint32_t *out, uint64_t n_queries);


int vss_remove_batch(vss_index *index, const int64_t *rowids, uint64_t count, uint64_t *out_removed);
int vss_compact(vss_index *index);
int vss_compact_ex(vss_index *index, int reorder, int *out_reordered);

uint64_t vss_size(vss_index *index);
uint64_t vss_nodes(vss_index *index);
uint64_t vss_capacity(vss_index *index);
uint64_t vss_max_level(vss_index *index);
uint64_t vss_memory_usage(vss_index *index);
uint64_t vss_dimensions(vss_index *index);
int vss_metric(vss_index *index);
int vss_level_stats(vss_index *index, uint64_t level, uint64_t *out4);
int vss_build_progress(vss_index *index, uint64_t *linked, uint64_t *total);


typedef int (*vss_write_cb)(void *ctx, const void *data, uint64_t size);
typedef int (*vss_read_cb)(void *ctx, void *data, uint64_t size);
uint64_t vss_serialized_length(vss_index *index);
int vss_save(vss_index *index, vss_write_cb write, void *ctx);
int vss_load(vss_index *index, vss_read_cb read, void *ctx);


int vss_distance_batch(int fn, const float *a, const float *b, int b_is_constant, uint64_t rows, uint64_t dim,
                       float *out, int device);
int vss_distance_batch_device(int fn, const float *d_a, const float *d_b, int b_is_constant, uint64_t rows,
                              uint64_t dim, float *d_out, void *hip_stream);


int vss_merge_topk_device(const float *d_in_distances, const int64_t *d_in_rowids, uint64_t n_shards,
                          uint64_t n_queries, uint64_t k, float *d_out_distances, int64_t *d_out_rowids,
                          uint32_t *d_out_counts, void *hip_stream);

uint64_t vss_packed_block_bytes(uint64_t n_queries, uint64_t k);
int vss_merge_topk_packed_device(const void *d_packed, uint64_t n_shards, uint64_t n_queries, uint64_t k,
                                 float *d_out_distances, int64_t *d_out_rowids, uint32_t *d_out_counts, void *hip_stream);

typedef struct vss_comm vss_comm;
int vss_exchange_available(void);
const char *vss_exchange_last_error(void);
int vss_exchange_unique_id(void *id128);
int vss_exchange_init_rank(vss_comm **out, int n_ranks, const void *id128, int rank, int device);
int vss_exchange_init_all(vss_comm **out, int n, const int *devices);
int vss_exchange_adopt(vss_comm **out, void *nccl_comm, int n_ranks, int rank);
int vss_exchange_ranks(vss_comm *comm);
int vss_exchange_allgather(vss_comm *comm, const void *d_local_block, void *d_gathered, uint64_t block_bytes, void *hip_stream);
int vss_exchange_group_begin(void);
int vss_exchange_group_end(void);
int vss_exchange_destroy(vss_comm *comm);

const char *vss_version(void);

#ifdef __cplusplus
}
#endif
#endif
```

Measured before the change: 1.702 million.

## Prefetch likely successors' neighbour lists into L2 from prescoring waves

In pipelined launches that prescore with int8 row codes, scoring waves now pick up to four rows whose estimated distance beats the current bound and a walker-supplied hint. While their full-vector loads are in flight, they issue loads of those rows' neighbour lists at the current level so the walker finds them in L2. The mailbox now carries the level and hint, the feature is on by default behind a new option, and touch counters are exposed. The cost is extra memory traffic, register pressure and a switch from wave sync to LDS sync, and the prefetches may be wasted if the guessed successor is not the one expanded.

```diff
diff --git a/duckdb-vss_amd/__init__.py b/duckdb-vss_amd/__init__.py
--- a/duckdb-vss_amd/__init__.py
+++ b/duckdb-vss_amd/__init__.py
@@ -120,6 +120,7 @@
     "vss_last_search_shape": (_int, [_vp, _vp]),
     "vss_last_search_prescore": (_int, [_vp, _vp]),
     "vss_last_search_prescore_descent": (_int, [_vp, _vp]),
+    "vss_last_search_touches": (_int, [_vp, _vp]),
     "vss_last_search_query_stats": (_int, [_vp, _vp, _u64]),
     "vss_timing": (_int, [_vp, _vp, _int]),
     "vss_build_work": (_int, [_vp, _vp]),
@@ -737,6 +738,11 @@
         self._check(self.lib.vss_last_search_prescore_descent(self.h, _p(out)))
         return out
 
+    def last_search_touches(self):
+        out = np.zeros(4, dtype=np.uint64)
+        self._check(self.lib.vss_last_search_touches(self.h, _p(out)))
+        return out
+
     def last_exact_fallbacks(self):
         return int(self.lib.vss_last_exact_fallbacks(self.h))
 
diff --git a/duckdb-vss_amd/csrc/hnsw_kernels.h b/duckdb-vss_amd/csrc/hnsw_kernels.h
--- a/duckdb-vss_amd/csrc/hnsw_kernels.h
+++ b/duckdb-vss_amd/csrc/hnsw_kernels.h
@@ -206,11 +206,15 @@
 	uint32_t touch_lines = 0;
 	uint32_t *spill_box = nullptr;
 	uint32_t query = 0;
+#ifdef VSS_PHASE_TIMERS
+	uint32_t t_list_wait = 0;
+#endif
 };
 
 struct WorkCounters {
 	uint32_t distances;
 	uint32_t cycles;
+	uint32_t pipelined, fresh;
 #ifdef VSS_PHASE_TIMERS
 	uint32_t t_pick, t_gather, t_dist, t_accept, t_descend, t_total;
 	uint32_t t_sync1, t_look, t_slice, t_sync2, t_team_passes, t_solo_passes;
@@ -264,6 +268,13 @@
 			id = first;
 		else
 			id = (off + lane < cap) ? lp[off + lane] : EMPTY_SLOT;
+#ifdef VSS_PHASE_TIMERS
+		if (FILTER) {
+			const unsigned long long tl0 = __builtin_readcyclecounter();
+			asm volatile("s_waitcnt vmcnt(0)" : "+v"(id));
+			lds.t_list_wait += (uint32_t)(__builtin_readcyclecounter() - tl0);
+		}
+#endif
 		bool take = id != EMPTY_SLOT;
 		if (FILTER) {
 			take = mark_first_visit(lds.visited, id, take, gv.twins != 0, bad);
@@ -527,124 +538,6 @@
 #ifndef VSS_SCORER_IDLE_SLEEP
 #define VSS_SCORER_IDLE_SLEEP 2
 #endif
-struct Mailbox {
-	unsigned long long ticket;
-	uint32_t done;
-	uint32_t qa2_bits;
-	uint32_t slots;
-	uint32_t bound_bits;
-	uint32_t pad[2];
-};
-
-struct PrescoreView {
-	const uint32_t *codes;
-	const RowCodeMeta *meta;
-	unsigned long long *counters;
-};
-constexpr uint32_t PRESCORE_SLOTS = 16;
-__host__ __device__ constexpr int prescore_claim_rows(int R) {
-	return 4 * R;
-}
-__device__ __forceinline__ float code_to_float(uint32_t w, int k) {
-	return (float)(int)(int8_t)(w >> (8 * k));
-}
-template <int MT, int NCH, int CR>
-__device__ __forceinline__ unsigned long long prescore_codes(const RowSpace &sp, const PrescoreView &pv, uint32_t dim,
-                                                             const float4 *q_lds, float qa2, const uint32_t *ids, int n,
-                                                             float bound, float *out, uint32_t &rejected) {
-	static_assert(NCH >= 2, "full-wave rows only");
-	const uint32_t lane = lane_id();
-	constexpr int PER = 64 / CR;
-	uint32_t w[NCH][CR];
-	float sc[CR];
-#pragma unroll
-	for (int r = 0; r < CR; ++r) {
-		const uint32_t id = ids[r < n ? r : n - 1];
-		const uint32_t *crow = pv.codes + (size_t)id * sp.V;
-#pragma unroll
-		for (int ch = 0; ch < NCH; ++ch)
-			w[ch][r] = crow[lane + ch * 64];
-		sc[r] = MT == 0 ? pv.meta[id].scale : 0.f;
-	}
-	const int jm = (int)(lane / PER) < n ? (int)(lane / PER) : n - 1;
-	const float4 mraw = *reinterpret_cast<const float4 *>(pv.meta + ids[jm]);
-	__builtin_amdgcn_sched_barrier(0);
-	float t[CR];
-#pragma unroll
-	for (int r = 0; r < CR; ++r)
-		t[r] = 0.f;
-#pragma unroll
-	for (int ch = 0; ch < NCH; ++ch) {
-		const float4 q = q_lds[lane + ch * 64];
-		const float qs[4] = {q.x, q.y, q.z, q.w};
-#pragma unroll
-		for (int r = 0; r < CR; ++r)
-#pragma unroll
-			for (int k = 0; k < 4; ++k) {
-				const float c = code_to_float(w[ch][r], k);
-				if (MT == 0) {
-					const float v = __fmaf_rn(-sc[r], c, qs[k]);
-					t[r] = __fmaf_rn(v, v, t[r]);
-				} else {
-					t[r] = __fmaf_rn(qs[k], c, t[r]);
-				}
-			}
-	}
-	transposed_reduce64<CR>(t);
-	RowCodeMeta m;
-	m.scale = mraw.x, m.err = mraw.y, m.norm = mraw.z, m.spare = 0;
-	const float lb = prescore_bound(MT, t[0], t[0], m, MT == 0 ? 1.f : vss_sqrt(qa2), dim);
-	const bool mine = (lane % PER) == 0 && (int)(lane / PER) < n;
-	const bool rej = mine && lb >= bound;
-	if (rej)
-		out[lane / PER] = __builtin_inff();
-	rejected += (uint32_t)__popcll(__ballot(rej));
-	return __ballot(mine && !rej);
-}
-template <int MT, int NCH, int RR>
-__device__ __forceinline__ void wave_distances_picked(const RowSpace &sp, const float4 *q_lds, float qa2, const uint32_t *ids,
-                                                      unsigned long long &left, int lane_shift, float *out) {
-	const uint32_t lane = lane_id();
-	int pos[RR], last = 0;
-	const float4 *row[RR];
-#pragma unroll
-	for (int r = 0; r < RR; ++r) {
-		if (left)
-			last = (int)(__builtin_ctzll(left) >> lane_shift);
-		pos[r] = last;
-		left &= left - 1ull;
-		row[r] = sp.vectors + (size_t)ids[pos[r]] * sp.V;
-	}
-	float4 x[NCH][RR];
-#pragma unroll
-	for (int ch = 0; ch < NCH; ++ch)
-#pragma unroll
-		for (int r = 0; r < RR; ++r)
-			x[ch][r] = row[r][lane + ch * 64];
-	float ab[RR], b2[RR];
-#pragma unroll
-	for (int r = 0; r < RR; ++r)
-		ab[r] = 0.f, b2[r] = 0.f;
-#pragma unroll
-	for (int ch = 0; ch < NCH; ++ch) {
-		const float4 q = q_lds[lane + ch * 64];
-#pragma unroll
-		for (int r = 0; r < RR; ++r)
-			accumulate4<MT>(q, x[ch][r], ab[r], b2[r]);
-	}
-	transposed_reduce64<RR>(ab);
-	if (MT == 1)
-		transposed_reduce64<RR>(b2);
-	constexpr int PER = 64 / RR;
-	int j = pos[0];
-#pragma unroll
-	for (int r = 1; r < RR; ++r)
-		j = (int)(lane / PER) == r ? pos[r] : j;
-	if ((lane % PER) == 0)
-		out[j] = finish_distance<MT>(ab[0], qa2, b2[0]);
-}
-
-
 typedef __attribute__((address_space(3))) unsigned long long lds_u64;
 typedef __attribute__((address_space(3))) uint32_t lds_u32;
 typedef __attribute__((address_space(3))) float lds_f32;
@@ -665,17 +558,178 @@
 #define VSS_LDS_STORE_REL(type, ptr, v) __hip_atomic_store(VSS_LDS_PTR(type, ptr), (v), VSS_MB_RELEASE, __HIP_MEMORY_SCOPE_WORKGROUP)
 #define VSS_LDS_ADD_ACQ(type, ptr, v) __hip_atomic_fetch_add(VSS_LDS_PTR(type, ptr), (v), VSS_MB_ACQUIRE, __HIP_MEMORY_SCOPE_WORKGROUP)
 #define VSS_LDS_ADD_REL(type, ptr, v) __hip_atomic_fetch_add(VSS_LDS_PTR(type, ptr), (v), VSS_MB_RELEASE, __HIP_MEMORY_SCOPE_WORKGROUP)
-
+struct Mailbox {
+	unsigned long long ticket;
+	uint32_t done;
+	uint32_t qa2_bits;
+	uint32_t slots;
+	uint32_t bound_bits;
+	uint32_t touch_bits;
+	uint32_t level;
+};
+
+struct PrescoreView {
+	const uint32_t *codes;
+	const RowCodeMeta *meta;
+	unsigned long long *counters;
+};
+constexpr uint32_t PRESCORE_SLOTS = 16;
+__host__ __device__ constexpr int prescore_claim_rows(int R) {
+	return 4 * R;
+}
+__device__ __forceinline__ float code_to_float(uint32_t w, int k) {
+	return (float)(int)(int8_t)(w >> (8 * k));
+}
+constexpr int TOUCH_MAX = 4;
+template <int MT, int NCH, int CR>
+__device__ __forceinline__ unsigned long long prescore_codes(const RowSpace &sp, const PrescoreView &pv, uint32_t dim,
+                                                             const float4 *q_lds, float qa2, const uint32_t *ids, int n,
+                                                             float bound, float *out, uint32_t &rejected,
+                                                             const uint32_t *hint_word, unsigned long long &touch) {
+	static_assert(NCH >= 2, "full-wave rows only");
+	const uint32_t lane = lane_id();
+	constexpr int PER = 64 / CR;
+	uint32_t w[NCH][CR];
+	float sc[CR];
+#pragma unroll
+	for (int r = 0; r < CR; ++r) {
+		const uint32_t id = ids[r < n ? r : n - 1];
+		const uint32_t *crow = pv.codes + (size_t)id * sp.V;
+#pragma unroll
+		for (int ch = 0; ch < NCH; ++ch)
+			w[ch][r] = crow[lane + ch * 64];
+		sc[r] = MT == 0 ? pv.meta[id].scale : 0.f;
+	}
+	const int jm = (int)(lane / PER) < n ? (int)(lane / PER) : n - 1;
+	const float4 mraw = *reinterpret_cast<const float4 *>(pv.meta + ids[jm]);
+	__builtin_amdgcn_sched_barrier(0);
+	float t[CR];
+#pragma unroll
+	for (int r = 0; r < CR; ++r)
+		t[r] = 0.f;
+#pragma unroll
+	for (int ch = 0; ch < NCH; ++ch) {
+		const float4 q = q_lds[lane + ch * 64];
+		const float qs[4] = {q.x, q.y, q.z, q.w};
+#pragma unroll
+		for (int r = 0; r < CR; ++r)
+#pragma unroll
+			for (int k = 0; k < 4; ++k) {
+				const float c = code_to_float(w[ch][r], k);
+				if (MT == 0) {
+					const float v = __fmaf_rn(-sc[r], c, qs[k]);
+					t[r] = __fmaf_rn(v, v, t[r]);
+				} else {
+					t[r] = __fmaf_rn(qs[k], c, t[r]);
+				}
+			}
+	}
+	transposed_reduce64<CR>(t);
+	RowCodeMeta m;
+	m.scale = mraw.x, m.err = mraw.y, m.norm = mraw.z, m.spare = 0;
+	const float qn = MT == 0 ? 1.f : vss_sqrt(qa2);
+	const float lb = prescore_bound(MT, t[0], t[0], m, qn, dim);
+	const bool mine = (lane % PER) == 0 && (int)(lane / PER) < n;
+	const bool rej = mine && lb >= bound;
+	if (rej)
+		out[lane / PER] = __builtin_inff();
+	rejected += (uint32_t)__popcll(__ballot(rej));
+	touch = 0;
+	if (hint_word) {
+		const float hint = __uint_as_float((uint32_t)uniform((int)VSS_LDS_LOAD(lds_u32, hint_word)));
+		unsigned long long cand = __ballot(mine && !rej && prescore_touches(prescore_estimate(MT, t[0], t[0], m, qn), bound, hint));
+#pragma unroll
+		for (int i = 0; i < TOUCH_MAX; ++i) {
+			touch |= cand & (0ull - cand);
+			cand &= cand - 1ull;
+		}
+	}
+	return __ballot(mine && !rej);
+}
+template <int MT, int NCH, int RR, class Hook>
+__device__ __forceinline__ void wave_distances_picked(const RowSpace &sp, const float4 *q_lds, float qa2, const uint32_t *ids,
+                                                      unsigned long long &left, int lane_shift, float *out, const Hook &after_issue) {
+	const uint32_t lane = lane_id();
+	int pos[RR], last = 0;
+	const float4 *row[RR];
+#pragma unroll
+	for (int r = 0; r < RR; ++r) {
+		if (left)
+			last = (int)(__builtin_ctzll(left) >> lane_shift);
+		pos[r] = last;
+		left &= left - 1ull;
+		row[r] = sp.vectors + (size_t)ids[pos[r]] * sp.V;
+	}
+	float4 x[NCH][RR];
+#pragma unroll
+	for (int ch = 0; ch < NCH; ++ch)
+#pragma unroll
+		for (int r = 0; r < RR; ++r)
+			x[ch][r] = row[r][lane + ch * 64];
+	after_issue();
+	float ab[RR], b2[RR];
+#pragma unroll
+	for (int r = 0; r < RR; ++r)
+		ab[r] = 0.f, b2[r] = 0.f;
+#pragma unroll
+	for (int ch = 0; ch < NCH; ++ch) {
+		const float4 q = q_lds[lane + ch * 64];
+#pragma unroll
+		for (int r = 0; r < RR; ++r)
+			accumulate4<MT>(q, x[ch][r], ab[r], b2[r]);
+	}
+	transposed_reduce64<RR>(ab);
+	if (MT == 1)
+		transposed_reduce64<RR>(b2);
+	constexpr int PER = 64 / RR;
+	int j = pos[0];
+#pragma unroll
+	for (int r = 1; r < RR; ++r)
+		j = (int)(lane / PER) == r ? pos[r] : j;
+	if ((lane % PER) == 0)
+		out[j] = finish_distance<MT>(ab[0], qa2, b2[0]);
+}
+
+
+
+constexpr uint32_t TOUCH_NO_LEVEL = 0xFFFFFFFFu;
+struct NoTouch {
+	__device__ __forceinline__ void operator()() const {
+	}
+};
+struct SuccessorTouch {
+	const GraphView *gv;
+	const uint32_t *ids;
+	unsigned long long lanes;
+	uint32_t level;
+	int shift;
+	uint32_t *sink;
+	__device__ __forceinline__ void operator()() const {
+		if (lanes) {
+			const uint32_t l = (uint32_t)lane_id(), row = l >> shift, line = l & ((1u << shift) - 1u);
+			const uint32_t lines = (level == 0 ? gv->M0 : gv->M) > 32 ? 2u : 1u;
+			if (((lanes >> (row << shift)) & 1ull) && line < lines) {
+				const uint32_t id = ids[row];
+				const uint32_t *list = level == 0 ? gv->links0 + (size_t)id * gv->M0
+				                                  : gv->links_up + ((size_t)gv->upper_off[id] + (level - 1)) * gv->M;
+				*sink = list[line * 32u];
+			}
+		}
+	}
+};
 template <int MT, int NCH, int R, bool PRE = false>
 __device__ __forceinline__ bool pool_score(Mailbox *mb, unsigned long long *scrap, const RowSpace &sp, const float4 *q,
                                            const uint32_t *ids, float *dist, const PrescoreView *pv = nullptr, uint32_t dim = 0,
-                                           uint32_t *pre_counts = nullptr) {
+                                           uint32_t *pre_counts = nullptr, const GraphView *gv = nullptr, uint32_t touch_on = 0) {
 	const int lane = lane_id();
+	uint32_t sink = 0;
 	unsigned long long *ticket_or_scrap = lane == 0 ? &mb->ticket : scrap + lane;
 	uint32_t *done_or_scrap = lane == 0 ? &mb->done : reinterpret_cast<uint32_t *>(scrap + lane);
 	bool worked = false;
 	for (;;) {
 		uint32_t slots = (uint32_t)uniform((int)VSS_LDS_LOAD(lds_u32, &mb->slots));
+		if constexpr (PRE)
+			asm volatile("" ::"v"(sink));
 		const bool wide_claim = PRE && slots == PRESCORE_SLOTS;
 		slots = slots == 1 || slots == 2 ? slots : (uint32_t)R;
 		const uint32_t pass = wide_claim ? (uint32_t)prescore_claim_rows(R) : slots * (64u >> sp.logG);
@@ -713,18 +767,24 @@
 					constexpr int CR = prescore_claim_rows(R);
 					constexpr int SHIFT = CR == 16 ? 2 : CR == 8 ? 3 : 4;
 					static_assert(CR == 16 || CR == 8 || CR == 4, "rows of codes per claim");
-					unsigned long long left = prescore_codes<MT, NCH, CR>(sp, *pv, dim, q, qa2, ids + c, (int)cnt, bound, dist + c, pre_counts[1]);
+					const uint32_t level = touch_on ? (uint32_t)uniform((int)VSS_LDS_LOAD(lds_u32, &mb->level)) : TOUCH_NO_LEVEL;
+					SuccessorTouch touch {gv, ids + c, 0ull, level, SHIFT, &sink};
+					unsigned long long left = prescore_codes<MT, NCH, CR>(sp, *pv, dim, q, qa2, ids + c, (int)cnt, bound, dist + c, pre_counts[1],
+					                                                      level != TOUCH_NO_LEVEL ? &mb->touch_bits : nullptr, touch.lanes);
 					pre_counts[0] += cnt;
+					pre_counts[2] += level == 0 ? (uint32_t)__popcll(touch.lanes) : 0u;
+					pre_counts[3] += level == 0 ? 0u : (uint32_t)__popcll(touch.lanes);
 					while (left) {
 						const int have = __popcll(left);
 						if (have >= 3 && R >= 4)
-							wave_distances_picked<MT, NCH, (R >= 4 ? 4 : 1)>(sp, q, qa2, ids + c, left, SHIFT, dist + c);
+							wave_distances_picked<MT, NCH, (R >= 4 ? 4 : 1)>(sp, q, qa2, ids + c, left, SHIFT, dist + c, touch);
 						else if (have >= 2)
-							wave_distances_picked<MT, NCH, 2>(sp, q, qa2, ids + c, left, SHIFT, dist + c);
+							wave_distances_picked<MT, NCH, 2>(sp, q, qa2, ids + c, left, SHIFT, dist + c, touch);
 						else
-							wave_distances_picked<MT, NCH, 1>(sp, q, qa2, ids + c, left, SHIFT, dist + c);
+							wave_distances_picked<MT, NCH, 1>(sp, q, qa2, ids + c, left, SHIFT, dist + c, touch);
+						touch.lanes = 0;
 					}
-					wave_sync();
+					lds_sync();
 					VSS_LDS_ADD_REL(lds_u32, done_or_scrap, cnt);
 					VSS_TRACE_INC(sp, 29);
 					worked = true;
@@ -770,13 +830,16 @@
 	uint32_t touch_ok;
 	uint32_t prescore_ok;
 	unsigned long long *descent_counters;
+	uint32_t touch_successors;
+	mutable uint32_t level_known = 0;
 	mutable uint32_t crew_on = 0;
 	mutable uint32_t level = 0;
 	mutable float hop_bound = __builtin_inff();
 	mutable uint32_t hop_filtered = 0;
-	static constexpr bool bounds_descent = PRE;
+	static constexpr bool bounds_descent = PRE, counts_successors = PRE;
 	__device__ __forceinline__ void at_level(int l) const {
 		level = (uint32_t)l;
+		level_known = 1u;
 	}
 	__device__ __forceinline__ void at_bound(float bound) const {
 		hop_bound = (PRE && descent_counters) ? bound : __builtin_inff();
@@ -799,7 +862,8 @@
 		const uint32_t active = (uint32_t)uniform((int)VSS_LDS_LOAD(lds_u32, walkers_left));
 		return active ? active : 1u;
 	}
-	__device__ __forceinline__ bool post(int buf, const RowSpace &sp, int n, float bound = __builtin_inff()) const {
+	__device__ __forceinline__ bool post(int buf, const RowSpace &sp, int n, float bound = __builtin_inff(),
+	                                     uint32_t touch_level = TOUCH_NO_LEVEL) const {
 		Mailbox *box = mb + buf;
 		bool sent = false;
 		const uint32_t lg = 6u - sp.logG;
@@ -809,6 +873,9 @@
 			const bool filtered = bound < __builtin_inff() && a * x2 > scorers;
 			VSS_LDS_STORE(lds_u32, &box->slots, a * x1 <= scorers ? 1u : a * x2 <= scorers ? 2u : filtered ? PRESCORE_SLOTS : (uint32_t)R);
 			VSS_LDS_STORE(lds_u32, &box->bound_bits, __float_as_uint(filtered ? bound : __builtin_inff()));
+			if (touch_successors)
+				VSS_LDS_STORE(lds_u64, reinterpret_cast<unsigned long long *>(&box->touch_bits),
+				              ((unsigned long long)touch_level << 32) | 0x7F800000ull);
 			sent = filtered;
 		} else {
 			VSS_LDS_STORE(lds_u32, &box->slots, a * x1 <= scorers ? 1u : a * x2 <= scorers ? 2u : (uint32_t)R);
@@ -839,7 +906,8 @@
 		wave_sync();
 		VSS_TRACE_INC(sp, 18);
 	}
-	__device__ __forceinline__ bool begin(int buf, const RowSpace &sp, float qa2, int n, float bound = __builtin_inff()) const {
+	__device__ __forceinline__ bool begin(int buf, const RowSpace &sp, float qa2, int n, float bound = __builtin_inff(),
+	                                      uint32_t touch_level = TOUCH_NO_LEVEL) const {
 		if (crew_ok && !crew_on && uniform((int)VSS_LDS_LOAD(lds_u32, walkers_left)) == 1) {
 			crew_on = 1u;
 #ifdef VSS_PHASE_TIMERS
@@ -857,7 +925,17 @@
 			lds_barrier();
 			return false;
 		}
-		return post(buf, sp, n, bound);
+		return post(buf, sp, n, bound, touch_level);
+	}
+	__device__ __forceinline__ void hint(int buf, float best_unexpanded) const {
+		if (PRE && touch_successors && !crew_on)
+			VSS_LDS_STORE(lds_u32, &mb[buf].touch_bits, __float_as_uint(best_unexpanded));
+	}
+	__device__ __forceinline__ void add_touch_counts(unsigned long long *counters, uint32_t expansions, uint32_t fresh) const {
+		if (PRE && touch_successors && expansions && lane_id() == 0) {
+			atomicAdd(counters + 6, (unsigned long long)expansions);
+			atomicAdd(counters + 7, (unsigned long long)fresh);
+		}
 	}
 	__device__ __forceinline__ void end(int buf, const RowSpace &sp, int n) const {
 		if (crew_on)
@@ -874,7 +952,7 @@
 			return;
 		}
 		VSS_TICK(tp0);
-		hop_filtered = begin(0, sp, qa2, n, hop_bound) ? 1u : 0u;
+		hop_filtered = begin(0, sp, qa2, n, hop_bound, level_known ? level : TOUCH_NO_LEVEL) ? 1u : 0u;
 		VSS_TICK(tpb);
 		VSS_ACC(t_solo_passes, tp0, tpb);
 		before_loads();
@@ -1346,7 +1424,7 @@
 	ListCache<PK> ahead;
 	float e_d = __builtin_inff();
 	uint32_t e_s = EMPTY_SLOT;
-	auto request_ahead = [&] {
+	auto request_ahead = [&](int buf, int n) {
 		float d1 = 0.f;
 		uint32_t s1 = 0, s2 = 0;
 		int have;
@@ -1357,6 +1435,8 @@
 		}
 		e_d = have > 0 ? d1 : __builtin_inff();
 		e_s = have > 0 ? s1 : EMPTY_SLOT;
+		if (n > 0)
+			pool.hint(buf, e_d);
 		if (!pool.wants_requests())
 			return;
 		if (have > 0)
@@ -1375,8 +1455,11 @@
 		const int n = gather_neighbors<true>(gv, lds, cs, 0, have_first, first_cells);
 		VSS_TICK(tg1);
 		VSS_ACC(t_gather, tg0, tg1);
+#ifdef VSS_PHASE_TIMERS
+		wc.t_team_passes += lds.t_list_wait, lds.t_list_wait = 0;
+#endif
 		if (n > 0)
-			pool.begin(buf, gv.sp, qa2, n, L.size >= limit ? radius : __builtin_inff());
+			pool.begin(buf, gv.sp, qa2, n, L.size >= limit ? radius : __builtin_inff(), 0u);
 		VSS_TICK(tg2);
 		VSS_ACC(t_solo_passes, tg1, tg2);
 		return n;
@@ -1400,12 +1483,14 @@
 				break;
 			L.mark_expanded(pos);
 			wc.cycles += 1;
+			if constexpr (Pool::counts_successors)
+				wc.pipelined += 1;
 			VSS_TICK(tk1);
 			VSS_ACC(t_pick, tk0, tk1);
 			n_cur = open_expansion(cs, b);
 			if (n_cur < 0)
 				return LEVEL_VISITED_OVERFLOW;
-			request_ahead();
+			request_ahead(b, n_cur);
 			continue;
 		}
 		VSS_TICK(tw0);
@@ -1430,8 +1515,11 @@
 			const unsigned long long who = __ballot(admitted && !(d > m));
 			const float ms = __int_as_float(uniform(__float_as_int(m)));
 			tie = who && (__popcll(who) > 1 || !(__builtin_fabsf(ms) < __builtin_inff()) || ms == e_d);
-			if (!tie)
+			if (!tie) {
 				next = (who && ms < e_d) ? read_lane(id, __builtin_ctzll(who)) : e_s;
+				if constexpr (Pool::counts_successors)
+					wc.fresh += (who && ms < e_d) ? 1u : 0u;
+			}
 		}
 		VSS_TICK(tw2);
 		VSS_ACC(t_pick, tw1, tw2);
@@ -1446,6 +1534,8 @@
 		int n_next = 0;
 		if (next != EMPTY_SLOT) {
 			wc.cycles += 1;
+			if constexpr (Pool::counts_successors)
+				wc.pipelined += 1;
 			n_next = open_expansion(next, nb);
 			if (n_next < 0)
 				return LEVEL_VISITED_OVERFLOW;
@@ -1469,7 +1559,7 @@
 		if (next == EMPTY_SLOT)
 			break;
 		L.mark_expanded(pos);
-		request_ahead();
+		request_ahead(nb, n_next);
 		VSS_TICK(ta1);
 		VSS_ACC(t_accept, ta0, ta1);
 		b = nb;
@@ -1568,6 +1658,7 @@
 	unsigned long long *phase_ticks;
 	PrescoreView prescore;
 	uint32_t prescore_descent;
+	uint32_t touch_successors;
 };
 
 __device__ __forceinline__ void bind_visited(VisitedSet &v, uint32_t *table, uint32_t hash_log2) {
@@ -1833,17 +1924,22 @@
 		boxes[threadIdx.x].qa2_bits = 0;
 		boxes[threadIdx.x].slots = R;
 		boxes[threadIdx.x].bound_bits = 0x7F800000u;
+		boxes[threadIdx.x].touch_bits = 0x7F800000u, boxes[threadIdx.x].level = TOUCH_NO_LEVEL;
 	}
 	__syncthreads();
 	constexpr bool PRE = NCH >= 2 && E >= 1 && E != LDS_LIST_E && E <= pipelined_max_regs(THREADS);
 
 	if (wave >= S) {
-		uint32_t pre_counts[2] = {0, 0};
+		uint32_t pre_counts[4] = {0, 0, 0, 0};
 		auto leave = [&] {
 			if constexpr (PRE) {
 				if (lane == 0 && pre_counts[0]) {
 					atomicAdd(a.prescore.counters, (unsigned long long)pre_counts[0]);
 					atomicAdd(a.prescore.counters + 1, (unsigned long long)pre_counts[1]);
+					if (pre_counts[2] | pre_counts[3]) {
+						atomicAdd(a.prescore.counters + 4, (unsigned long long)pre_counts[2]);
+						atomicAdd(a.prescore.counters + 5, (unsigned long long)pre_counts[3]);
+					}
 				}
 			}
 		};
@@ -1856,7 +1952,8 @@
 					const EngineSlot es =
 					    engine_slot(smem, s >> 1, a.hash_log2, a.gv.sp.V, a.list_cap_max, hash_in_lds, a.stage_cap, list_cells);
 					worked |= pool_score<MT, NCH, R, PRE>(&boxes[s], scrap, a.gv.sp, es.q, (s & 1) ? es.ids2 : es.ids,
-					                                      (s & 1) ? es.dist2 : es.dist, &a.prescore, a.gv.dim, pre_counts);
+					                                      (s & 1) ? es.dist2 : es.dist, &a.prescore, a.gv.dim, pre_counts, &a.gv,
+					                                      a.touch_successors);
 				}
 			}
 			if (uniform((int)VSS_LDS_LOAD(lds_u32, exit_flag))) {
@@ -1889,7 +1986,8 @@
 	PoolScorer<MT, NCH, R, PRE> score {&boxes[2 * wave], exit_flag, a.engine_error, walkers_left, (blockDim.x >> 6) - S, crew, wave,
 	                                   ((a.crew & CREW_ON) && !a.spec_active) ? 1u : 0u, (a.crew & CREW_NO_REQUESTS) ? 1u : 0u,
 	                                   (a.crew & CREW_TOUCH) ? 1u : 0u, (PRE && a.prescore.codes) ? 1u : 0u,
-	                                   (PRE && a.prescore.codes && a.prescore_descent) ? a.prescore.counters + 2 : nullptr};
+	                                   (PRE && a.prescore.codes && a.prescore_descent) ? a.prescore.counters + 2 : nullptr,
+	                                   (PRE && a.prescore.codes) ? a.touch_successors : 0u};
 	const SpecBuffers sb {es.ids, es.ids2, es.dist, es.dist2};
 	CandQueue cq;
 	cq.bind(a.cand_buf + gslot * 2 * a.cand_cap, reinterpret_cast<uint32_t *>(a.cand_buf + gslot * 2 * a.cand_cap) + a.cand_cap,
@@ -1952,9 +2050,11 @@
 		else if (a.spec_active)
 			rc = level_search_spec<MT>(a.gv, lds, sb, qa2, closest, limit, L, score, a.spec_active, wc);
 		else if (E > 0 && E != LDS_LIST_E && E <= pipelined_max_regs(THREADS) && a.pipelined) {
-			if constexpr (E > 0 && E != LDS_LIST_E && E <= pipelined_max_regs(THREADS))
+			if constexpr (E > 0 && E != LDS_LIST_E && E <= pipelined_max_regs(THREADS)) {
 				rc = level_search_pipelined<MT, PK>(a.gv, lds, sb, qa2, closest, limit, L, score, wc);
-			else
+				if constexpr (PRE)
+					score.add_touch_counts(a.prescore.counters, wc.pipelined, wc.fresh);
+			} else
 				rc = LEVEL_INTERNAL;
 		} else
 			rc = level_search_impl<MT, false, false, PK>(a.gv, lds, qa2, closest, EMPTY_SLOT, 0, limit, L, cq, score, wc);
diff --git a/duckdb-vss_amd/csrc/host_logic.h b/duckdb-vss_amd/csrc/host_logic.h
--- a/duckdb-vss_amd/csrc/host_logic.h
+++ b/duckdb-vss_amd/csrc/host_logic.h
@@ -322,6 +322,7 @@
 	bool search_pipelined = true, search_wide_lists = true;
 	uint32_t search_list_lds = 1, search_prescore = 1;
 	bool search_prescore_descent = true;
+	bool search_touch_successors = true;
 	bool retry_in_place = true;
 	uint64_t visited_per_limit = 0;
 	uint32_t hash_lds_max_log2 = 13, hash_lds_max_override = 0;
@@ -349,6 +350,7 @@
 	uint32_t pipelined = 0, crew = 0, touch_lines = 0, spec_active = 0;
 	bool wants_prescore = false;
 	uint32_t prescore_descent = 0;
+	uint32_t touch_successors = 0;
 	uint64_t global_hash = 0, retry_hash = 0, list_buf = 0, cand_buf = 0;
 	uint32_t shape[8] = {0, 0, 0, 0, 0, 0, 0, 0};
 };
@@ -433,6 +435,7 @@
 	a.crew = shape.crew ? (CREW_ON | ((policy.touch_lists && list_cap_max <= 64) ? CREW_TOUCH : 0u) | e.search_crew_tune) : 0u;
 	a.wants_prescore = a.pipelined && !in.direct_io && (e.search_prescore == 2 || !wide_limit);
 	a.prescore_descent = (a.wants_prescore && e.search_prescore_descent) ? 1u : 0u;
+	a.touch_successors = (a.wants_prescore && e.search_touch_successors) ? 1u : 0u;
 	a.nch = chunks_per_lane(e.V, e.G, policy.force_looping);
 	a.regs = (uint32_t)((in.limit + 63) / 64);
 	a.lds_bytes = solo ? solo_lds + (a.team ? TEAM_BOX_BYTES : 0u) : engine_lds(S);
diff --git a/duckdb-vss_amd/csrc/prescore_bound.h b/duckdb-vss_amd/csrc/prescore_bound.h
--- a/duckdb-vss_amd/csrc/prescore_bound.h
+++ b/duckdb-vss_amd/csrc/prescore_bound.h
@@ -60,4 +60,31 @@
 	return prescore_round_down(lb);
 }
 
+constexpr float PRESCORE_NO_ESTIMATE = INFINITY;
+
+VSS_PRESCORE_HD inline float prescore_estimate(int metric, float t, float s2, const RowCodeMeta &m, float q_norm) {
+	const double scale = m.scale, E = m.err, rn = m.norm, qn = q_norm;
+	if (!(E < (double)INFINITY) || !(scale > 0.0) || !(rn >= 0x1p-40 && rn <= 0x1p40) || !(E <= rn))
+		return PRESCORE_NO_ESTIMATE;
+	if (metric != 0 && !(qn >= 0x1p-40 && qn <= 0x1p40))
+		return PRESCORE_NO_ESTIMATE;
+	double est;
+	if (metric == 0) {
+		if (!(s2 >= 0.f) || !(s2 < INFINITY))
+			return PRESCORE_NO_ESTIMATE;
+		return s2;
+	}
+	if (!(fabsf(t) < INFINITY))
+		return PRESCORE_NO_ESTIMATE;
+	est = metric == 1 ? 1.0 - scale * (double)t / (qn * rn) : 1.0 - scale * (double)t;
+	if (!(est == est))
+		return PRESCORE_NO_ESTIMATE;
+	return (float)est;
 }
+
+VSS_PRESCORE_HD inline bool prescore_touches(float estimate, float bound, float hint) {
+	const float lim = hint < bound ? hint : bound;
+	return estimate < lim && bound < INFINITY;
+}
+
+}
diff --git a/duckdb-vss_amd/csrc/vss_engine.hip b/duckdb-vss_amd/csrc/vss_engine.hip
--- a/duckdb-vss_amd/csrc/vss_engine.hip
+++ b/duckdb-vss_amd/csrc/vss_engine.hip
@@ -581,7 +581,7 @@
 		uint64_t stats[4] = {0, 0, 0, 0};
 		DevBuf<unsigned long long> d_prescore;
 		unsigned long long *h_prescore = nullptr;
-		unsigned long long prescore_base[4] = {0, 0, 0, 0};
+		unsigned long long prescore_base[8] = {0, 0, 0, 0, 0, 0, 0, 0};
 		bool prescore_first = false, prescore_used = false;
 	};
 	static constexpr int EXPLICIT_CTX = 4, MAX_CTX = 12;
@@ -617,6 +617,7 @@
 
 	uint32_t search_prescore = 1;
 	bool search_prescore_descent = true;
+	bool search_touch_successors = true;
 	DevBuf<uint32_t> d_codes;
 	DevBuf<RowCodeMeta> d_code_meta;
 	StaleSlots codes_stale;
@@ -624,6 +625,7 @@
 	uint64_t codes_refused_capacity = 0;
 	uint64_t last_prescore[4] = {0, 0, 0, 0};
 	uint64_t last_prescore_descent[2] = {0, 0};
+	uint64_t last_touches[4] = {0, 0, 0, 0};
 	bool codes_wanted() const {
 		const uint32_t nch = (G == 64 && V % 64 == 0 && !force_looping) ? V / 64 : 0;
 		return search_prescore && (nch == 2 || nch == 3 || nch == 4 || nch == 6);
@@ -1084,6 +1086,7 @@
 		e.search_waves = search_waves, e.search_walkers_cap = search_walkers_cap, e.search_wgs_per_cu = search_wgs_per_cu;
 		e.search_spec_active = search_spec_active, e.search_pipelined = search_pipelined, e.search_wide_lists = search_wide_lists;
 		e.search_list_lds = search_list_lds, e.search_prescore = search_prescore, e.search_prescore_descent = search_prescore_descent;
+		e.search_touch_successors = search_touch_successors;
 		e.retry_in_place = retry_in_place, e.visited_per_limit = visited_per_limit;
 		e.hash_lds_max_log2 = HASH_LDS_MAX_LOG2, e.hash_lds_max_override = hash_lds_max_override;
 		e.visited_compact_on = visited_compact_on, e.search_crew_tune = search_crew_tune;
@@ -1394,15 +1397,16 @@
 		}
 		if (codes_ready) {
 			if (!c.d_prescore.p) {
-				c.d_prescore.ensure(4, 0, c.stream, 0);
-				HIP_TRY(hipHostMalloc((void **)&c.h_prescore, 4 * sizeof(unsigned long long), hipHostMallocDefault));
-				for (int i = 0; i < 4; ++i)
+				c.d_prescore.ensure(8, 0, c.stream, 0);
+				HIP_TRY(hipHostMalloc((void **)&c.h_prescore, 8 * sizeof(unsigned long long), hipHostMallocDefault));
+				for (int i = 0; i < 8; ++i)
 					c.h_prescore[i] = 0, c.prescore_base[i] = 0;
 			}
 			a.prescore = PrescoreView {d_codes.p, d_code_meta.p, c.d_prescore.p};
 			c.prescore_used = true;
 		}
 		a.prescore_descent = a.prescore.codes ? plan.prescore_descent : 0u;
+		a.touch_successors = a.prescore.codes ? plan.touch_successors : 0u;
 		if (c.first_pass)
 			c.prescore_first = a.prescore.codes != nullptr;
 		a.global_hash = nullptr;
@@ -1473,7 +1477,7 @@
 			HIP_TRY(hipMemcpyAsync(c.h_stats, c.d_stats.p, c.nq * 8, hipMemcpyDeviceToHost, c.stream));
 		}
 		if (a.prescore.codes)
-			HIP_TRY(hipMemcpyAsync(c.h_prescore, c.d_prescore.p, 4 * sizeof(unsigned long long), hipMemcpyDeviceToHost, c.stream));
+			HIP_TRY(hipMemcpyAsync(c.h_prescore, c.d_prescore.p, 8 * sizeof(unsigned long long), hipMemcpyDeviceToHost, c.stream));
 	}
 
 	bool search_gating = true;
@@ -1866,6 +1870,11 @@
 				last_prescore_descent[1] = c.h_prescore[3] - c.prescore_base[3];
 				c.prescore_base[2] = c.h_prescore[2], c.prescore_base[3] = c.h_prescore[3];
 			}
+			for (int i = 0; i < 4; ++i) {
+				last_touches[i] = c.prescore_used ? c.h_prescore[4 + i] - c.prescore_base[4 + i] : 0;
+				if (c.prescore_used)
+					c.prescore_base[4 + i] = c.h_prescore[4 + i];
+			}
 			last_prescore[3] = d_codes.n * sizeof(uint32_t) + d_code_meta.n * sizeof(RowCodeMeta);
 			timing[0] = c.kernel_ms;
 			if (keep_query_stats)
@@ -2495,6 +2504,7 @@
 			std::fill(last_shape, last_shape + 8, 0);
 			std::fill(last_prescore, last_prescore + 4, 0);
 			last_prescore_descent[0] = last_prescore_descent[1] = 0;
+			std::fill(last_touches, last_touches + 4, 0);
 		}
 		if (!ng && !n_unknown)
 			return VSS_OK;
@@ -3322,6 +3332,8 @@
      "at most 256, 2 in every pipelined launch"},
     {"search.prescore_descent", 0, 1, [](vss_index *h, int64_t v) { h->search_prescore_descent = v != 0; },
      "in launches that filter on row codes, the greedy descent's rows are bounded against its closest distance too"},
+    {"search.touch_successors", 0, 1, [](vss_index *h, int64_t v) { h->search_touch_successors = v != 0; },
+     "in launches that filter on row codes, scoring waves pull the likely successor's neighbour list into L2 ahead of the walker"},
 };
 const char *set_option_checked(vss_index *h, const char *name, int64_t value) {
 	for (const OptionRule &r : OPTION_RULES) {
@@ -3394,7 +3406,7 @@
 	    {"VSS_SEARCH_RETRY_IN_PLACE", "search.retry_in_place"}, {"VSS_HASH_LDS_MAX_LOG2", "search.visited_lds_log2_max"},
 	    {"VSS_VISITED_PER_LIMIT", "search.visited_cells_per_limit"}, {"VSS_PROBE_FLAG_WAIT", "search.probe_flag_wait"},
 	    {"VSS_SEARCH_LIST_LDS", "search.list_lds"}, {"VSS_SEARCH_PRESCORE", "search.prescore"},
-	    {"VSS_SEARCH_PRESCORE_DESCENT", "search.prescore_descent"},
+	    {"VSS_SEARCH_PRESCORE_DESCENT", "search.prescore_descent"}, {"VSS_SEARCH_TOUCH_SUCCESSORS", "search.touch_successors"},
 	};
 	for (const auto &e : ENV_OPTIONS)
 		if (const char *t = getenv(e.env)) {
@@ -4469,6 +4481,14 @@
 	})
 }
 
+int vss_last_search_touches(vss_index *h, uint64_t *out4) {
+	VSS_SHARED(h, {
+		std::lock_guard<std::mutex> lk(h->stats_mu);
+		std::memcpy(out4, h->last_touches, sizeof h->last_touches);
+		return VSS_OK;
+	})
+}
+
 uint64_t vss_last_exact_fallbacks(vss_index *h) {
 	if (!h)
 		return 0;
diff --git a/include/vssgpu.h b/include/vssgpu.h
--- a/include/vssgpu.h
+++ b/include/vssgpu.h
@@ -182,6 +182,7 @@
 int vss_last_search_shape(vss_index *index, uint32_t *out8);
 int vss_last_search_prescore(vss_index *index, uint64_t *out4);
 int vss_last_search_prescore_descent(vss_index *index, uint64_t *out2);
+int vss_last_search_touches(vss_index *index, uint64_t *out4);
 int vss_timing(vss_index *index, double *out6, int reset);
 int vss_build_work(vss_index *index, uint64_t *out3);
 int vss_last_search_query_stats(vss_index *index, uint32_t *out, uint64_t n_queries);
```

New measurement: 1.500 million. -11.9%, worse.
